# eric612/Mobilenet-YOLO-Pytorch

Hardware: AMD Instinct MI355X
Metric: images/sec MobileNetV2-YOLO 352x352 fwd+bwd @ bs256 (higher is better)
Workload: dtype f32; 1 GPU; MobileNetV2-YOLO 352x352 bs=256/GPU fwd+loss+bwd fp32 (BASELINE configs[1]); global_batch=256, parallelism=dp1

## Files before the change

### include/mnyolo.h

```cpp
#ifndef MNYOLO_H
#define MNYOLO_H

#include <stddef.h>
#include <stdint.h>

#ifdef __cplusplus
extern "C" {
#endif
#pragma GCC visibility push(default)

#define MNY_OK 0
#define MNY_EINVAL (-1)
#define MNY_EHIP (-2)
#define MNY_EUNSUPPORTED (-3)

#define MNY_ACT_NONE 0
#define MNY_ACT_RELU6 1
#define MNY_ACT_LEAKY 2
#define MNY_ACT_RELU 3
#define MNY_ACT_HSWISH 4
#define MNY_ACT_HSIGMOID 5

int mny_version(void);
const char* mny_last_error(void);
// ... 58 lines not shown
int mny_bn_bwd_parts(int64_t M, int C);
int mny_bn_bwd_finalize(const float* red, int parts, int64_t count, const float* gamma,
                        const float* mean, const float* invstd,
                        float* dgamma, float* dbeta, float* coef , int C, void* stream);
int mny_bn_bwd_apply(const float* g, const float* y, const float* scale, const float* shift, int act,
                     const float* coef, float* dy, int64_t M, int C, void* stream);

int mny_add_views(const float* a, const float* a_scale, const float* a_shift, int a_act,
                  const float* b, const float* b_scale, const float* b_shift, int b_act,
                  const float* up, float* out, int N, int H, int W, int C, void* stream);
int mny_mul_views(const float* a, const float* a_scale, const float* a_shift, int a_act,
                  const float* b, const float* b_scale, const float* b_shift, int b_act,
                  float* out, int64_t M, int C, void* stream);
int mny_mul_views_bwd(const float* g, const float* o, const float* o_scale, const float* o_shift, int o_act,
                      const float* addend, float* dst, int64_t M, int C, void* stream);
int mny_partadd_up(const float* a, const float* a_scale, const float* a_shift, int a_act, const float* up,
                   float* out, int N, int H, int W, int Ca, int Cb, void* stream);
int mny_slice_channels(const float* src, float* dst, int accumulate, int64_t M, int Ca, int Cb, void* stream);
int mny_upsample_bwd(const float* src, float* dst, int accumulate, int N, int H, int W, int C, void* stream);
int mny_axpy(const float* src, const float* alpha, float* dst, int accumulate, int64_t n, void* stream);

typedef struct {
    int N, g, A, C;
    int n_anchors_all;
    float ignore_thresh, iou_thresh, iou_weighting;
} mny_yolo_head;

int mny_yolo_loss(const float* head, const float* targets, const int32_t* t_off,
                  const float* anchors_all, const int32_t* mask, const mny_yolo_head* hp,
                  float* out7, float* dhead, void* ws, void* stream);
size_t mny_yolo_loss_ws_bytes(const mny_yolo_head* hp, int total_targets);

int mny_yolo_decode(const float* head, const float* anchors_all, const int32_t* mask,
                    const mny_yolo_head* hp, float val_conf, float* rows, int row_stride,
                    const int32_t* base_counts, int32_t* counts, void* stream);

int mny_nms_per_class(const float* rows, const int32_t* seg_begin, const int32_t* seg_count, int S,
                      int capacity, int max_seg_rows, int num_classes, double thr,
                      int32_t* out_idx, int32_t* out_counts, float* out_rows, void* ws, void* stream);
size_t mny_nms_ws_bytes(int S, int capacity, int num_classes);
size_t mny_nms_status_offset(int S, int capacity, int num_classes);
size_t mny_nms_prefix_offset(int S, int capacity, int num_classes);

int mny_dw_bnbwd_supported(int K, int stride);
int mny_dw_bnbwd_parts(int N, int H, int W, int C);
int mny_dw_bnbwd_parts_k(int N, int H, int W, int C, int K, int flags);
int mny_dw_bnbwd(const float* g, const float* y, const float* scale, const float* shift, int act, const float* coef,
                 const float* x, const float* in_scale, const float* in_shift, int in_act, const float* w,
                 const float* addend, float* dx, float* dw, float* ws, int N, int H, int W, int C, int K, int stride,
                 void* stream);
int mny_dw_bnbwd_s2_parts(int N, int H, int W, int C);
int mny_dw_bnbwd_s2(const float* g, const float* y, const float* scale, const float* shift, int act, const float* coef,
                    const float* x, const float* in_scale, const float* in_shift, int in_act, const float* w,
                    const float* addend, float* dx, float* dw, float* ws, int N, int H, int W, int C, void* stream);
int mny_dw_bnbwd_red(const float* g, const float* y, const float* scale, const float* shift, int act, const float* coef,
                     const float* x, const float* in_scale, const float* in_shift, int in_act, const float* in_mean,
                     const float* in_invstd, const float* w, const float* addend, float* dx, float* dw, float* ws, float* in_red,
                     int N, int H, int W, int C, int K, int stride, void* stream);

int mny_lr_supported(int64_t M, int K, int C);
int mny_lr_gram_parts(int64_t M, int K);
int mny_lr_gram(const float* x, const float* in_scale, const float* in_shift, int in_act, float* parts, int64_t M, int K, void* stream);
int mny_lr_gram_bf16(const void* x, const float* in_scale, const float* in_shift, int in_act, float* parts, int64_t M, int K, void* stream);
int mny_lr_prep(const float* coef, const float* w, float* q, float* r, int C, int K, void* stream);
int mny_pw_lr_fix_parts(int64_t M, int K, int r_act);
int mny_pw_lr_fix(const float* x, const float* in_scale, const float* in_shift, const float* q, const float* r, const float* addend, float* dx,
                  const float* ry, const float* r_scale, const float* r_shift, int r_act, const float* r_mean, const float* r_invstd, float* red,
                  int64_t M, int K, void* stream);
int mny_lr_wfix(float* dw, const float* gram_sums, const float* coef, const float* w, int C, int K, void* stream);
int mny_dw_bnbwd_s2_red_dz(const float* g, const float* y, const float* scale, const float* shift, int act, const float* coef,
                           const float* x, const float* in_scale, const float* in_shift, int in_act, const float* in_mean,
                           const float* in_invstd, const float* w, const float* addend, float* dx, float* dw, float* ws, float* in_red,
                           int N, int H, int W, int C, void* stream);
int mny_dw_bnbwd_s2k5_parts(int N, int H, int W, int C);
int mny_dw_bnbwd_s2k5(const float* g, const float* y, const float* scale, const float* shift, int act, const float* coef,
                      const float* x, const float* in_scale, const float* in_shift, int in_act, const float* in_mean,
                      const float* in_invstd, const float* w, const float* addend, float* dx, float* dw, float* ws, float* in_red,
                      int N, int H, int W, int C, void* stream);
int mny_dw_bnbwd_s2k5_bf16(const void* g, const void* y, const float* scale, const float* shift, int act, const float* coef,
                           const void* x, const float* in_scale, const float* in_shift, int in_act, const float* in_mean,
                           const float* in_invstd, const float* w, const void* addend, void* dx, float* dw, float* ws, float* in_red,
                           int N, int H, int W, int C, void* stream);
int mny_dw_bnbwd_red_dz_supported(int K, int C, int bf16);
int mny_dw_bnbwd_red_dz(const float* g, const float* y, const float* scale, const float* shift, int act, const float* coef,
                        const float* x, const float* in_scale, const float* in_shift, int in_act, const float* in_mean,
                        const float* in_invstd, const float* w, const float* addend, float* dx, float* dw, float* ws, float* in_red,
                        int N, int H, int W, int C, int K, int stride, void* stream);

int mny_pad_rows(const float* src, const float* alpha, float* dst, int64_t M, int C, int Cp, void* stream);
int mny_transpose_pad(const float* src , float* dst , int R, int Cc, int Rp, void* stream);

typedef struct mny_reduce_job {
    const float* parts;
    float* out;
    int64_t n;
    int32_t nparts, block0;
} mny_reduce_job;
int mny_reduce_batch(const mny_reduce_job* jobs, const int32_t* block_job, int nblocks, void* stream);
int mny_pw_wgrad_splits(int64_t M, int K, int Nc);

typedef struct mny_transpose_job {
    const float* src;
    void* dst;
    int32_t R, Cc, Rp, block0;
} mny_transpose_job;
int mny_transpose_batch(const mny_transpose_job* jobs, const int32_t* block_job, int nblocks, void* stream);

typedef struct mny_adamw_chunk {
    float* p;
    const float* g;
    float* m;
    float* v;
    int n;
    int vec4;
} mny_adamw_chunk;
int mny_adamw_step(const mny_adamw_chunk* table_dev, int nchunks, double lr, double beta1, double beta2, double eps,
                   double weight_decay, int64_t step, void* stream);

int mny_pw_dgrad_bnred_supported(int64_t M, int K, int Nc, int act);
int mny_pw_dgrad_bnred_parts(int64_t M, int K, int Nc);
int mny_pw_dgrad_bnred(const float* dy, const float* wT, float* dx, const float* y, const float* scale,
                       const float* shift, int act, const float* mean, const float* invstd, float* red,
                       int64_t M, int K, int Nc, void* stream);
int mny_pw_dgrad_bnred_add_supported(int64_t M, int K, int Nc, int act);
int mny_pw_dgrad_bnred_add(const float* dy, const float* wT, const float* addend, float* dx, const float* y, const float* scale,
                           const float* shift, int act, const float* mean, const float* invstd, float* red, int64_t M, int K, int Nc,
                           void* stream);

typedef struct mny_cut3_job {
    const float* src;
    void* dst;
    int32_t R, C, block0, pad;
} mny_cut3_job;
int mny_pw_w6_supported(int64_t M, int K, int Nc);
size_t mny_pw_w6_bytes(int K, int Nc);
int mny_cut3_batch(const mny_cut3_job* jobs, const int32_t* block_job, int nblocks, void* stream);
int mny_pw_fwd_w6(const float* x, const float* in_scale, const float* in_shift, int in_act, const void* w6, const float* bias,
                  const float* addend, float* y, float* stats, int64_t M, int K, int Nc, void* stream);
int mny_pw_dgrad_bnred_w6(const float* dy, const void* wT6, const float* addend, float* dx, const float* y, const float* scale,
                          const float* shift, int act, const float* mean, const float* invstd, float* red, int64_t M, int K, int Nc,
                          void* stream);

enum {
    MNY_ROUTE_TILE_V1 = 0,
    MNY_ROUTE_DMA_F32 = 1,
    MNY_ROUTE_DMA_X6 = 2,
    MNY_ROUTE_THIN = 3,
    MNY_ROUTE_WIDE = 4,
    MNY_ROUTE_WGRAD_STREAM = 5,
    MNY_ROUTE_WAVE16 = 6
};
int mny_pw_route(int op, int bf16, int64_t M, int K, int Nc);
int mny_pw_last_route(void);

size_t mny_map_ws_bytes(int64_t D, int64_t T);
int mny_map_eval(const float* det_boxes , const float* det_labels, const float* det_scores,
                 const int32_t* det_off , const float* true_boxes ,
                 const float* true_labels, const float* true_diff, const int32_t* true_off, int n_images,
                 int64_t D, int64_t T, int n_classes, float* ap, float* tp_sum, float* fp_sum, float* prec11,
                 float* mean_ap, void* ws, void* stream);
int mny_eval_pack(const float* rows, int64_t D, const float* targets, int64_t T, float* det_boxes,
                  float* det_labels, float* det_scores, float* true_boxes, float* true_labels,
                  float* true_diff, void* stream);

size_t mny_seg_loss_ws_bytes(int64_t n);
int mny_seg_loss(const float* head, const float* seg_maps, int64_t n, float* out3, float* dhead, void* ws,
                 void* stream);
int mny_seg_sigmoid(const float* head , int h, int w, int C, float* out,
                    void* stream);

typedef struct mny_image_desc {
    int64_t offset;
    int32_t h, w;
} mny_image_desc;
size_t mny_prep_ws_bytes(int N, int max_in_h, int max_in_w, int out_h, int out_w);
int mny_prep_batch(const uint8_t* src, const mny_image_desc* desc, int N, int max_in_h, int max_in_w, int out_h,
                   int out_w, const float* mean3, const float* std3, float* out, void* ws, void* stream);

#define MNY_AUG_BRIGHTNESS 0
#define MNY_AUG_CONTRAST 1
#define MNY_AUG_SATURATION 2
#define MNY_AUG_HUE 3
#define MNY_AUG_GAMMA 4
typedef struct mny_aug_item {
    mny_image_desc src;
    int32_t n_ops;
    int32_t op[5];
    float factor[5];
    int32_t hue_shift;
    uint8_t gamma_map[256];
    int32_t exp_h, exp_w, exp_top, exp_left;
    int32_t crop_top, crop_left, crop_h, crop_w;
    int32_t flip;
    int32_t sample;
    int32_t tile_x, tile_y, tile_w, tile_h;
    int32_t mask_x0, mask_y0, mask_x1, mask_y1;
} mny_aug_item;
typedef struct mny_aug_sample {
    int32_t first_item, n_items, canvas_slot, reserved;
} mny_aug_sample;
size_t mny_aug_ws_bytes(int n_items, int n_out, int n_mosaic, int max_in_h, int max_in_w, int canvas, int out_h,
                        int out_w);
int mny_aug_photometric(const uint8_t* src, const mny_aug_item* items, int n, int max_in_h, int max_in_w,
                        uint8_t* dst, void* ws, void* stream);
int mny_aug_batch(const uint8_t* src, const mny_aug_item* items, int n_items, const mny_aug_sample* samples,
                  int n_out, int max_in_h, int max_in_w, int canvas, int n_mosaic, int out_h, int out_w,
                  const float* mean3, const float* std3, float* out, void* ws, void* stream);

#define MNY_AUG_SEG_MAX_CLASSES 8
size_t mny_aug_seg_ws_bytes(int n_items, int n_out, int n_classes, int max_in_h, int max_in_w, int out_h, int out_w);
int mny_aug_seg_batch(const uint8_t* seg_src, const int64_t* seg_offsets, const mny_aug_item* items, int n_items,
                      const mny_aug_sample* samples, int n_out, int n_classes, int max_in_h, int max_in_w, int out_h,
                      int out_w, float* out, void* ws, void* stream);

int mny_stem_fwd_bf16(const float* x_nchw, const float* w, void* y, float* stats, int N, int H, int W, int Cout, void* stream);
int mny_stem_wgrad_bf16(const float* x_nchw, const void* dy, float* dw, float* ws, int N, int H, int W, int Cout, void* stream);
int mny_dw_fwd_bf16(const void* x, const float* in_scale, const float* in_shift, int in_act, const float* w, void* y,
                    float* stats, int N, int H, int W, int C, int K, int stride, void* stream);
int mny_dw_bwd_data_bf16(const void* dy, const float* w, const void* addend, void* dx, int N, int H, int W, int C, int K,
                         int stride, void* stream);
int mny_dw_bwd_weight_bf16(const void* x, const float* in_scale, const float* in_shift, int in_act, const void* dy,
                           float* dw, float* ws, int N, int H, int W, int C, int K, int stride, void* stream);
int mny_pw_fwd_bf16(const void* x, const float* in_scale, const float* in_shift, int in_act, const void* w_bf16,
                    const float* bias, const void* addend, void* y, float* stats, int64_t M, int K, int Nc, void* stream);
int mny_transpose_bf16(const float* src , void* dst , int R, int Cc, void* stream);
int mny_pw_stat_parts_bf16(int64_t M, int K, int Nc);
int mny_pw_wgrad_bf16(const void* x, const float* in_scale, const float* in_shift, int in_act, const void* dy, float* dw,
                      float* dbias, float* ws, int64_t M, int K, int Nc, void* stream);
int mny_bn_bwd_reduce_bf16(const void* g, const void* y, const float* scale, const float* shift, int act, const float* mean,
                           const float* invstd, float* red, int64_t M, int C, void* stream);
int mny_bn_bwd_apply_bf16(const void* g, const void* y, const float* scale, const float* shift, int act, const float* coef,
                          void* dy, int64_t M, int C, void* stream);
int mny_add_views_bf16(const void* a, const float* a_scale, const float* a_shift, int a_act, const void* b,
                       const float* b_scale, const float* b_shift, int b_act, const void* up, void* out, int N, int H, int W,
                       int C, void* stream);
int mny_mul_views_bf16(const void* a, const float* a_scale, const float* a_shift, int a_act, const void* b,
                       const float* b_scale, const float* b_shift, int b_act, void* out, int64_t M, int C, void* stream);
int mny_mul_views_bwd_bf16(const void* g, const void* o, const float* o_scale, const float* o_shift, int o_act,
                           const void* addend, void* dst, int64_t M, int C, void* stream);
int mny_partadd_up_bf16(const void* a, const float* a_scale, const float* a_shift, int a_act, const void* up, void* out,
                        int N, int H, int W, int Ca, int Cb, void* stream);
int mny_slice_channels_bf16(const void* src, void* dst, int accumulate, int64_t M, int Ca, int Cb, void* stream);
int mny_upsample_bwd_bf16(const void* src, void* dst, int accumulate, int N, int H, int W, int C, void* stream);
int mny_dw_bnbwd_bf16(const void* g, const void* y, const float* scale, const float* shift, int act, const float* coef,
                      const void* x, const float* in_scale, const float* in_shift, int in_act, const float* w,
                      const void* addend, void* dx, float* dw, float* ws, int N, int H, int W, int C, int K, int stride,
                      void* stream);
int mny_dw_bnbwd_s2_bf16(const void* g, const void* y, const float* scale, const float* shift, int act, const float* coef,
                         const void* x, const float* in_scale, const float* in_shift, int in_act, const float* w,
                         const void* addend, void* dx, float* dw, float* ws, int N, int H, int W, int C, void* stream);
int mny_dw_bnbwd_red_bf16(const void* g, const void* y, const float* scale, const float* shift, int act, const float* coef,
                          const void* x, const float* in_scale, const float* in_shift, int in_act, const float* in_mean,
                          const float* in_invstd, const float* w, const void* addend, void* dx, float* dw, float* ws, float* in_red,
                          int N, int H, int W, int C, int K, int stride, void* stream);
int mny_pad_rows_bf16(const float* src, const float* alpha, void* dst, int64_t M, int C, int Cp, void* stream);
int mny_transpose_pad_bf16(const float* src, void* dst, int R, int Cc, int Rp, void* stream);
int mny_stem_bnwgrad_bf16(const float* x_nchw, const void* g, const void* y, const float* scale, const float* shift, int act,
                          const float* coef, float* dw, float* ws, int N, int H, int W, int Cout, void* stream);
int mny_pw_bnbwd_supported_bf16(int64_t M, int K, int Nc);
int mny_pw_bnbwd_bf16(const void* g, const void* y, const float* scale, const float* shift, int act, const float* mean, const float* invstd,
                      const float* gamma, const void* x, const float* in_scale, const float* in_shift, int in_act, const float* w,
                      const void* addend, void* dx, float* dw, float* dgamma, float* dbeta, float* ws, int64_t M, int K, int Nc, void* stream);
int mny_pw_dgrad_bnred_supported_bf16(int64_t M, int K, int Nc, int act);
int mny_pw_dgrad_bnred_parts_bf16(int64_t M, int K, int Nc);
int mny_pw_dgrad_bnred_bf16(const void* dy, const void* wT, void* dx, const void* y, const float* scale, const float* shift, int act,
                            const float* mean, const float* invstd, float* red, int64_t M, int K, int Nc, void* stream);
int mny_pw_dgrad_bnred_add_supported_bf16(int64_t M, int K, int Nc, int act);
int mny_pw_dgrad_bnred_add_bf16(const void* dy, const void* wT, const void* addend, void* dx, const void* y, const float* scale,
                                const float* shift, int act, const float* mean, const float* invstd, float* red, int64_t M, int K,
                                int Nc, void* stream);
int mny_transpose_batch_bf16(const mny_transpose_job* jobs, const int32_t* block_job, int nblocks, void* stream);
int mny_pw_wgrad_splits_bf16(int64_t M, int K, int Nc);
int mny_axpy_bf16(const void* src, const float* alpha, void* dst, int accumulate, int64_t n, void* stream);
typedef struct mny_cvt_job {
    const float* src;
    void* dst;
    int64_t n;
    int32_t block0, pad_;
} mny_cvt_job;
int mny_cvt_batch_f32_bf16(const mny_cvt_job* jobs, const int32_t* block_job, int nblocks, void* stream);
int mny_cvt_f32_bf16(const float* src, void* dst, int64_t n, void* stream);
int mny_cvt_bf16_f32(const void* src, float* dst, int64_t n, void* stream);

int mny_bn_eval_stats(const float* running_mean, const float* running_var, float eps, float* mean_out, float* invstd_out, int C,
                      void* stream);
int mny_bn_bwd_finalize_frozen(const float* red, int parts, int64_t count, const float* gamma, const float* mean, const float* invstd,
                               float* dgamma, float* dbeta, float* coef, int C, void* stream);
int mny_exdw_supported(int N, int H, int W, int K, int C, int stride);
int mny_exdw_stat_parts(int64_t M, int K, int C);
int mny_exdw_stats(const float* x, const float* in_scale, const float* in_shift, int in_act, const float* w_exp, float* stats,
                   int64_t M, int K, int C, void* stream);
int mny_exdw_fwd_parts(int N, int H, int W, int K, int C, int stride);
int mny_exdw_fwd(const float* x, const float* in_scale, const float* in_shift, int in_act, const float* w_exp,
                 const float* e_scale, const float* e_shift, const float* w_dw, float* z, float* z_stats,
                 int N, int H, int W, int K, int C, int stride, void* stream);
int mny_exdw_bwd_parts(int N, int H, int W, int K, int C, int stride);
size_t mny_exdw_bwd_ws_floats(int N, int H, int W, int K, int C, int stride);
int mny_exdw_bwd(const float* gz, const float* z, const float* z_scale, const float* z_shift, int z_act, const float* z_coef,
                 const float* x, const float* in_scale, const float* in_shift, int in_act, const float* w_exp,
                 const float* e_scale, const float* e_shift, const float* e_mean, const float* e_invstd, const float* e_gamma,
                 const float* w_dw, const float* addend, float* dx, float* dw_exp, float* dgamma_e, float* dbeta_e,
                 float* dw_dw, float* dw_ws, float* ws, int N, int H, int W, int K, int C, int stride, void* stream);
int mny_exdw_bwd_red_parts(int N, int H, int W, int K, int C, int stride);
int mny_exdw_bwd_red(const float* gz, const float* z, const float* z_scale, const float* z_shift, int z_act, const float* z_coef,
                     const float* x, const float* in_scale, const float* in_shift, int in_act, const float* in_mean, const float* in_invstd,
                     const float* w_exp, const float* e_scale, const float* e_shift, const float* e_mean, const float* e_invstd,
// ... 59 lines not shown
```

### mobilenet-yolo-pytorch_amd/_lib.py

```python
import ctypes
import os
from ctypes import c_char_p, c_double, c_float, c_int, c_int32, c_int64, c_size_t, c_void_p

from . import switches

HERE = os.path.dirname(os.path.abspath(__file__))
LIB_PATH = switches.get("MNY_LIB") or os.path.join(HERE, "libmnyolo.so")

ACT_NONE, ACT_RELU6, ACT_LEAKY, ACT_RELU, ACT_HSWISH, ACT_HSIGMOID = 0, 1, 2, 3, 4, 5
ROUTE_TILE_V1, ROUTE_DMA_F32, ROUTE_DMA_X6, ROUTE_THIN, ROUTE_WIDE, ROUTE_WGRAD_STREAM, ROUTE_WAVE16 = 0, 1, 2, 3, 4, 5, 6


class MnyError(RuntimeError):
    pass


class YoloHead(ctypes.Structure):
    _fields_ = [("N", c_int), ("g", c_int), ("A", c_int), ("C", c_int), ("n_anchors_all", c_int),
                ("ignore_thresh", c_float), ("iou_thresh", c_float), ("iou_weighting", c_float)]


P = c_void_p
_SIGS = {
    "mny_version": (c_int, []),
    "mny_last_error": (c_char_p, []),
    "mny_max_parts": (c_int, []),
    "mny_stem_fwd": (c_int, [P, P, P, P, c_int, c_int, c_int, c_int, P]),
    "mny_stem_stat_parts": (c_int, [c_int, c_int, c_int, c_int]),
    "mny_stem_wgrad": (c_int, [P, P, P, P, c_int, c_int, c_int, c_int, P]),
    "mny_stem_bnwgrad_supported": (c_int, [c_int]),
    "mny_stem_bnwgrad": (c_int, [P, P, P, P, P, c_int, P, P, P, c_int, c_int, c_int, c_int, P]),
    "mny_stem_wgrad_parts": (c_int, [c_int, c_int, c_int, c_int]),
    "mny_dw_fwd": (c_int, [P, P, P, c_int, P, P, P, c_int, c_int, c_int, c_int, c_int, c_int, P]),
    "mny_dw_stat_parts": (c_int, [c_int] * 6),
    "mny_dw_stat_parts_x": (c_int, [c_int] * 7),
    "mny_dw_bwd_data": (c_int, [P, P, P, P, c_int, c_int, c_int, c_int, c_int, c_int, P]),
    "mny_dw_bwd_weight": (c_int, [P, P, P, c_int, P, P, P, c_int, c_int, c_int, c_int, c_int, c_int, P]),
    "mny_dw_wgrad_parts": (c_int, [c_int] * 6),
    "mny_dw_bnbwd_supported": (c_int, [c_int, c_int]),
    "mny_dw_bnbwd_parts": (c_int, [c_int] * 4),
    "mny_dw_bnbwd_parts_k": (c_int, [c_int] * 6),
    "mny_dw_bnbwd": (c_int, [P, P, P, P, c_int, P, P, P, P, c_int, P, P, P, P, P, c_int, c_int, c_int, c_int, c_int, c_int, P]),
    "mny_dw_bnbwd_s2_parts": (c_int, [c_int] * 4),
    "mny_dw_bnbwd_s2": (c_int, [P, P, P, P, c_int, P, P, P, P, c_int, P, P, P, P, P, c_int, c_int, c_int, c_int, P]),
    "mny_dw_bnbwd_red": (c_int, [P, P, P, P, c_int, P, P, P, P, c_int, P, P, P, P, P, P, P, P, c_int, c_int, c_int, c_int, c_int, c_int, P]),
    "mny_exdw_supported": (c_int, [c_int] * 6),
    "mny_exdw_stat_parts": (c_int, [c_int64, c_int, c_int]),
    "mny_exdw_stats": (c_int, [P, P, P, c_int, P, P, c_int64, c_int, c_int, P]),
    "mny_exdw_fwd_parts": (c_int, [c_int] * 6),
    "mny_exdw_fwd": (c_int, [P, P, P, c_int, P, P, P, P, P, P, c_int, c_int, c_int, c_int, c_int, c_int, P]),
    "mny_exdw_bwd_parts": (c_int, [c_int] * 6),
    "mny_exdw_bwd_ws_floats": (c_size_t, [c_int] * 6),
    "mny_exdw_bwd": (c_int, [P, P, P, P, c_int, P, P, P, P, c_int, P, P, P, P, P, P, P, P, P, P, P, P, P, P, P,
                             c_int, c_int, c_int, c_int, c_int, c_int, P]),
    "mny_exdw_bwd_red_parts": (c_int, [c_int] * 6),
    "mny_exdw_bwd_red": (c_int, [P, P, P, P, c_int, P, P, P, P, c_int, P, P, P, P, P, P, P, P, P, P, P, P, P, P, P, P, P, P,
                                 c_int, c_int, c_int, c_int, c_int, c_int, P]),
    "mny_pj_bwd_supported": (c_int, [c_int64, c_int, c_int, c_int]),
    "mny_pj_bwd_parts": (c_int, [c_int64, c_int, c_int]),
    "mny_pj_bwd": (c_int, [P, P, P, P, P, P, P, P, c_int, P, P, P, P, P, c_int64, c_int, c_int, P]),
    "mny_stemdw_supported": (c_int, [c_int] * 6),
    "mny_stemdw_bwd_parts": (c_int, [c_int] * 4),
    "mny_stemdw_bwd_ws_floats": (c_size_t, [c_int] * 4),
    "mny_stemdw_bwd": (c_int, [P, P, P, P, c_int, P, P, P, P, P, P, P, c_int, P, P, P, P, P, P, P, P, P, c_int, c_int, c_int, c_int, P]),
    "mny_adamw_step": (c_int, [P, c_int, c_double, c_double, c_double, c_double, c_double, c_int64, P]),
    "mny_pw_fwd": (c_int, [P, P, P, c_int, P, P, P, P, P, c_int64, c_int, c_int, P]),
    "mny_pw_stat_parts": (c_int, [c_int64, c_int, c_int]),
    "mny_pw_wgrad": (c_int, [P, P, P, c_int, P, P, P, P, c_int64, c_int, c_int, P]),
    "mny_pw_wgrad_ws_floats": (c_size_t, [c_int64, c_int, c_int]),
    "mny_pw_bnbwd_supported": (c_int, [c_int64, c_int, c_int]),
    "mny_pw_bnbwd_ws_floats": (c_size_t, [c_int64, c_int, c_int]),
    "mny_pw_bnbwd": (c_int, [P, P, P, P, c_int, P, P, P, P, P, P, c_int, P, P, P, P, P, P, P, c_int64, c_int, c_int, P]),
    "mny_pw_dgrad_bnred_supported": (c_int, [c_int64, c_int, c_int, c_int]),
    "mny_pw_dgrad_bnred_parts": (c_int, [c_int64, c_int, c_int]),
    "mny_pw_dgrad_bnred": (c_int, [P, P, P, P, P, P, c_int, P, P, P, c_int64, c_int, c_int, P]),
    "mny_pw_dgrad_bnred_add_supported": (c_int, [c_int64, c_int, c_int, c_int]),
    "mny_pw_dgrad_bnred_add": (c_int, [P, P, P, P, P, P, P, c_int, P, P, P, c_int64, c_int, c_int, P]),
    "mny_pw_route": (c_int, [c_int, c_int, c_int64, c_int, c_int]),
    "mny_pw_last_route": (c_int, []),
    "mny_pw_w6_supported": (c_int, [c_int64, c_int, c_int]),
    "mny_pw_w6_bytes": (c_size_t, [c_int, c_int]),
    "mny_cut3_batch": (c_int, [P, P, c_int, P]),
    "mny_pw_fwd_w6": (c_int, [P, P, P, c_int, P, P, P, P, P, c_int64, c_int, c_int, P]),
    "mny_pw_dgrad_bnred_w6": (c_int, [P, P, P, P, P, P, P, c_int, P, P, P, c_int64, c_int, c_int, P]),
    "mny_transpose_batch": (c_int, [P, P, c_int, P]),
    "mny_reduce_batch": (c_int, [P, P, c_int, P]),
    "mny_pw_wgrad_splits": (c_int, [c_int64, c_int, c_int]),
    "mny_transpose": (c_int, [P, P, c_int, c_int, P]),
    "mny_transpose_pad": (c_int, [P, P, c_int, c_int, c_int, P]),
    "mny_pad_rows": (c_int, [P, P, P, c_int64, c_int, c_int, P]),
    "mny_bn_finalize": (c_int, [P, c_int, c_int64, P, P, c_float, c_float, P, P, P, P, P, P, c_int, P]),
    "mny_bn_eval_coeffs": (c_int, [P, P, P, P, c_float, P, P, c_int, P]),
    "mny_bn_bwd_reduce": (c_int, [P, P, P, P, c_int, P, P, P, c_int64, c_int, P]),
    "mny_bn_bwd_parts": (c_int, [c_int64, c_int]),
    "mny_bn_bwd_finalize": (c_int, [P, c_int, c_int64, P, P, P, P, P, P, c_int, P]),
    "mny_bn_eval_stats": (c_int, [P, P, c_float, P, P, c_int, P]),
    "mny_bn_bwd_finalize_frozen": (c_int, [P, c_int, c_int64, P, P, P, P, P, P, c_int, P]),
    "mny_bn_bwd_apply": (c_int, [P, P, P, P, c_int, P, P, c_int64, c_int, P]),
    "mny_add_views": (c_int, [P, P, P, c_int, P, P, P, c_int, P, P, c_int, c_int, c_int, c_int, P]),
    "mny_mul_views": (c_int, [P, P, P, c_int, P, P, P, c_int, P, c_int64, c_int, P]),
    "mny_mul_views_bwd": (c_int, [P, P, P, P, c_int, P, P, c_int64, c_int, P]),
    "mny_partadd_up": (c_int, [P, P, P, c_int, P, P, c_int, c_int, c_int, c_int, c_int, P]),
    "mny_slice_channels": (c_int, [P, P, c_int, c_int64, c_int, c_int, P]),
    "mny_upsample_bwd": (c_int, [P, P, c_int, c_int, c_int, c_int, c_int, P]),
    "mny_axpy": (c_int, [P, P, P, c_int, c_int64, P]),
    "mny_yolo_loss": (c_int, [P, P, P, P, P, ctypes.POINTER(YoloHead), P, P, P, P]),
    "mny_yolo_loss_ws_bytes": (c_size_t, [ctypes.POINTER(YoloHead), c_int]),
    "mny_yolo_decode": (c_int, [P, P, P, ctypes.POINTER(YoloHead), c_float, P, c_int, P, P, P]),
    "mny_nms_per_class": (c_int, [P, P, P, c_int, c_int, c_int, c_int, c_double, P, P, P, P, P]),
    "mny_nms_ws_bytes": (c_size_t, [c_int, c_int, c_int]),
    "mny_nms_status_offset": (c_size_t, [c_int, c_int, c_int]),
    "mny_nms_prefix_offset": (c_size_t, [c_int, c_int, c_int]),
    "mny_map_ws_bytes": (c_size_t, [c_int64, c_int64]),
    "mny_map_eval": (c_int, [P, P, P, P, P, P, P, P, c_int, c_int64, c_int64, c_int, P, P, P, P, P, P, P]),
    "mny_seg_loss_ws_bytes": (c_size_t, [c_int64]),
    "mny_seg_loss": (c_int, [P, P, c_int64, P, P, P, P]),
    "mny_seg_sigmoid": (c_int, [P, c_int, c_int, c_int, P, P]),
    "mny_prep_ws_bytes": (c_size_t, [c_int] * 5),
    "mny_prep_batch": (c_int, [P, P, c_int, c_int, c_int, c_int, c_int, P, P, P, P, P]),
    "mny_aug_ws_bytes": (c_size_t, [c_int] * 8),
    "mny_aug_photometric": (c_int, [P, P, c_int, c_int, c_int, P, P, P]),
    "mny_aug_batch": (c_int, [P, P, c_int, P, c_int, c_int, c_int, c_int, c_int, c_int, c_int, P, P, P, P, P]),
    "mny_aug_seg_ws_bytes": (c_size_t, [c_int] * 7),
    "mny_aug_seg_batch": (c_int, [P, P, P, c_int, P, c_int, c_int, c_int, c_int, c_int, c_int, P, P, P]),
    "mny_eval_pack": (c_int, [P, c_int64, P, c_int64, P, P, P, P, P, P, P]),
}
BF16_TWINS = ("mny_pj_bwd_supported", "mny_pj_bwd_parts", "mny_pj_bwd", "mny_pw_bnbwd_supported", "mny_pw_bnbwd", "mny_pw_wgrad_splits", "mny_transpose_batch", "mny_pw_dgrad_bnred_supported", "mny_pw_dgrad_bnred_parts", "mny_pw_dgrad_bnred", "mny_pw_dgrad_bnred_add", "mny_pw_dgrad_bnred_add_supported", "mny_stem_bnwgrad", "mny_pad_rows", "mny_transpose_pad", "mny_dw_bnbwd", "mny_dw_bnbwd_s2", "mny_dw_bnbwd_red", "mny_stem_fwd", "mny_stem_wgrad", "mny_dw_fwd", "mny_dw_bwd_data", "mny_dw_bwd_weight", "mny_pw_fwd",
              "mny_pw_stat_parts", "mny_pw_wgrad", "mny_bn_bwd_reduce", "mny_bn_bwd_apply", "mny_add_views", "mny_mul_views",
              "mny_mul_views_bwd", "mny_partadd_up", "mny_slice_channels", "mny_upsample_bwd", "mny_axpy")
for _n in BF16_TWINS:
    _SIGS[_n + "_bf16"] = _SIGS[_n]
_SIGS["mny_gate_supported"] = (c_int, [c_int64, c_int, c_int])
_SIGS["mny_gate_parts"] = (c_int, [c_int64])
_SIGS["mny_gate_bwd_parts"] = (c_int, [c_int64])
_SIGS["mny_gate_bwd_red3_supported"] = (c_int, [c_int, c_int])
_SIGS["mny_gate_wq_bytes"] = (c_size_t, [c_int, c_int])
_SIGS["mny_gate_cut_batch_bf16"] = (c_int, [P, c_int, P])
_SIGS["mny_gate_stats1_bf16"] = (c_int, [P, P, P, P, P, c_int64, c_int, c_int, P])
_SIGS["mny_gate_stats2_bf16"] = (c_int, [P, P, P, P, P, P, P, c_int64, c_int, c_int, P])
_SIGS["mny_gate_fwd_bf16"] = (c_int, [P, P, P, P, P, P, P, P, P, P, P, c_int, P, c_int64, c_int, c_int, P])
_SIGS["mny_gate_bwd1_bf16"] = (c_int, [P] * 12 + [c_int64, c_int, c_int, P])
_SIGS["mny_gate_bwd2_bf16"] = (c_int, [P] * 14 + [c_int64, c_int, c_int, P])
_SIGS["mny_gate_bwd3_bf16"] = (c_int, [P] * 16 + [c_int64, c_int, c_int, P])
_SIGS["mny_lr_supported"] = (c_int, [c_int64, c_int, c_int])
_SIGS["mny_lr_gram_parts"] = (c_int, [c_int64, c_int])
_SIGS["mny_lr_gram"] = (c_int, [P, P, P, c_int, P, c_int64, c_int, P])
_SIGS["mny_lr_gram_bf16"] = _SIGS["mny_lr_gram"]
_SIGS["mny_lr_prep"] = (c_int, [P, P, P, P, c_int, c_int, P])
_SIGS["mny_pw_lr_fix_parts"] = (c_int, [c_int64, c_int, c_int])
_SIGS["mny_pw_lr_fix"] = (c_int, [P, P, P, P, P, P, P, P, P, P, c_int, P, P, P, c_int64, c_int, P])
_SIGS["mny_lr_wfix"] = (c_int, [P, P, P, P, c_int, c_int, P])
_SIGS["mny_pw_bnbwd_red_supported"] = (c_int, [c_int64, c_int, c_int])
_SIGS["mny_pw_bnbwd_red_parts"] = (c_int, [c_int64, c_int, c_int])
_SIGS["mny_pw_bnbwd_red"] = (c_int, [P, P, P, P, c_int, P, P, P, P, P, P, c_int, P, P, P, P, P, P, P, P, P, P, c_int, P, P, P, c_int64, c_int, c_int, P])
_SIGS["mny_dw_bnbwd_red_dz_supported"] = (c_int, [c_int, c_int, c_int])
_SIGS["mny_dw_bnbwd_red_dz"] = _SIGS["mny_dw_bnbwd_red"]
_SIGS["mny_dw_bnbwd_s2_red_dz"] = (c_int, [P, P, P, P, c_int, P, P, P, P, c_int, P, P, P, P, P, P, P, P, c_int, c_int, c_int, c_int, P])
_SIGS["mny_dw_bnbwd_s2k5_parts"] = (c_int, [c_int] * 4)
_SIGS["mny_dw_bnbwd_s2k5"] = _SIGS["mny_dw_bnbwd_s2_red_dz"]
_SIGS["mny_dw_bnbwd_s2k5_bf16"] = _SIGS["mny_dw_bnbwd_s2_red_dz"]
_SIGS["mny_transpose_bf16"] = _SIGS["mny_transpose"]
_SIGS["mny_cvt_f32_bf16"] = (c_int, [P, P, c_int64, P])
_SIGS["mny_cvt_batch_f32_bf16"] = (c_int, [P, P, c_int, P])
_SIGS["mny_cvt_bf16_f32"] = (c_int, [P, P, c_int64, P])
EXPORTS = tuple(_SIGS)

_lib = None


def load():
    global _lib
    if _lib is None:
        if not os.path.exists(LIB_PATH):
            raise MnyError("libmnyolo.so not found at %s — run __graft_entry__.build() (hipcc, gfx950). "
                           "There is no CPU fallback." % LIB_PATH)
        switches.warn_unknown()
        lib = ctypes.CDLL(LIB_PATH)
        for name, (res, args) in _SIGS.items():
            fn = getattr(lib, name)
            fn.restype = res
            fn.argtypes = args
        _lib = lib
    return _lib


def call(name, *args):
    lib = load()
    rc = getattr(lib, name)(*args)
    if rc != 0:
        raise MnyError("%s failed (%d): %s" % (name, rc, lib.mny_last_error().decode()))


def query(name, *args):
    v = getattr(load(), name)(*args)
    if isinstance(v, int) and v < 0:
        raise MnyError("%s(%s) -> %d: %s" % (name, args, v, load().mny_last_error().decode()))
    return v
```

### mobilenet-yolo-pytorch_amd/build.py

```python
import os
import subprocess
from concurrent.futures import ThreadPoolExecutor

HERE = os.path.dirname(os.path.abspath(__file__))
CSRC = os.path.join(HERE, "csrc")
OBJ = os.path.join(CSRC, "_obj")
LIB = os.path.join(HERE, "libmnyolo.so")
HIPCC = os.environ.get("HIPCC", "/opt/rocm/bin/hipcc")
ARCH = "gfx950"
BASE_FLAGS = ["--offload-arch=" + ARCH, "-O3", "-std=c++17", "-fPIC", "-Wall", "-Wno-unused-function",
              "-fvisibility=hidden", "-fvisibility-inlines-hidden"]
EXTRA = {"detect.hip": ["-ffp-contract=off"], "evalmap.hip": ["-ffp-contract=off"], "prep.hip": ["-ffp-contract=off"],
         "augment.hip": ["-ffp-contract=off"]}


def sources():
    return sorted(f for f in os.listdir(CSRC) if f.endswith(".hip"))


def _stale(target, deps):
    if not os.path.exists(target):
        return True
    t = os.path.getmtime(target)
    return any(os.path.getmtime(d) > t for d in deps)


def build(force=False, verbose=False):
    os.makedirs(OBJ, exist_ok=True)
    headers = [os.path.join(CSRC, "common.h"), os.path.join(CSRC, "x6.h"), os.path.join(HERE, "..", "include", "mnyolo.h")]
    jobs, objs = [], []
    for src in sources():
        s = os.path.join(CSRC, src)
        o = os.path.join(OBJ, src[:-4] + ".o")
        objs.append(o)
        if force or _stale(o, [s] + headers):
            jobs.append([HIPCC] + BASE_FLAGS + EXTRA.get(src, []) + ["-c", s, "-o", o])

    def run(cmd):
        if verbose:
            print(" ".join(cmd))
        subprocess.check_call(cmd)

    if jobs:
        with ThreadPoolExecutor(max_workers=min(4, len(jobs))) as ex:
            list(ex.map(run, jobs))
    if jobs or force or _stale(LIB, objs):
        run([HIPCC, "--offload-arch=" + ARCH, "-shared", "-fPIC", "-fvisibility=hidden", "-Wl,--exclude-libs,ALL", "-o", LIB] + objs)
    return LIB


if __name__ == "__main__":
    print(build(verbose=True))
```

### mobilenet-yolo-pytorch_amd/csrc/bn_eltwise.hip

```cpp
#include "common.h"

namespace mny {

__device__ __forceinline__ void sum_partial_rows(const float* __restrict__ rows, int parts, int C, int c, int slice, double& s, double& q) {
    double s1 = 0.0, q1 = 0.0, s2 = 0.0, q2 = 0.0, s3 = 0.0, q3 = 0.0;
    s = 0.0; q = 0.0;
    int p = slice;
    const int64_t step = (int64_t)64 * C;
    const float* a = rows + (int64_t)p * 2 * C + c;
    for (; p + 480 < parts; p += 512, a += 16 * step) {
        float v[16], u[16];
#pragma unroll
        for (int i = 0; i < 16; ++i) { v[i] = a[i * step]; u[i] = a[i * step + C]; }
#pragma unroll
        for (int i = 0; i < 16; i += 4) {
            s += (double)v[i];      q += (double)u[i];
            s1 += (double)v[i + 1]; q1 += (double)u[i + 1];
            s2 += (double)v[i + 2]; q2 += (double)u[i + 2];
            s3 += (double)v[i + 3]; q3 += (double)u[i + 3];
        }
    }
    for (; p + 96 < parts; p += 128, a += 4 * step) {
        const float v0 = a[0], u0 = a[C], v1 = a[step], u1 = a[step + C], v2 = a[2 * step], u2 = a[2 * step + C], v3 = a[3 * step], u3 = a[3 * step + C];
        s += (double)v0;  q += (double)u0;
        s1 += (double)v1; q1 += (double)u1;
        s2 += (double)v2; q2 += (double)u2;
        s3 += (double)v3; q3 += (double)u3;
    }
    for (; p < parts; p += 32, a += step) {
        s += (double)a[0];
        q += (double)a[C];
    }
    s = (s + s1) + (s2 + s3);
    q = (q + q1) + (q2 + q3);
}

__global__ __launch_bounds__(1024) void bn_finalize_kernel(const float* __restrict__ stats, int parts, double count,
                                                          const float* __restrict__ gamma, const float* __restrict__ beta,
                                                          float eps, float momentum, float* running_mean, float* running_var,
                                                          float* scale, float* shift, float* mean_out, float* invstd_out, int C) {
    __shared__ double red[2][32][32];
    const int cl = threadIdx.x & 31, slice = threadIdx.x >> 5;
    const int c = blockIdx.x * 32 + cl;
    double s = 0.0, q = 0.0;
    if (c < C) {
        sum_partial_rows(stats, parts, C, c, slice, s, q);
    }
    red[0][slice][cl] = s;
    red[1][slice][cl] = q;
    __syncthreads();
    if (slice == 0 && c < C) {
        s = 0.0; q = 0.0;
        for (int i = 0; i < 32; ++i) { s += red[0][i][cl]; q += red[1][i][cl]; }
        const double mean = s / count;
        double var = q / count - mean * mean;
        if (var < 0.0) var = 0.0;
        const float invstd = (float)(1.0 / sqrt(var + (double)eps));
        const float sc = gamma[c] * invstd;
        scale[c] = sc;
        shift[c] = beta[c] - (float)mean * sc;
        if (mean_out) mean_out[c] = (float)mean;
        if (invstd_out) invstd_out[c] = invstd;
        if (running_mean) {
            const double unbiased = count > 1.0 ? var * count / (count - 1.0) : var;
            running_mean[c] = (1.f - momentum) * running_mean[c] + momentum * (float)mean;
            running_var[c] = (1.f - momentum) * running_var[c] + momentum * (float)unbiased;
        }
    }
}

__global__ void bn_eval_coeffs_kernel(const float* gamma, const float* beta, const float* rm, const float* rv, float eps,
                                      float* scale, float* shift, int C) {
    const int c = blockIdx.x * blockDim.x + threadIdx.x;
    if (c >= C) return;
    const float sc = gamma[c] / sqrtf(rv[c] + eps);
    scale[c] = sc;
    shift[c] = beta[c] - rm[c] * sc;
}

template <typename T>
__global__ __launch_bounds__(256) void bn_bwd_reduce_kernel(const T* __restrict__ g, const T* __restrict__ y,
                                                            const float* __restrict__ scale, const float* __restrict__ shift, int act,
                                                            const float* __restrict__ mean, const float* __restrict__ invstd,
                                                            float* __restrict__ red_out, int64_t M, int C, int cgb, int cg_total) {
    __shared__ float4 red[256 * 2];
    const int tid = threadIdx.x;
    const int cgl = tid % cgb, pix = tid / cgb, ppb = blockDim.x / cgb;
    const int cg = blockIdx.y * cgb + cgl;
    const bool cvalid = cg < cg_total;
    const int c = cg * 4;
    float4 s1 = f4zero(), s2 = f4zero();
    if (cvalid) {
        const float4 sc = ld4(scale + c), sh = ld4(shift + c), mu = ld4(mean + c), is = ld4(invstd + c);
        auto accum = [&](float4 gv, float4 yv) {
            float4 dz;
            dz.x = gv.x * act_bwd(fmaf(yv.x, sc.x, sh.x), act);
            dz.y = gv.y * act_bwd(fmaf(yv.y, sc.y, sh.y), act);
            dz.z = gv.z * act_bwd(fmaf(yv.z, sc.z, sh.z), act);
            dz.w = gv.w * act_bwd(fmaf(yv.w, sc.w, sh.w), act);
            add4(s1, dz);
            s2.x = fmaf(dz.x, (yv.x - mu.x) * is.x, s2.x);
            s2.y = fmaf(dz.y, (yv.y - mu.y) * is.y, s2.y);
            s2.z = fmaf(dz.z, (yv.z - mu.z) * is.z, s2.z);
            s2.w = fmaf(dz.w, (yv.w - mu.w) * is.w, s2.w);
        };
        const int64_t stride = (int64_t)gridDim.x * ppb;
        int64_t m = (int64_t)blockIdx.x * ppb + pix;
        constexpr int U = sizeof(T) == 2 ? 4 : 1;
        if (U > 1) {
            for (; m + (U - 1) * stride < M; m += U * stride) {
                float4 gv[U], yv[U];
#pragma unroll
                for (int u = 0; u < U; ++u) { gv[u] = ld4(g + (m + u * stride) * C + c); yv[u] = ld4(y + (m + u * stride) * C + c); }
#pragma unroll
                for (int u = 0; u < U; ++u) accum(gv[u], yv[u]);
            }
        }
        for (; m < M; m += stride) accum(ld4(g + m * C + c), ld4(y + m * C + c));
    }
    red[tid * 2] = s1;
    red[tid * 2 + 1] = s2;
    __syncthreads();
    if (pix == 0 && cvalid) {
        float4 a = f4zero(), b = f4zero();
        for (int p = 0; p < ppb; ++p) { add4(a, red[(p * cgb + cgl) * 2]); add4(b, red[(p * cgb + cgl) * 2 + 1]); }
        st4(red_out + (int64_t)blockIdx.x * 2 * C + c, a);
        st4(red_out + (int64_t)blockIdx.x * 2 * C + C + c, b);
    }
}

__global__ __launch_bounds__(1024) void bn_bwd_finalize_kernel(const float* __restrict__ red_in, int parts, double count,
                                                              const float* __restrict__ gamma, const float* __restrict__ mean,
                                                              const float* __restrict__ invstd, float* dgamma, float* dbeta,
                                                              float* coef, int C) {
    __shared__ double red[2][32][32];
    const int cl = threadIdx.x & 31, slice = threadIdx.x >> 5;
    const int c = blockIdx.x * 32 + cl;
    double s = 0.0, q = 0.0;
    if (c < C) {
        sum_partial_rows(red_in, parts, C, c, slice, s, q);
    }
    red[0][slice][cl] = s;
    red[1][slice][cl] = q;
    __syncthreads();
    if (slice == 0 && c < C) {
        s = 0.0; q = 0.0;
        for (int i = 0; i < 32; ++i) { s += red[0][i][cl]; q += red[1][i][cl]; }
        dbeta[c] = (float)s;
        dgamma[c] = (float)q;
        const double a = (double)gamma[c] * (double)invstd[c];
        const double b = -a * (double)invstd[c] * q / count;
        coef[c] = (float)a;
        coef[C + c] = (float)b;
        coef[2 * C + c] = (float)(-a * s / count - b * (double)mean[c]);
    }
}

template <typename T>
__global__ __launch_bounds__(256) void bn_bwd_apply_kernel(const T* __restrict__ g, const T* __restrict__ y,
                                                           const float* __restrict__ scale, const float* __restrict__ shift, int act,
                                                           const float* __restrict__ coef, T* __restrict__ dy,
                                                           int64_t M, int C, int cgb, int cg_total) {
    const int cgl = threadIdx.x % cgb, pix = threadIdx.x / cgb, ppb = blockDim.x / cgb;
    const int cg = blockIdx.y * cgb + cgl;
    if (cg >= cg_total) return;
    const int c = cg * 4;
    const float4 sc = scale ? ld4(scale + c) : f4one(), sh = scale ? ld4(shift + c) : f4zero();
    const float4 ca = coef ? ld4(coef + c) : f4one();
    const float4 cb = coef ? ld4(coef + C + c) : f4zero();
    const float4 cc = coef ? ld4(coef + 2 * C + c) : f4zero();
    for (int64_t m = (int64_t)blockIdx.x * ppb + pix; m < M; m += (int64_t)gridDim.x * ppb) {
        const float4 gv = ld4(g + m * C + c), yv = ld4(y + m * C + c);
        float4 o;
        o.x = fmaf(ca.x, gv.x * act_bwd(fmaf(yv.x, sc.x, sh.x), act), fmaf(cb.x, yv.x, cc.x));
        o.y = fmaf(ca.y, gv.y * act_bwd(fmaf(yv.y, sc.y, sh.y), act), fmaf(cb.y, yv.y, cc.y));
        o.z = fmaf(ca.z, gv.z * act_bwd(fmaf(yv.z, sc.z, sh.z), act), fmaf(cb.z, yv.z, cc.z));
        o.w = fmaf(ca.w, gv.w * act_bwd(fmaf(yv.w, sc.w, sh.w), act), fmaf(cb.w, yv.w, cc.w));
        st4_stream(dy + m * C + c, o);
    }
}

template <typename T>
__global__ __launch_bounds__(256) void add_views_kernel(const T* __restrict__ a, const float* __restrict__ a_scale,
                                                        const float* __restrict__ a_shift, int a_act,
                                                        const T* __restrict__ b, const float* __restrict__ b_scale,
                                                        const float* __restrict__ b_shift, int b_act,
                                                        const T* __restrict__ up, T* __restrict__ out,
                                                        int N, int H, int W, int C, int cgb, int cg_total) {
    const int cgl = threadIdx.x % cgb, pix = threadIdx.x / cgb, ppb = blockDim.x / cgb;
    const int cg = blockIdx.y * cgb + cgl;
    if (cg >= cg_total) return;
    const int c = cg * 4;
    const float4 asc = a_scale ? ld4(a_scale + c) : f4one(), ash = a_scale ? ld4(a_shift + c) : f4zero();
    const float4 bsc = b_scale ? ld4(b_scale + c) : f4one(), bsh = b_scale ? ld4(b_shift + c) : f4zero();
    const int64_t M = (int64_t)N * H * W;
    for (int64_t m = (int64_t)blockIdx.x * ppb + pix; m < M; m += (int64_t)gridDim.x * ppb) {
        float4 o = xform4(ld4(a + m * C + c), asc, ash, a_act);
        if (b) add4(o, xform4(ld4(b + m * C + c), bsc, bsh, b_act));
        if (up) {
            const int wi = (int)(m % W), hi = (int)((m / W) % H);
            const int64_t n = m / ((int64_t)W * H);
            add4(o, ld4(up + ((n * (H / 2) + hi / 2) * (W / 2) + wi / 2) * C + c));
        }
        st4_stream(out + m * C + c, o);
    }
}

template <typename T>
__global__ __launch_bounds__(256) void upsample_bwd_kernel(const T* __restrict__ src, T* __restrict__ dst, int accumulate,
                                                           int N, int H, int W, int C, int cgb, int cg_total) {
    const int cgl = threadIdx.x % cgb, pix = threadIdx.x / cgb, ppb = blockDim.x / cgb;
    const int cg = blockIdx.y * cgb + cgl;
    if (cg >= cg_total) return;
    const int c = cg * 4;
    const int Hh = H / 2, Wh = W / 2;
    const int64_t M = (int64_t)N * Hh * Wh;
    for (int64_t m = (int64_t)blockIdx.x * ppb + pix; m < M; m += (int64_t)gridDim.x * ppb) {
        const int wi = (int)(m % Wh), hi = (int)((m / Wh) % Hh);
        const int64_t n = m / ((int64_t)Wh * Hh);
        const T* s = src + ((n * H + 2 * hi) * W + 2 * wi) * C + c;
        float4 o = accumulate ? ld4(dst + m * C + c) : f4zero();
        add4(o, ld4(s)); add4(o, ld4(s + C));
        add4(o, ld4(s + (int64_t)W * C)); add4(o, ld4(s + (int64_t)W * C + C));
        st4(dst + m * C + c, o);
    }
}

template <typename T>
__global__ __launch_bounds__(256) void axpy_kernel(const T* __restrict__ src, const float* __restrict__ alpha,
                                                   T* __restrict__ dst, int accumulate, int64_t n4, int64_t n) {
    const float a = alpha ? alpha[0] : 1.f;
    for (int64_t i = (int64_t)blockIdx.x * blockDim.x + threadIdx.x; i < n4; i += (int64_t)gridDim.x * blockDim.x) {
        float4 v = ld4(src + i * 4);
        float4 d = accumulate ? ld4(dst + i * 4) : f4zero();
        d.x = fmaf(a, v.x, d.x); d.y = fmaf(a, v.y, d.y); d.z = fmaf(a, v.z, d.z); d.w = fmaf(a, v.w, d.w);
        st4(dst + i * 4, d);
    }
    if (blockIdx.x == 0 && threadIdx.x < (n & 3)) {
        const int64_t i = n4 * 4 + threadIdx.x;
        st1(dst + i, (accumulate ? ld1(dst + i) : 0.f) + a * ld1(src + i));
    }
}


template <typename T>
__global__ __launch_bounds__(256) void bn_bwd_reduce_c1_kernel(const T* __restrict__ g, const T* __restrict__ y,
                                                               const float* __restrict__ scale, const float* __restrict__ shift, int act,
                                                               const float* __restrict__ mean, const float* __restrict__ invstd,
                                                               float* __restrict__ red_out, int64_t M, int C, int cb) {
    __shared__ float red[256 * 2];
    const int tid = threadIdx.x;
    const int cl = tid % cb, pix = tid / cb, ppb = blockDim.x / cb;
    const int c = blockIdx.y * cb + cl;
    float s1 = 0.f, s2 = 0.f;
    if (c < C) {
        const float sc = scale[c], sh = shift[c], mu = mean[c], is = invstd[c];
        for (int64_t m = (int64_t)blockIdx.x * ppb + pix; m < M; m += (int64_t)gridDim.x * ppb) {
            const float yv = ld1(y + m * C + c);
            const float dz = ld1(g + m * C + c) * act_bwd(fmaf(yv, sc, sh), act);
            s1 += dz;
            s2 = fmaf(dz, (yv - mu) * is, s2);
        }
    }
    red[tid * 2] = s1; red[tid * 2 + 1] = s2;
    __syncthreads();
    if (pix == 0 && c < C) {
        float a = 0.f, b = 0.f;
        for (int p = 0; p < ppb; ++p) { a += red[(p * cb + cl) * 2]; b += red[(p * cb + cl) * 2 + 1]; }
        red_out[(int64_t)blockIdx.x * 2 * C + c] = a;
        red_out[(int64_t)blockIdx.x * 2 * C + C + c] = b;
    }
}

template <typename T>
__global__ __launch_bounds__(256) void bn_bwd_apply_c1_kernel(const T* __restrict__ g, const T* __restrict__ y,
                                                              const float* __restrict__ scale, const float* __restrict__ shift, int act,
                                                              const float* __restrict__ coef, T* __restrict__ dy, int64_t total, int C) {
    for (int64_t e = (int64_t)blockIdx.x * blockDim.x + threadIdx.x; e < total; e += (int64_t)gridDim.x * blockDim.x) {
        const int c = (int)(e % C);
        const float sc = scale ? scale[c] : 1.f, sh = scale ? shift[c] : 0.f;
        const float ca = coef ? coef[c] : 1.f, cb = coef ? coef[C + c] : 0.f, cc = coef ? coef[2 * C + c] : 0.f;
        const float yv = ld1(y + e);
        st1(dy + e, fmaf(ca, ld1(g + e) * act_bwd(fmaf(yv, sc, sh), act), fmaf(cb, yv, cc)));
    }
}

template <typename T>
__global__ __launch_bounds__(256) void mul_views_kernel(const T* __restrict__ a, const float* __restrict__ a_scale,
                                                        const float* __restrict__ a_shift, int a_act,
                                                        const T* __restrict__ b, const float* __restrict__ b_scale,
                                                        const float* __restrict__ b_shift, int b_act,
                                                        const T* __restrict__ addend, T* __restrict__ out,
                                                        int64_t M, int C, int cgb, int cg_total, int bwd) {
    const int cgl = threadIdx.x % cgb, pix = threadIdx.x / cgb, ppb = blockDim.x / cgb;
    const int cg = blockIdx.y * cgb + cgl;
    if (cg >= cg_total) return;
    const int c = cg * 4;
    const float4 asc = a_scale ? ld4(a_scale + c) : f4one(), ash = a_scale ? ld4(a_shift + c) : f4zero();
    const float4 bsc = b_scale ? ld4(b_scale + c) : f4one(), bsh = b_scale ? ld4(b_shift + c) : f4zero();
    for (int64_t m = (int64_t)blockIdx.x * ppb + pix; m < M; m += (int64_t)gridDim.x * ppb) {
        const float4 x = bwd ? ld4(a + m * C + c) : xform4(ld4(a + m * C + c), asc, ash, a_act);
        const float4 w = xform4(ld4(b + m * C + c), bsc, bsh, b_act);
        float4 o = addend ? ld4(addend + m * C + c) : f4zero();
        fma4(o, x, w);
        st4(out + m * C + c, o);
    }
}

// ... 349 lines not shown
```

### mobilenet-yolo-pytorch_amd/csrc/common.h

```cpp
#pragma once
#include <hip/hip_runtime.h>
#include <stdint.h>
#include <stdio.h>
#include <stdlib.h>
#include <type_traits>

#include "../../include/mnyolo.h"

namespace mny {

void set_error(const char* fmt, ...);
int check_launch(const char* what);
bool allow_lds(const void* kernel, size_t bytes);

#define MNY_REQUIRE(cond, ...)                 \
    do {                                       \
        if (!(cond)) {                         \
            mny::set_error(__VA_ARGS__);       \
            return MNY_EINVAL;                 \
        }                                      \
    } while (0)

constexpr int kWave = 64;
constexpr int kMaxParts = 1024;

__host__ __device__ inline int64_t cdiv(int64_t a, int64_t b) { return (a + b - 1) / b; }

__device__ __forceinline__ float act_slope(int act) { return act == MNY_ACT_NONE ? 1.f : (act == MNY_ACT_LEAKY ? 0.1f : 0.f); }
__device__ __forceinline__ float act_hi(int act) { return act == MNY_ACT_RELU6 ? 6.f : INFINITY; }
__device__ __forceinline__ float act_fwd(float z, int act) {
    if (act >= MNY_ACT_HSWISH) {
        const float h = fminf(fmaxf(z + 3.f, 0.f), 6.f) * (1.f / 6.f);
        return act == MNY_ACT_HSWISH ? z * h : h;
    }
    return fminf(fmaxf(z, act_slope(act) * z), act_hi(act));
}
__device__ __forceinline__ float act_bwd(float z, int act) {
    if (act == MNY_ACT_HSWISH) return z <= -3.f ? 0.f : (z >= 3.f ? 1.f : (2.f * z + 3.f) * (1.f / 6.f));
    if (act == MNY_ACT_HSIGMOID) return (z > -3.f && z < 3.f) ? (1.f / 6.f) : 0.f;
    return (z > 0.f ? 1.f : act_slope(act)) * (z < act_hi(act) ? 1.f : 0.f);
}

__device__ __forceinline__ float4 xform4(float4 v, float4 sc, float4 sh, int act) {
    float4 r;
    r.x = act_fwd(fmaf(v.x, sc.x, sh.x), act);
    r.y = act_fwd(fmaf(v.y, sc.y, sh.y), act);
    r.z = act_fwd(fmaf(v.z, sc.z, sh.z), act);
    r.w = act_fwd(fmaf(v.w, sc.w, sh.w), act);
    return r;
}

__device__ __forceinline__ float4 ld4(const float* p) { return *reinterpret_cast<const float4*>(p); }
__device__ __forceinline__ void st4(float* p, float4 v) { *reinterpret_cast<float4*>(p) = v; }

struct bf16_t { uint16_t v; };
__device__ __forceinline__ uint32_t pack_bf16x2(float lo, float hi) {
    typedef __attribute__((ext_vector_type(2))) __bf16 bf2_t;
    typedef __attribute__((ext_vector_type(2))) float f2_t;
    const f2_t f = {lo, hi};
    return __builtin_bit_cast(uint32_t, __builtin_convertvector(f, bf2_t));
}
__device__ __forceinline__ float4 ld4(const bf16_t* p) {
    const uint2 u = *reinterpret_cast<const uint2*>(p);
    return make_float4(__uint_as_float(u.x << 16), __uint_as_float(u.x & 0xffff0000u), __uint_as_float(u.y << 16),
                       __uint_as_float(u.y & 0xffff0000u));
}
__device__ __forceinline__ void st4(bf16_t* p, float4 v) {
    *reinterpret_cast<uint2*>(p) = make_uint2(pack_bf16x2(v.x, v.y), pack_bf16x2(v.z, v.w));
}
typedef float mny_f4v __attribute__((ext_vector_type(4)));
typedef unsigned mny_u2v __attribute__((ext_vector_type(2)));
__device__ __forceinline__ void st4_stream(float* p, float4 v) {
    const mny_f4v t = {v.x, v.y, v.z, v.w};
    __builtin_nontemporal_store(t, reinterpret_cast<mny_f4v*>(p));
}
__device__ __forceinline__ void st4_stream(bf16_t* p, float4 v) {
    const mny_u2v t = {pack_bf16x2(v.x, v.y), pack_bf16x2(v.z, v.w)};
    __builtin_nontemporal_store(t, reinterpret_cast<mny_u2v*>(p));
}
template <typename T> __device__ __forceinline__ T* at_bytes(T* base, unsigned byte_off) {
    return (T*)((char*)base + byte_off);
}
template <typename T> __device__ __forceinline__ const T* at_bytes(const T* base, unsigned byte_off) {
    return (const T*)((const char*)base + byte_off);
}

__device__ __forceinline__ float ld1(const float* p) { return *p; }
__device__ __forceinline__ void st1(float* p, float v) { *p = v; }
__device__ __forceinline__ float ld1(const bf16_t* p) { return __uint_as_float((uint32_t)p->v << 16); }
__device__ __forceinline__ void st1(bf16_t* p, float v) { p->v = (uint16_t)(pack_bf16x2(v, 0.f) & 0xffffu); }
template <typename T> __device__ __forceinline__ float stored(float v);
template <> __device__ __forceinline__ float stored<float>(float v) { return v; }
template <> __device__ __forceinline__ float stored<bf16_t>(float v) { return __uint_as_float(pack_bf16x2(v, 0.f) << 16); }
template <typename T> __device__ __forceinline__ float4 stored4(float4 v) {
    return make_float4(stored<T>(v.x), stored<T>(v.y), stored<T>(v.z), stored<T>(v.w));
}
__device__ __forceinline__ float4 f4zero() { return make_float4(0.f, 0.f, 0.f, 0.f); }
__device__ __forceinline__ float4 f4one() { return make_float4(1.f, 1.f, 1.f, 1.f); }
__device__ __forceinline__ void fma4(float4& acc, float4 a, float4 b) {
    acc.x = fmaf(a.x, b.x, acc.x); acc.y = fmaf(a.y, b.y, acc.y);
    acc.z = fmaf(a.z, b.z, acc.z); acc.w = fmaf(a.w, b.w, acc.w);
}
__device__ __forceinline__ void add4(float4& acc, float4 a) { acc.x += a.x; acc.y += a.y; acc.z += a.z; acc.w += a.w; }

typedef float v2f __attribute__((ext_vector_type(2)));
struct F4P { v2f lo, hi; };
__device__ __forceinline__ F4P f4p(float4 v) { F4P r; r.lo = v2f{v.x, v.y}; r.hi = v2f{v.z, v.w}; return r; }
__device__ __forceinline__ F4P f4p0() { F4P r; r.lo = v2f{0.f, 0.f}; r.hi = v2f{0.f, 0.f}; return r; }
__device__ __forceinline__ float4 f4u(F4P v) { return make_float4(v.lo.x, v.lo.y, v.hi.x, v.hi.y); }
__device__ __forceinline__ void pfma(F4P& acc, F4P a, F4P b) {
    acc.lo = __builtin_elementwise_fma(a.lo, b.lo, acc.lo);
    acc.hi = __builtin_elementwise_fma(a.hi, b.hi, acc.hi);
}

typedef float v4f_t __attribute__((ext_vector_type(4)));
typedef unsigned v4u_t __attribute__((ext_vector_type(4)));
__device__ __forceinline__ unsigned lds_off(const void* p) {
    return (unsigned)(uintptr_t)(const __attribute__((address_space(3))) char*)p;
}
__device__ __forceinline__ v4f_t lds_read_f4(const float* p) {
    v4f_t v;
    asm volatile("ds_read_b128 %0, %1" : "=v"(v) : "v"(lds_off(p)) : "memory");
    return v;
}
__device__ __forceinline__ v4u_t lds_read_u4(const float* p) {
    v4u_t v;
    asm volatile("ds_read_b128 %0, %1" : "=v"(v) : "v"(lds_off(p)) : "memory");
    return v;
}
template <int OFF>
__device__ __forceinline__ v4f_t lds_read_f4_at(unsigned base) {
    static_assert(OFF >= 0 && OFF < 65536, "ds offset field");
    v4f_t v;
    asm volatile("ds_read_b128 %0, %1 offset:%2" : "=v"(v) : "v"(base), "n"(OFF) : "memory");
    return v;
}
template <int B, int E, typename F>
__device__ __forceinline__ void static_for(F&& f) {
    if constexpr (B < E) {
        f(std::integral_constant<int, B>{});
        static_for<B + 1, E>(f);
    }
}
#define MNY_LGKM_WAIT(first) asm volatile("s_waitcnt lgkmcnt(0)" : "+v"(first))
#define MNY_LGKM_DEP(x) asm volatile("" : "+v"(x))

template <int N>
__device__ __forceinline__ void wait_vmcnt() { asm volatile("s_waitcnt vmcnt(%0)" ::"n"(N) : "memory"); }

#define MNY_SWITCHES(X)                                                                                                              \
    X(GEMM_V1, "MNY_GEMM_V1", kFlag, 0, 1, "pointwise forward / data gradients on the first-generation tile kernels")                \
    X(WGRAD_V1, "MNY_WGRAD_V1", kFlag, 0, 1, "pointwise weight gradients on the first-generation tile kernel")                       \
    X(WGRAD_NO_XCD, "MNY_WGRAD_NO_XCD", kFlag, 0, 1, "weight-gradient workgroups in plain order, not grouped per XCD")               \
    X(X6, "MNY_X6", kInt, -1, 1, "six-product bf16 GEMM: 0 = never (fp32 MFMA), 1 = wherever supported, -1 = per-shape rule")        \
    X(NO_W6, "MNY_NO_W6", kFlag, 0, 1, "no pre-cut weight operand for the six-product GEMM")                                         \
    X(NO_WIDE, "MNY_NO_WIDE", kFlag, 0, 1, "no barrier-free short-reduction kernel (pwwide.hip)")                                    \
    X(NO_WGS, "MNY_NO_WGS", kFlag, 0, 1, "no stream weight-gradient kernel (pwwgs.hip)")                                             \
    X(NO_THIN, "MNY_NO_THIN", kFlag, 0, 1, "no vector-ALU kernel for K = 8..32 (pwthin.hip)")                                        \
    X(NO_PWT, "MNY_NO_PWT", kFlag, 0, 1, "no wave-per-16-pixels thin pointwise kernel (gate.hip)")                                   \
    X(NO_PWE, "MNY_NO_PWE", kFlag, 0, 1, "no wave form of the thin expand unit backward (gate.hip)")                                 \
    X(NO_PJBWD, "MNY_NO_PJBWD", kFlag, 0, 1, "no fused projection backward (pjbwd.hip, gate.hip)")                                   \
    X(NO_LR, "MNY_NO_LR", kFlag, 0, 1, "no low-rank BatchNorm backward of the wide expand units (lrbwd.hip)")                        \
    X(NO_EXDW, "MNY_NO_EXDW", kFlag, 0, 1, "no fused expand + depthwise unit: the materialised path")                                \
    X(EXDW_STATS, "MNY_EXDW_STATS", kWord, 0, 0, "gram (default) | direct: how mny_exdw_stats forms its sums")                       \
    X(NO_STEMDW, "MNY_NO_STEMDW", kFlag, 0, 1, "no fused stem + depthwise backward (stemdw.hip)")                                    \
    X(STEM_WGRAD_VALU, "MNY_STEM_WGRAD_VALU", kFlag, 0, 1, "stem weight gradient on the vector ALU, not the matrix cores")           \
    X(DW_V1, "MNY_DW_V1", kFlag, 0, 1, "3x3 depthwise forward on the first-generation sliding-window kernel")                        \
    X(NO_DWT5, "MNY_NO_DWT5", kFlag, 0, 1, "no tile form of the 5x5 depthwise unit backward")                                        \
    X(DWT3, "MNY_DWT3", kInt, -1, 1, "tile form of the 3x3 depthwise unit backward: 0 / 1, -1 = per-shape rule")                     \
    X(DWTF, "MNY_DWTF", kInt, -1, 1, "tile form of the depthwise forward: 0 / 1, -1 = per-shape rule")                               \
    X(NMS_SMALL, "MNY_NMS_SMALL", kFlag, 0, 0, "NMS buckets of any size through the one-workgroup path")
enum SwitchType { kFlag, kInt, kWord };
enum Switch {
#define X(id, name, type, def, latch, doc) SW_##id,
    MNY_SWITCHES(X)
#undef X
    SW_COUNT
};
int sw(Switch id);

struct CgLayout {
    int cg_total;
    int chunks;
    int cgb;
    int ppb;
    int threads;
};
inline CgLayout make_cg_layout(int C) {
    CgLayout L;
    L.cg_total = C / 4;
    L.chunks = (int)cdiv(L.cg_total, 256);
    L.cgb = (int)cdiv(L.cg_total, L.chunks);
    L.ppb = 256 / L.cgb; if (L.ppb < 1) L.ppb = 1;
    L.threads = L.cgb * L.ppb;
    return L;
}


inline CgLayout make_stencil_layout(int C, int max_cgb = 64) {
    CgLayout L;
    L.cg_total = C / 4;
    L.chunks = (int)cdiv(L.cg_total, max_cgb);
    L.cgb = (int)cdiv(L.cg_total, L.chunks);
    L.ppb = 256 / L.cgb; if (L.ppb < 1) L.ppb = 1;
    L.threads = L.cgb * L.ppb;
    return L;
}

__global__ void reduce_parts_f64_kernel(const float* __restrict__ parts, int nparts, int n, float* __restrict__ out);
int launch_reduce_parts(const float* parts, int nparts, int n, float* out, hipStream_t st);

bool dwt_use(int K, int bf, int red, int C);
int dwt_parts(int N, int H, int W, int C, int K, int bf);
bool dwt_fwd_use(int K, int stride, int bf, int C);
int dwt_fwd_parts(int N, int H, int W, int C, int K);
int dwt_fwd_launch(int bf, const void* x, const float* in_scale, const float* in_shift, int in_act, const float* w, void* y, float* stats, int N, int H,
                   int W, int C, int K, void* stream);
int dwt_launch(int bf, const void* g, const void* y, const float* scale, const float* shift, int act, const float* coef, const void* x,
               const float* in_scale, const float* in_shift, int in_act, const float* w, const void* addend, void* dx, float* dw, float* ws, int N, int H,
               int W, int C, int K, void* stream, const float* in_mean, const float* in_invstd, float* in_red);

bool pwt_ok(int64_t M, int K, int N, int in_act, bool has_bias);
int pwt_parts(int64_t M);
int pwt_launch(const void* x, const float* xs, const float* xb, int xact, const void* w, const void* addend, void* y, float* stats, int64_t M, int K, int N,
               hipStream_t st, const void* rY = nullptr, const float* r_scale = nullptr, const float* r_shift = nullptr, const float* r_mean = nullptr,
               const float* r_invstd = nullptr, int r_act = 0);

bool pwe_ok(int64_t M, int K, int N);
size_t pwe_ws_floats(int64_t M, int K, int N);
int pwe_launch(const void* g, const void* y, const float* scale, const float* shift, int act, const float* mean, const float* invstd, const float* gamma,
               const void* x, const float* in_scale, const float* in_shift, int in_act, const float* w, const void* addend, void* dx, float* dw,
               float* dgamma, float* dbeta, float* ws, int64_t M, int K, int Nc, hipStream_t st);

bool pw_thin_ok(int bf, int red, int64_t M, int K, int N);
int pw_thin_parts(int64_t M, int K, int N, int red);
int pw_thin_launch(int bf, const void* A, const float* in_scale, const float* in_shift, int in_act, const void* W, const float* bias,
                   const void* addend, void* C, float* stats, int64_t M, int K, int N, int red, const void* rY, const float* r_scale,
                   const float* r_shift, const float* r_mean, const float* r_invstd, int r_act, hipStream_t st);

bool pw_wide_ok(int64_t M, int K, int N, bool red);
int pw_wide_parts(int64_t M, int K, int N, bool red);
int pw_wide_launch(const float* A, const float* in_scale, const float* in_shift, int in_act, const float* W, float* C, float* stats,
                   int64_t M, int K, int N, const float* rY, const float* r_scale, const float* r_shift, const float* r_mean,
                   const float* r_invstd, int r_act, const float* addend, hipStream_t st);

bool pw_wide_fix_ok(int64_t M, int K);
int pw_wide_fix_parts(int64_t M, int K);
int pw_wide_fix_launch(const float* A, const float* in_scale, const float* in_shift, const float* Q, const float* bias, const float* addend, float* C,
                       float* stats, int64_t M, int K, const float* rY, const float* r_scale, const float* r_shift, const float* r_mean,
                       const float* r_invstd, int r_act, hipStream_t st);

bool pw_wgs_ok(int64_t M, int K, int N);
int pw_wgs_splits(int64_t M, int K, int N);
int pw_wgs_launch(const float* x, const float* in_scale, const float* in_shift, int in_act, const float* dy, float* partial,
                  int64_t M, int K, int N, hipStream_t st);

__host__ __device__ inline int64_t bnw_stride(int N, int K) { return (int64_t)N * K + (int64_t)K * K + 2 * N + K; }
int pw_bnbwd_finalize_launch(const float* partials, int nparts, float* red, const float* w, const float* gamma, const float* mean,
                             const float* invstd, int64_t M, int Nc, int K, float* dw, float* dgamma, float* dbeta, float* B1, float* Q,
                             float* bias, hipStream_t st);

}
```

### mobilenet-yolo-pytorch_amd/csrc/pwgemm.hip

```cpp
#include <stdlib.h>

#include <map>
#include <type_traits>
#include <mutex>

#include "common.h"
#include "x6.h"

namespace mny {

constexpr int BM = 128;

struct GemmArgs {
    const void* A; const float* in_scale; const float* in_shift; int in_act;
    const void* B; const float* bias; const void* addend; void* C; float* stats;
    int64_t M; int K; int N;
    int m_tiles; int tiles_per_block;
};

template <typename T, int TN, int BK>
__global__ __launch_bounds__(256) void pw_gemm_nt_kernel(GemmArgs p) {
    constexpr int BN = 32 * TN;
    const T* pA = (const T*)p.A;
    const T* pAdd = (const T*)p.addend;
// ... 2304 lines not shown
                    rs1 = make_float4(a1[0], a1[1], a1[2], a1[3]); rs2 = make_float4(a2[0], a2[1], a2[2], a2[3]);
                }
            }
        }
        asm volatile("" ::: "memory");
        load_ad(next);
    }
    if constexpr (RED) {
        __syncthreads();
        float4* sr = reinterpret_cast<float4*>(sB);
        sr[tid] = rs1; sr[256 + tid] = rs2;
        __syncthreads();
        if (tid < 16 && tid * 4 < Kc) {
            float4 a = f4zero(), b = f4zero();
            for (int w = 0; w < 4; ++w)
                for (int h = 0; h < 2; ++h)
                    for (int j = 0; j < 4; ++j) {
                        const int l = w * 64 + h * 32 + tid * 4 + j;
                        add4(a, sr[l]); add4(b, sr[256 + l]);
                    }
            float* dst = p.red + (int64_t)blockIdx.x * 2 * Kc;
            st4(dst + tid * 4, a);
            st4(dst + Kc + tid * 4, b);
        }
    }
}

struct BnwPlan { int TI, splits; int64_t rows_per_block; size_t lds1, lds2; int gx2, tiles_per_block, m_tiles; int TIs, nsl; };

static bool bnw_supported(int64_t M, int K, int N) {
    return M >= 4096 && K <= 32 && K % 4 == 0 && N % 4 == 0 && N <= 192 && N > K;
}

static BnwPlan bnw_plan(int64_t M, int K, int N) {
    BnwPlan pl;
    pl.TI = (int)cdiv(N, 32);
    pl.nsl = pl.TI >= 5 ? 2 : 1;
    pl.TIs = (int)cdiv(pl.TI, pl.nsl);
    int64_t splits = (pl.TIs <= 3 ? 768 : 1024) / pl.nsl;
    const int64_t max_splits = cdiv(M, 64);
    if (splits > max_splits) splits = max_splits;
    pl.rows_per_block = cdiv(cdiv(M, splits), 16) * 16;
    pl.splits = (int)cdiv(M, pl.rows_per_block);
    pl.lds1 = (size_t)3 * 16 * (2 * 32 * pl.TIs + 32) * sizeof(float);
    const size_t need = (size_t)4 * (2 * pl.TIs + 1) * 32 * sizeof(float);
    if (pl.lds1 < need) pl.lds1 = need;
    if (pl.lds1 < 3 * 16 * 64 * sizeof(float)) pl.lds1 = 3 * 16 * 64 * sizeof(float);
    pl.lds2 = (size_t)3 * (64 * 32 + 32 * 32) * sizeof(float) + 64 * sizeof(float) + 2 * 16 * 64 * sizeof(float);
    pl.m_tiles = (int)cdiv(M, 64);
    int gx = pl.m_tiles < 768 ? pl.m_tiles : 768;
    pl.tiles_per_block = (int)cdiv(pl.m_tiles, gx);
    pl.gx2 = (int)cdiv(pl.m_tiles, pl.tiles_per_block);
    return pl;
}

int pw_bnbwd_finalize_launch(const float* partials, int nparts, float* red, const float* w, const float* gamma, const float* mean,
                             const float* invstd, int64_t M, int Nc, int K, float* dw, float* dgamma, float* dbeta, float* B1, float* Q,
                             float* bias, hipStream_t st) {
    const int64_t stride = bnw_stride(Nc, K);
    hipLaunchKernelGGL(reduce_parts_kernel, dim3((unsigned)cdiv(stride, 32)), dim3(256), 0, st, partials, nparts, stride, red);
    hipLaunchKernelGGL(pw_bnbwd_finalize_kernel, dim3((unsigned)cdiv((int64_t)Nc * K, 256)), dim3(256), bnw_finalize_lds(Nc, K), st, red, w, gamma,
                       mean, invstd, (double)M, Nc, K, dw, dgamma, dbeta, B1, Q, bias);
    return check_launch("pw_bnbwd_finalize_kernel");
}

}

using namespace mny;
static thread_local int g_pw_route = -1;

extern "C" int mny_pw_stat_parts(int64_t M, int K, int Nc) {
    if (M <= 0 || K <= 0 || Nc <= 0) return MNY_EINVAL;
    if (pw_thin_ok(0, 0, M, K, Nc)) return pw_thin_parts(M, K, Nc, 0);
    if (pw_wide_ok(M, K, Nc, false)) return pw_wide_parts(M, K, Nc, false) + ((M & 31) ? nt2_plan(M & 31, K, Nc, true).gx : 0);
    if ((K & 3) == 0 && !sw(SW_GEMM_V1)) return nt2_plan(M, K, Nc, true).gx;
    return nt_plan(M, K, Nc).gx;
}
extern "C" int mny_pw_stat_parts_bf16(int64_t M, int K, int Nc) {
    if (M <= 0 || K <= 0 || Nc <= 0) return MNY_EINVAL;
    if (pwt_ok(M, K, Nc, MNY_ACT_NONE, false)) return pwt_parts(M);
    if (pw_thin_ok(1, 0, M, K, Nc)) return pw_thin_parts(M, K, Nc, 0);
    if ((K & 7) == 0 && !sw(SW_GEMM_V1)) return nt2_plan(M, K, Nc, true, 1).gx;
    return nt_plan(M, K, Nc).gx;
}

template <typename T>
static int pw_fwd_v1(const T* x, const float* in_scale, const float* in_shift, int in_act, const T* w, const float* bias,
                     const T* addend, T* y, float* stats, int64_t M, int K, int Nc, hipStream_t st) {
    const bool xf = in_scale != nullptr || in_act != MNY_ACT_NONE;
    NtPlan pl = nt_plan(M, K, Nc, xf);
    MNY_REQUIRE(pl.lds <= 160 * 1024, "pw_fwd: K=%d too large for the LDS scale cache", K);
    GemmArgs a{x, in_scale, in_shift, in_act, w, bias, addend, y, stats, M, K, Nc, pl.m_tiles, pl.tiles_per_block};
    dim3 grid(pl.gx, pl.n_tiles), block(256);
    {
        const void* ks[] = {(const void*)pw_gemm_nt_kernel<T, 1, 16>, (const void*)pw_gemm_nt_kernel<T, 2, 16>, (const void*)pw_gemm_nt_kernel<T, 3, 16>,
                            (const void*)pw_gemm_nt_kernel<T, 4, 16>, (const void*)pw_gemm_nt_kernel<T, 1, 32>, (const void*)pw_gemm_nt_kernel<T, 2, 32>,
                            (const void*)pw_gemm_nt_kernel<T, 3, 32>, (const void*)pw_gemm_nt_kernel<T, 4, 32>};
        for (const void* k : ks)
            if (!allow_lds(k, 160 * 1024)) {
                set_error("pw_fwd: hipFuncSetAttribute failed"); return MNY_EHIP;
            }
    }
#define MNY_NT(TN_, B) hipLaunchKernelGGL((pw_gemm_nt_kernel<T, TN_, B>), grid, block, pl.lds, st, a)
    switch (pl.TN * 100 + pl.BK) {
        case 116: MNY_NT(1, 16); break; case 216: MNY_NT(2, 16); break; case 316: MNY_NT(3, 16); break; case 416: MNY_NT(4, 16); break;
        case 132: MNY_NT(1, 32); break; case 232: MNY_NT(2, 32); break; case 332: MNY_NT(3, 32); break; default: MNY_NT(4, 32); break;
    }
#undef MNY_NT
    return check_launch("pw_gemm_nt_kernel");
}

extern "C" int mny_pw_fwd(const float* x, const float* in_scale, const float* in_shift, int in_act, const float* w,
                          const float* bias, const float* addend, float* y, float* stats, int64_t M, int K, int Nc,
                          void* stream) {
    MNY_REQUIRE(x && w && y, "pw_fwd: null pointer");
    MNY_REQUIRE(M > 0 && K > 0 && Nc > 0, "pw_fwd: empty problem");
    MNY_REQUIRE(!(stats && bias), "pw_fwd: stats and bias are mutually exclusive");
    hipStream_t st = (hipStream_t)stream;
    const bool xf = in_scale != nullptr || in_act != MNY_ACT_NONE;
    const bool force_v1 = sw(SW_GEMM_V1);
    if (pw_thin_ok(0, 0, M, K, Nc)) {
        g_pw_route = MNY_ROUTE_THIN;
        return pw_thin_launch(0, x, in_scale, in_shift, in_act, w, bias, addend, y, stats, M, K, Nc, 0, nullptr, nullptr, nullptr, nullptr, nullptr, 0, st);
    }
    bool took_wide = false;
    if (pw_wide_ok(M, K, Nc, false)) {
        if (!bias && !addend && in_act != MNY_ACT_HSIGMOID) {
            const int64_t Mf = M & ~(int64_t)31;
            g_pw_route = MNY_ROUTE_WIDE;
            took_wide = true;
            const int rc = pw_wide_launch(x, in_scale, in_shift, in_act, w, y, stats, Mf, K, Nc, nullptr, nullptr, nullptr, nullptr, nullptr, 0, nullptr, st);
            if (rc != 0 || Mf == M) return rc;
            if (stats) stats += (int64_t)pw_wide_parts(M, K, Nc, false) * 2 * Nc;
            x += Mf * K; y += Mf * Nc; M -= Mf;
        } else {
            MNY_REQUIRE(!stats, "pw_fwd: statistics with a bias / addend / h-sigmoid input on a wide-kernel shape");
        }
    }
    if ((K & 3) == 0 && !force_v1) {
        Nt2Plan p2 = nt2_plan(M, K, Nc, xf);
        MNY_REQUIRE(p2.lds <= 64 * 1024, "pw_fwd: K=%d too large for the LDS scale cache", K);
        Gemm2Args g{x, in_scale, in_shift, in_act, w, bias, addend, y, stats, M, K, Nc, p2.m_tiles, p2.tiles_per_block, p2.gx, p2.n_tiles,
                    nullptr, nullptr, nullptr, nullptr, nullptr, 0};
        dim3 grid2(p2.grid), block2(256);
        const int XF = !xf ? 0 : (in_act == MNY_ACT_HSWISH ? 2 : 1);
        if (!took_wide) g_pw_route = nt_x6(M, K, Nc) ? MNY_ROUTE_DMA_X6 : MNY_ROUTE_DMA_F32;
        hipLaunchKernelGGL(nt2_kernel(p2.TN, XF, 0, nt_x6(M, K, Nc)), grid2, block2, p2.lds, st, g);
        return check_launch("pw_gemm_nt_dma_kernel");
    }
    if (!took_wide) g_pw_route = MNY_ROUTE_TILE_V1;
    return pw_fwd_v1<float>(x, in_scale, in_shift, in_act, w, bias, addend, y, stats, M, K, Nc, st);
}

constexpr int kRedMaxTn = 4;
static bool dgrad_bnred_ok(int64_t M, int K, int Nc, int act) {
    if (K >= 512 && Nc >= 512) return false;
    if ((pw_thin_ok(0, 1, M, K, Nc) || pw_thin_ok(1, 1, M, K, Nc)) && act == MNY_ACT_HSIGMOID) return false;
    if (pw_wide_ok(M, K, Nc, true) && act >= MNY_ACT_HSWISH) return false;
    return M > 0 && K > 0 && Nc > 0 && (K & 3) == 0 && act >= MNY_ACT_NONE && act <= MNY_ACT_HSIGMOID && !sw(SW_GEMM_V1);
}
extern "C" int mny_pw_dgrad_bnred_supported(int64_t M, int K, int Nc, int act) { return dgrad_bnred_ok(M, K, Nc, act) ? 1 : 0; }
extern "C" int mny_pw_dgrad_bnred_parts(int64_t M, int K, int Nc) {
    if (M <= 0 || K <= 0 || Nc <= 0 || (K & 3)) return MNY_EINVAL;
    if (pw_thin_ok(0, 1, M, K, Nc)) return pw_thin_parts(M, K, Nc, 1);
    if (pw_wide_ok(M, K, Nc, true)) return pw_wide_parts(M, K, Nc, true) + ((M & 31) ? nt2_plan(M & 31, K, Nc, false, 0, kRedMaxTn).gx : 0);
    return nt2_plan(M, K, Nc, false, 0, kRedMaxTn).gx;
}
template <int BF>
static int pw_dgrad_bnred_impl(const void* dy, const void* wT, void* dx, const void* y, const float* scale, const float* shift, int act,
                               const float* mean, const float* invstd, float* red, int64_t M, int K, int Nc, void* stream, const void* addend = nullptr) {
    MNY_REQUIRE(dy && wT && dx && y && scale && shift && mean && invstd && red, "pw_dgrad_bnred: null pointer");
    MNY_REQUIRE(dgrad_bnred_ok(M, K, Nc, act) && (!BF || (K & 7) == 0), "pw_dgrad_bnred: unsupported problem M=%lld K=%d N=%d act=%d (see mny_pw_dgrad_bnred_supported)",
                (long long)M, K, Nc, act);
    if (BF && pwt_ok(M, K, Nc, MNY_ACT_NONE, false)) {
        g_pw_route = MNY_ROUTE_WAVE16;
        return pwt_launch(dy, nullptr, nullptr, MNY_ACT_NONE, wT, addend, dx, red, M, K, Nc, (hipStream_t)stream, y, scale, shift, mean, invstd, act);
    }
    if (pw_thin_ok(BF, 1, M, K, Nc)) g_pw_route = MNY_ROUTE_THIN;
    if (pw_thin_ok(BF, 1, M, K, Nc))
        return pw_thin_launch(BF, dy, nullptr, nullptr, MNY_ACT_NONE, wT, nullptr, addend, dx, red, M, K, Nc, addend ? 2 : 1, y, scale, shift, mean, invstd, act,
                              (hipStream_t)stream);
    bool took_wide = false;
    if (!BF && pw_wide_ok(M, K, Nc, true)) {
        g_pw_route = MNY_ROUTE_WIDE;
        took_wide = true;
        const int64_t Mf = M & ~(int64_t)31;
        const int rc = pw_wide_launch((const float*)dy, nullptr, nullptr, MNY_ACT_NONE, (const float*)wT, (float*)dx, red, Mf, K, Nc, (const float*)y, scale, shift,
                                      mean, invstd, act, (const float*)addend, (hipStream_t)stream);
        if (rc != 0 || Mf == M) return rc;
        red += (int64_t)pw_wide_parts(M, K, Nc, true) * 2 * Nc;
        dy = (const float*)dy + Mf * K; dx = (float*)dx + Mf * Nc; y = (const float*)y + Mf * Nc;
        if (addend) addend = (const float*)addend + Mf * Nc;
        M -= Mf;
    }
    Nt2Plan p2 = nt2_plan(M, K, Nc, false, BF, kRedMaxTn);
    MNY_REQUIRE(p2.lds <= 64 * 1024, "pw_dgrad_bnred: K=%d too large", K);
    Gemm2Args g{dy, nullptr, nullptr, MNY_ACT_NONE, wT, nullptr, addend, dx, red, M, K, Nc, p2.m_tiles, p2.tiles_per_block, p2.gx, p2.n_tiles,
                y, scale, shift, mean, invstd, act};
    Nt2Kernel k;
    constexpr int X = BF ? 0 : 1;
    const bool x6 = !BF && nt_x6(M, K, Nc);
    if (!took_wide) g_pw_route = x6 ? MNY_ROUTE_DMA_X6 : MNY_ROUTE_DMA_F32;
    if (addend) switch (p2.TN) {
        case 1: k = x6 ? (Nt2Kernel)pw_gemm_nt_dma_kernel<1, 0, BF, 2, X> : (Nt2Kernel)pw_gemm_nt_dma_kernel<1, 0, BF, 2>; break;
        case 2: k = x6 ? (Nt2Kernel)pw_gemm_nt_dma_kernel<2, 0, BF, 2, X> : (Nt2Kernel)pw_gemm_nt_dma_kernel<2, 0, BF, 2>; break;
        case 3: k = x6 ? (Nt2Kernel)pw_gemm_nt_dma_kernel<3, 0, BF, 2, X> : (Nt2Kernel)pw_gemm_nt_dma_kernel<3, 0, BF, 2>; break;
        default: k = x6 ? (Nt2Kernel)pw_gemm_nt_dma_kernel<4, 0, BF, 2, X> : (Nt2Kernel)pw_gemm_nt_dma_kernel<4, 0, BF, 2>; break;
    }
    else switch (p2.TN) {
        case 1: k = x6 ? (Nt2Kernel)pw_gemm_nt_dma_kernel<1, 0, BF, 1, X> : (Nt2Kernel)pw_gemm_nt_dma_kernel<1, 0, BF, 1>; break;
        case 2: k = x6 ? (Nt2Kernel)pw_gemm_nt_dma_kernel<2, 0, BF, 1, X> : (Nt2Kernel)pw_gemm_nt_dma_kernel<2, 0, BF, 1>; break;
        case 3: k = x6 ? (Nt2Kernel)pw_gemm_nt_dma_kernel<3, 0, BF, 1, X> : (Nt2Kernel)pw_gemm_nt_dma_kernel<3, 0, BF, 1>; break;
        default: k = x6 ? (Nt2Kernel)pw_gemm_nt_dma_kernel<4, 0, BF, 1, X> : (Nt2Kernel)pw_gemm_nt_dma_kernel<4, 0, BF, 1>; break;
    }
    hipLaunchKernelGGL(k, dim3(p2.grid), dim3(256), p2.lds, (hipStream_t)stream, g);
    return check_launch("pw_gemm_nt_dma_kernel<RED>");
}
extern "C" int mny_pw_dgrad_bnred(const float* dy, const float* wT, float* dx, const float* y, const float* scale, const float* shift, int act,
                                  const float* mean, const float* invstd, float* red, int64_t M, int K, int Nc, void* stream) {
    return pw_dgrad_bnred_impl<0>(dy, wT, dx, y, scale, shift, act, mean, invstd, red, M, K, Nc, stream);
}
extern "C" int mny_pw_dgrad_bnred_add_supported(int64_t M, int K, int Nc, int act) {
    return dgrad_bnred_ok(M, K, Nc, act) && (pw_thin_ok(0, 1, M, K, Nc) || pw_wide_ok(M, K, Nc, true) || nt2_plan(M, K, Nc, false, 0, kRedMaxTn).TN <= 3) ? 1 : 0;
}
extern "C" int mny_pw_dgrad_bnred_add_supported_bf16(int64_t M, int K, int Nc, int act) {
    return dgrad_bnred_ok(M, K, Nc, act) && (K & 7) == 0 && (pwt_ok(M, K, Nc, MNY_ACT_NONE, false) || pw_thin_ok(1, 1, M, K, Nc) || nt2_plan(M, K, Nc, false, 1, kRedMaxTn).TN <= 3) ? 1 : 0;
}
extern "C" int mny_pw_dgrad_bnred_add(const float* dy, const float* wT, const float* addend, float* dx, const float* y, const float* scale, const float* shift,
                                      int act, const float* mean, const float* invstd, float* red, int64_t M, int K, int Nc, void* stream) {
    MNY_REQUIRE(addend && mny_pw_dgrad_bnred_add_supported(M, K, Nc, act), "pw_dgrad_bnred_add: null addend or unsupported shape (mny_pw_dgrad_bnred_add_supported)");
    return pw_dgrad_bnred_impl<0>(dy, wT, dx, y, scale, shift, act, mean, invstd, red, M, K, Nc, stream, addend);
}
extern "C" int mny_pw_dgrad_bnred_add_bf16(const void* dy, const void* wT, const void* addend, void* dx, const void* y, const float* scale, const float* shift,
                                           int act, const float* mean, const float* invstd, float* red, int64_t M, int K, int Nc, void* stream) {
    MNY_REQUIRE(addend && mny_pw_dgrad_bnred_add_supported_bf16(M, K, Nc, act), "pw_dgrad_bnred_add: null addend or unsupported shape");
    return pw_dgrad_bnred_impl<1>(dy, wT, dx, y, scale, shift, act, mean, invstd, red, M, K, Nc, stream, addend);
}
extern "C" int mny_pw_dgrad_bnred_supported_bf16(int64_t M, int K, int Nc, int act) { return dgrad_bnred_ok(M, K, Nc, act) && (K & 7) == 0 ? 1 : 0; }
extern "C" int mny_pw_dgrad_bnred_parts_bf16(int64_t M, int K, int Nc) {
    if (M <= 0 || K <= 0 || Nc <= 0 || (K & 7)) return MNY_EINVAL;
    if (pwt_ok(M, K, Nc, MNY_ACT_NONE, false)) return pwt_parts(M);
    if (pw_thin_ok(1, 1, M, K, Nc)) return pw_thin_parts(M, K, Nc, 1);
    return nt2_plan(M, K, Nc, false, 1, kRedMaxTn).gx;
}
extern "C" int mny_pw_dgrad_bnred_bf16(const void* dy, const void* wT, void* dx, const void* y, const float* scale, const float* shift, int act,
                                       const float* mean, const float* invstd, float* red, int64_t M, int K, int Nc, void* stream) {
    return pw_dgrad_bnred_impl<1>(dy, wT, dx, y, scale, shift, act, mean, invstd, red, M, K, Nc, stream);
}

static bool lr_fix_wide(int64_t M, int K, int r_act) {
    return pw_wide_fix_ok(M, K) && r_act < MNY_ACT_HSWISH;
}
static int pw_lr_fix_impl(const float* x, const float* in_scale, const float* in_shift, const float* q, const float* r, const float* addend, float* dx,
                          const float* ry, const float* r_scale, const float* r_shift, int r_act, const float* r_mean, const float* r_invstd, float* red,
                          int64_t M, int K, void* stream) {
    MNY_REQUIRE(x && q && r && addend && dx && M > 0 && K > 0 && (K & 3) == 0 && (!in_scale) == (!in_shift), "pw_lr_fix: bad arguments (K=%d)", K);
    MNY_REQUIRE(!red || (ry && r_scale && r_shift && r_mean && r_invstd && r_act >= MNY_ACT_NONE && r_act <= MNY_ACT_HSIGMOID), "pw_lr_fix: incomplete reduction target");
    const bool xf = in_scale != nullptr;
    if (red && lr_fix_wide(M, K, r_act)) {
        g_pw_route = MNY_ROUTE_WIDE;
        return pw_wide_fix_launch(x, in_scale, in_shift, q, r, addend, dx, red, M, K, ry, r_scale, r_shift, r_mean, r_invstd, r_act, (hipStream_t)stream);
    }
    Nt2Plan p2 = nt2_plan(M, K, K, xf, 0, 3);
    MNY_REQUIRE(p2.lds <= 64 * 1024, "pw_lr_fix: K=%d too large", K);
    Gemm2Args g{x, in_scale, in_shift, MNY_ACT_NONE, q, r, addend, dx, red, M, K, K, p2.m_tiles, p2.tiles_per_block, p2.gx, p2.n_tiles,
                ry, r_scale, r_shift, r_mean, r_invstd, r_act};
    const bool x6 = nt_x6(M, K, K);
    Nt2Kernel k;
#define MNY_FX(T) (xf ? (x6 ? (Nt2Kernel)pw_gemm_nt_dma_kernel<T, 1, 0, 2, 1, 1> : (Nt2Kernel)pw_gemm_nt_dma_kernel<T, 1, 0, 2, 0, 1>) \
                      : (x6 ? (Nt2Kernel)pw_gemm_nt_dma_kernel<T, 0, 0, 2, 1, 1> : (Nt2Kernel)pw_gemm_nt_dma_kernel<T, 0, 0, 2, 0, 1>))
    if (red) switch (p2.TN) { case 1: k = MNY_FX(1); break; case 2: k = MNY_FX(2); break; default: k = MNY_FX(3); break; }
    else k = nt2_kernel(p2.TN, xf ? 1 : 0, 0, x6 ? 1 : 0);
#undef MNY_FX
    g_pw_route = x6 ? MNY_ROUTE_DMA_X6 : MNY_ROUTE_DMA_F32;
    hipLaunchKernelGGL(k, dim3(p2.grid), dim3(256), p2.lds, (hipStream_t)stream, g);
    return check_launch("pw_gemm_nt_dma_kernel<lr_fix>");
}
extern "C" int mny_pw_lr_fix_parts(int64_t M, int K, int r_act) {
    if (M <= 0 || K <= 0 || (K & 3)) return MNY_EINVAL;
    return lr_fix_wide(M, K, r_act) ? pw_wide_fix_parts(M, K) : nt2_plan(M, K, K, true, 0, 3).gx;
}
extern "C" int mny_pw_lr_fix(const float* x, const float* in_scale, const float* in_shift, const float* q, const float* r, const float* addend, float* dx,
                             const float* ry, const float* r_scale, const float* r_shift, int r_act, const float* r_mean, const float* r_invstd, float* red,
                             int64_t M, int K, void* stream) {
    return pw_lr_fix_impl(x, in_scale, in_shift, q, r, addend, dx, ry, r_scale, r_shift, r_act, r_mean, r_invstd, red, M, K, stream);
}

static bool w6_ok(int64_t M, int K, int Nc) {
    const bool off = sw(SW_NO_W6);
    constexpr double min_ai = 30.0;
    const double ai = 2.0 * K * Nc / (4.0 * (K + Nc));
    return !off && M > 0 && K > 0 && Nc > 0 && (K & 3) == 0 && !pw_thin_ok(0, 0, M, K, Nc) && !pw_wide_ok(M, K, Nc, false) && !pw_wide_ok(M, K, Nc, true) && nt_x6(M, K, Nc) != 0 && ai >= min_ai &&
           !sw(SW_GEMM_V1);
}
extern "C" int mny_pw_w6_supported(int64_t M, int K, int Nc) { return w6_ok(M, K, Nc) ? 1 : 0; }
extern "C" size_t mny_pw_w6_bytes(int K, int Nc) { return (K <= 0 || Nc <= 0) ? 0 : (size_t)3 * Nc * ((K + 15) / 16) * 32; }
extern "C" int mny_cut3_batch(const mny_cut3_job* jobs, const int32_t* block_job, int nblocks, void* stream) {
    MNY_REQUIRE(jobs && block_job && nblocks > 0, "cut3_batch: bad arguments");
    static_assert(sizeof(mny_cut3_job) == sizeof(Cut3Job), "job layout");
    hipLaunchKernelGGL(cut3_batch_kernel, dim3(nblocks), dim3(256), 0, (hipStream_t)stream, reinterpret_cast<const Cut3Job*>(jobs), block_job);
    return check_launch("cut3_batch_kernel");
}
extern "C" int mny_pw_fwd_w6(const float* x, const float* in_scale, const float* in_shift, int in_act, const void* w6, const float* bias,
                             const float* addend, float* y, float* stats, int64_t M, int K, int Nc, void* stream) {
    MNY_REQUIRE(x && w6 && y, "pw_fwd_w6: null pointer");
    MNY_REQUIRE(w6_ok(M, K, Nc), "pw_fwd_w6: unsupported problem M=%lld K=%d N=%d (mny_pw_w6_supported)", (long long)M, K, Nc);
// ... 395 lines not shown
```

### mobilenet-yolo-pytorch_amd/csrc/pwwide.hip

```cpp
#include <mutex>
#include <vector>

#include "common.h"
#include "x6.h"

namespace mny {

struct WideArgs {
    const float* A; const float* in_scale; const float* in_shift; int in_act;
    const float* W;
    float* C; float* stats;
    int64_t M; int K, N;
    int gx, n_blocks; int64_t ntiles;
    const float* rY; const float* r_scale; const float* r_shift; const float* r_mean; const float* r_invstd; int r_act;
    const float* addend;
    const float* bias;
};

template <int KS, int TNB, int XF, int MODE>
__global__ __launch_bounds__(256) __attribute__((amdgpu_waves_per_eu(2, 2))) void pw_wide_kernel(WideArgs p) {
    constexpr int BN = 32 * TNB;
    constexpr bool TWO_ACC = false;
    extern __shared__ __attribute__((aligned(16))) float smem[];
    float* sB = smem;
    float* sScale = sB + TNB * KS * 3 * 256;
    float* sShift = sScale + KS * 16;
    const int tid = threadIdx.x, lane = tid & 63;
    const int wave = __builtin_amdgcn_readfirstlane(tid >> 6);
    const int lrow = lane & 31, khalf = lane >> 5;
    const int bid = blockIdx.x, xcd = bid & 7, local = bid >> 3;
    const int y = local % p.n_blocks, x = (local / p.n_blocks) * 8 + xcd;
    if (x >= p.gx) return;
    const int n0 = y * BN;
    const int K = p.K, N = p.N;

    for (int c = tid; c < TNB * KS * 64; c += 256) {
        const int sidx = c >> 6, l = c & 63, j = l & 31, h = l >> 5;
        const int u = sidx / KS, s = sidx - u * KS;
        const int n = n0 + u * 32 + j;
        const int k0 = s * 16 + 4 * h, k1 = k0 + 8;
        const float* src = p.W + (int64_t)(n < N ? n : 0) * K;
        const float4 v0 = (n < N && k0 < K) ? ld4(src + k0) : f4zero();
        const float4 v1 = (n < N && k1 < K) ? ld4(src + k1) : f4zero();
        bf16x8_t hh, mm, ll;
        x6_split(v4f_t{v0.x, v0.y, v0.z, v0.w}, v4f_t{v1.x, v1.y, v1.z, v1.w}, hh, mm, ll);
        float* dst = sB + (sidx * 3) * 256 + l * 4;
        *reinterpret_cast<v4f_t*>(dst) = __builtin_bit_cast(v4f_t, hh);
        *reinterpret_cast<v4f_t*>(dst + 256) = __builtin_bit_cast(v4f_t, mm);
        *reinterpret_cast<v4f_t*>(dst + 512) = __builtin_bit_cast(v4f_t, ll);
    }
    if ((XF != 0 && MODE < 2) || MODE == 4) {
        const bool has = p.in_scale != nullptr;
        for (int k = tid; k < KS * 16; k += 256) {
            sScale[k] = k < K ? (has ? p.in_scale[k] : 1.f) : 0.f;
            sShift[k] = (k < K && has) ? p.in_shift[k] : 0.f;
        }
    }
    __syncthreads();

    const float slope = act_slope(p.in_act), hi = act_hi(p.in_act);
    const int quad = lrow >> 2, jq = lane & 3;
    const float rslope = act_slope(p.r_act), rhi = act_hi(p.r_act);
    const bool rhsig = p.r_act == MNY_ACT_HSIGMOID;
    float s1[TNB], s2[TNB];
#pragma unroll
    for (int u = 0; u < TNB; ++u) { s1[u] = 0.f; s2[u] = 0.f; }

    const float* bl = sB + lane * 4;
    const float* scl = sScale + 4 * khalf;
    const float* shl = sShift + 4 * khalf;
    const int64_t nslots = (int64_t)p.gx * 4;
    const unsigned rowb = (unsigned)N * 4u;
    float4 g[2 * KS];
    float ry[MODE >= 2 ? 16 : 1], ra[MODE >= 3 ? 16 : 1];
    auto load_g = [&](int64_t tile, int s) {
        const int64_t r = tile * 32 + lrow;
        const float* row = p.A + (r < p.M ? r : p.M - 1) * K;
        int k0 = 16 * s + 4 * khalf, k1 = k0 + 8;
        if (s == KS - 1) { k0 = k0 < K ? k0 : 0; k1 = k1 < K ? k1 : 0; }
        g[2 * s] = ld4(row + k0); g[2 * s + 1] = ld4(row + k1);
    };
    auto load_r = [&](int64_t tile, int u) {
        const int col = n0 + u * 32 + lrow, cc = col < N ? col : 0;
        unsigned voff = (unsigned)(4 * khalf) * rowb + (unsigned)cc * 4u;
        asm volatile("" : "+v"(voff));
        const float* ub = p.rY + tile * 32 * N;
#pragma unroll
        for (int r = 0; r < 16; ++r) ry[r] = ld1(at_bytes(ub + (int64_t)(8 * (r >> 2) + (r & 3)) * N, voff));
        if constexpr (MODE >= 3) {
            const float* ua = p.addend + tile * 32 * N;
#pragma unroll
            for (int r = 0; r < 16; ++r) ra[r] = ld1(at_bytes(ua + (int64_t)(8 * (r >> 2) + (r & 3)) * N, voff));
        }
    };

    auto do_tile = [&](const int64_t tile, const int64_t next) {
        const int64_t wrow = tile * 32;
        bf16x8_t ah[KS], am[KS], al[KS];
#pragma unroll
        for (int s = 0; s < KS; ++s) {
            const float4 a0 = g[2 * s], a1 = g[2 * s + 1];
            float z[8] = {a0.x, a0.y, a0.z, a0.w, a1.x, a1.y, a1.z, a1.w};
            if ((XF != 0 && MODE < 2) || MODE == 4) {
                v4f_t c0 = *reinterpret_cast<const v4f_t*>(scl + 16 * s), c1 = *reinterpret_cast<const v4f_t*>(scl + 16 * s + 8);
                v4f_t h0 = *reinterpret_cast<const v4f_t*>(shl + 16 * s), h1 = *reinterpret_cast<const v4f_t*>(shl + 16 * s + 8);
                asm volatile("s_waitcnt lgkmcnt(0)" : "+v"(c0), "+v"(c1), "+v"(h0), "+v"(h1));
                const float sv[8] = {c0.x, c0.y, c0.z, c0.w, c1.x, c1.y, c1.z, c1.w}, hv[8] = {h0.x, h0.y, h0.z, h0.w, h1.x, h1.y, h1.z, h1.w};
#pragma unroll
                for (int e = 0; e < 8; ++e) {
                    const float t = fmaf(z[e], sv[e], hv[e]);
                    z[e] = MODE == 4 ? t : (XF == 1 ? fminf(fmaxf(t, slope * t), hi) : t * fminf(fmaxf(t + 3.f, 0.f), 6.f) * (1.f / 6.f));
                }
            }
            x6_split(v4f_t{z[0], z[1], z[2], z[3]}, v4f_t{z[4], z[5], z[6], z[7]}, ah[s], am[s], al[s]);
            asm volatile("" : "+v"(ah[s]), "+v"(am[s]), "+v"(al[s]) :: "memory");
            load_g(next, s);
            __builtin_amdgcn_sched_barrier(0);
        }
        float* cbase = p.C + wrow * N;
#pragma unroll
        for (int u = 0; u < TNB; ++u) {
            float4 rc = f4zero();
            float cbias = 0.f;
            if (MODE >= 2) {
                const int colx = n0 + u * 32 + lrow;
                rc = make_float4(p.r_scale[colx], p.r_shift[colx], p.r_mean[colx], p.r_invstd[colx]);
                if (MODE == 4) cbias = p.bias[colx];
            }
            f32x16 acc, acc1;
#pragma unroll
            for (int r = 0; r < 16; ++r) { acc[r] = 0.f; acc1[r] = 0.f; }
#pragma unroll
            for (int s = 0; s < KS; ++s) {
                const float* bsrc = bl + ((u * KS + s) * 3) * 256;
                const bf16x8_t bh = __builtin_bit_cast(bf16x8_t, *reinterpret_cast<const v4f_t*>(bsrc));
                const bf16x8_t bm = __builtin_bit_cast(bf16x8_t, *reinterpret_cast<const v4f_t*>(bsrc + 256));
                const bf16x8_t bl_ = __builtin_bit_cast(bf16x8_t, *reinterpret_cast<const v4f_t*>(bsrc + 512));
                f32x16& a = (TWO_ACC && (s & 1)) ? acc1 : acc;
                a = __builtin_amdgcn_mfma_f32_32x32x16_bf16(al[s], bh, a, 0, 0, 0);
                a = __builtin_amdgcn_mfma_f32_32x32x16_bf16(ah[s], bl_, a, 0, 0, 0);
                a = __builtin_amdgcn_mfma_f32_32x32x16_bf16(am[s], bm, a, 0, 0, 0);
                a = __builtin_amdgcn_mfma_f32_32x32x16_bf16(am[s], bh, a, 0, 0, 0);
                a = __builtin_amdgcn_mfma_f32_32x32x16_bf16(ah[s], bm, a, 0, 0, 0);
                a = __builtin_amdgcn_mfma_f32_32x32x16_bf16(ah[s], bh, a, 0, 0, 0);
            }
            if (TWO_ACC) {
#pragma unroll
                for (int r = 0; r < 16; ++r) acc[r] += acc1[r];
            }
            if (MODE >= 2) {
#pragma unroll
                for (int r = 0; r < 16; ++r) {
                    const float zz = fmaf(ry[r], rc.x, rc.y);
                    float dact;
                    if (XF == 0) dact = (zz > 0.f ? 1.f : rslope) * (zz < rhi ? 1.f : 0.f);
                    else {
                        const float dsw = zz <= -3.f ? 0.f : (zz >= 3.f ? 1.f : (2.f * zz + 3.f) * (1.f / 6.f));
                        const float dsg = (zz > -3.f && zz < 3.f) ? (1.f / 6.f) : 0.f;
                        dact = rhsig ? dsg : dsw;
                    }
                    if (MODE >= 3) acc[r] += ra[r];
                    if (MODE == 4) acc[r] += cbias;
                    const float dz = acc[r] * dact;
                    s1[u] += dz; s2[u] = fmaf(dz, (ry[r] - rc.z) * rc.w, s2[u]);
                }
                asm volatile("" : "+v"(acc) :: "memory");
                if (u + 1 < TNB) load_r(tile, u + 1); else load_r(next, 0);
                __builtin_amdgcn_sched_barrier(0);
            } else if (MODE == 1) {
                v2f a1 = v2f{0.f, 0.f}, a2 = v2f{0.f, 0.f};
#pragma unroll
                for (int r = 0; r < 16; r += 2) {
                    const v2f q = v2f{acc[r], acc[r + 1]};
                    a1 += q;
                    a2 = __builtin_elementwise_fma(q, q, a2);
                }
                s1[u] += a1.x + a1.y; s2[u] += a2.x + a2.y;
            }
            unsigned off0 = (unsigned)(4 * khalf + jq) * rowb + (unsigned)(n0 + u * 32 + quad * 4) * 4u;
            asm volatile("" : "+v"(off0));
#pragma unroll
            for (int gq = 0; gq < 4; ++gq) {
                float r0 = acc[gq * 4 + 0], r1 = acc[gq * 4 + 1], r2 = acc[gq * 4 + 2], r3 = acc[gq * 4 + 3];
                {
                    const bool odd = lane & 1;
                    const float xa = odd ? r0 : r1, xb = odd ? r2 : r3;
                    const float ya = __builtin_bit_cast(float, __builtin_amdgcn_mov_dpp(__builtin_bit_cast(int, xa), 0xB1, 0xF, 0xF, true));
                    const float yb = __builtin_bit_cast(float, __builtin_amdgcn_mov_dpp(__builtin_bit_cast(int, xb), 0xB1, 0xF, 0xF, true));
                    if (odd) { r0 = ya; r2 = yb; } else { r1 = ya; r3 = yb; }
                }
                {
                    const bool hi2 = lane & 2;
                    const float xa = hi2 ? r0 : r2, xb = hi2 ? r1 : r3;
                    const float ya = __builtin_bit_cast(float, __builtin_amdgcn_mov_dpp(__builtin_bit_cast(int, xa), 0x4E, 0xF, 0xF, true));
                    const float yb = __builtin_bit_cast(float, __builtin_amdgcn_mov_dpp(__builtin_bit_cast(int, xb), 0x4E, 0xF, 0xF, true));
                    if (hi2) { r0 = ya; r1 = yb; } else { r2 = ya; r3 = yb; }
                }
                st4(at_bytes(cbase + (int64_t)(8 * gq) * N, off0), make_float4(r0, r1, r2, r3));
            }
            __builtin_amdgcn_sched_barrier(0);
        }
    };

    int64_t tile = (int64_t)x * 4 + wave;
    if (tile < p.ntiles) {
#pragma unroll
        for (int s = 0; s < KS; ++s) load_g(tile, s);
        if (MODE >= 2) load_r(tile, 0);
    }
    if (tile < p.ntiles) {
        do_tile(tile, tile + nslots < p.ntiles ? tile + nslots : tile);
        tile += nslots;
        for (; tile < p.ntiles; tile += nslots) do_tile(tile, tile + nslots < p.ntiles ? tile + nslots : tile);
    }

    if (MODE != 0) {
        __syncthreads();
        float* red = smem;
#pragma unroll
        for (int u = 0; u < TNB; ++u) {
            const float a = s1[u] + __shfl_xor(s1[u], 32);
            const float b = s2[u] + __shfl_xor(s2[u], 32);
            if (khalf == 0) {
                red[(wave * BN + u * 32 + lrow) * 2 + 0] = a;
                red[(wave * BN + u * 32 + lrow) * 2 + 1] = b;
            }
        }
        __syncthreads();
        if (tid < BN) {
            float a = 0.f, b = 0.f;
#pragma unroll
            for (int w = 0; w < 4; ++w) { a += red[(w * BN + tid) * 2]; b += red[(w * BN + tid) * 2 + 1]; }
            p.stats[(int64_t)x * 2 * N + n0 + tid] = a;
            p.stats[(int64_t)x * 2 * N + N + n0 + tid] = b;
        }
    }
}

struct WidePlan { int KS, TNB, n_blocks, gx, grid; int64_t ntiles; size_t lds; };

static bool wide_on() {
    return !sw(SW_NO_WIDE) && !sw(SW_GEMM_V1);
}

static int wide_tnb(int , int N, bool red) {
    const int cap = red ? 3 : 4;
    if (N % 96 == 0 && cap >= 3) return 3;
    if (N % 128 == 0 && cap >= 4) return 4;
    return N % 64 == 0 ? 2 : 0;
}

bool pw_wide_ok(int64_t M, int K, int N, bool red) {
    return wide_on() && M >= 8192 && K >= 52 && K <= 96 && (K & 3) == 0 && N >= 64 && wide_tnb(K, N, red) != 0 && N >= K;
}

static WidePlan wide_plan(int64_t M, int K, int N, bool red) {
    WidePlan pl;
    pl.KS = (K + 15) / 16;
    pl.TNB = wide_tnb(K, N, red);
    pl.n_blocks = N / (32 * pl.TNB);
    pl.ntiles = M / 32;
    constexpr int res = 512;
    int64_t gx = res / pl.n_blocks;
    if (gx >= 8) gx = gx / 8 * 8;
    if (gx < 1) gx = 1;
    const int64_t max_gx = cdiv(pl.ntiles, 4);
    if (gx > max_gx) gx = max_gx;
    pl.gx = (int)gx;
    pl.grid = (int)(cdiv(gx, 8) * 8) * pl.n_blocks;
    pl.lds = (size_t)(pl.TNB * pl.KS * 3 * 256 + 2 * pl.KS * 16) * sizeof(float);
    const size_t need = (size_t)4 * 32 * pl.TNB * 2 * sizeof(float);
    if (pl.lds < need) pl.lds = need;
    return pl;
}

int pw_wide_parts(int64_t M, int K, int N, bool red) { return wide_plan(M, K, N, red).gx; }

typedef void (*WideKernel)(WideArgs);
template <int KS, int TNB>
static WideKernel wide_pick_fwd(int xf, int mode) {
    switch (mode * 3 + xf) {
        case 0: return pw_wide_kernel<KS, TNB, 0, 0>; case 1: return pw_wide_kernel<KS, TNB, 1, 0>; case 2: return pw_wide_kernel<KS, TNB, 2, 0>;
        case 3: return pw_wide_kernel<KS, TNB, 0, 1>; case 4: return pw_wide_kernel<KS, TNB, 1, 1>; default: return pw_wide_kernel<KS, TNB, 2, 1>;
    }
}
template <int KS, int TNB>
static WideKernel wide_pick_red(int xf, int mode) {
    if (mode == 4) {
        if constexpr (KS == TNB * 2) return pw_wide_kernel<KS, TNB, 0, 4>;
        else return nullptr;
    }
    return mode == 2 ? pw_wide_kernel<KS, TNB, 0, 2> : pw_wide_kernel<KS, TNB, 0, 3>;
}
static WideKernel wide_pick(int KS, int TNB, int xf, int mode) {
    if (mode >= 2) switch (KS * 10 + TNB) {
        case 42: return wide_pick_red<4, 2>(xf, mode); case 43: return wide_pick_red<4, 3>(xf, mode);
        case 52: return wide_pick_red<5, 2>(xf, mode); case 53: return wide_pick_red<5, 3>(xf, mode);
        case 62: return wide_pick_red<6, 2>(xf, mode); default: return wide_pick_red<6, 3>(xf, mode);
    }
    switch (KS * 10 + TNB) {
        case 42: return wide_pick_fwd<4, 2>(xf, mode); case 43: return wide_pick_fwd<4, 3>(xf, mode); case 44: return wide_pick_fwd<4, 4>(xf, mode);
        case 52: return wide_pick_fwd<5, 2>(xf, mode); case 53: return wide_pick_fwd<5, 3>(xf, mode); case 54: return wide_pick_fwd<5, 4>(xf, mode);
        case 62: return wide_pick_fwd<6, 2>(xf, mode); case 63: return wide_pick_fwd<6, 3>(xf, mode); default: return wide_pick_fwd<6, 4>(xf, mode);
    }
}

bool pw_wide_fix_ok(int64_t M, int K) { return pw_wide_ok(M, K, K, true) && (M & 31) == 0 && (K == 64 || K == 96); }
int pw_wide_fix_parts(int64_t M, int K) { return wide_plan(M, K, K, true).gx; }
int pw_wide_fix_launch(const float* A, const float* in_scale, const float* in_shift, const float* Q, const float* bias, const float* addend, float* C,
                       float* stats, int64_t M, int K, const float* rY, const float* r_scale, const float* r_shift, const float* r_mean,
                       const float* r_invstd, int r_act, hipStream_t st) {
    MNY_REQUIRE(pw_wide_fix_ok(M, K) && rY && addend && bias && stats && r_act < MNY_ACT_HSWISH, "pw_wide_fix: unsupported problem M=%lld K=%d", (long long)M, K);
    const WidePlan pl = wide_plan(M, K, K, true);
    WideArgs a{A, in_scale, in_shift, MNY_ACT_NONE, Q, C, stats, M, K, K, pl.gx, pl.n_blocks, pl.ntiles, rY, r_scale, r_shift, r_mean, r_invstd, r_act, addend, bias};
    const WideKernel k = wide_pick(pl.KS, pl.TNB, 0, 4);
    MNY_REQUIRE(k != nullptr, "pw_wide_fix: no kernel for K=%d", K);
    if (!allow_lds((const void*)k, 80 * 1024)) {
        set_error("pw_wide: hipFuncSetAttribute failed"); return MNY_EHIP;
    }
    hipLaunchKernelGGL(k, dim3(pl.grid), dim3(256), pl.lds, st, a);
    return check_launch("pw_wide_kernel<fix>");
}

int pw_wide_launch(const float* A, const float* in_scale, const float* in_shift, int in_act, const float* W, float* C, float* stats,
                   int64_t M, int K, int N, const float* rY, const float* r_scale, const float* r_shift, const float* r_mean,
                   const float* r_invstd, int r_act, const float* addend, hipStream_t st) {
    MNY_REQUIRE(pw_wide_ok(M, K, N, rY != nullptr) && (M & 31) == 0, "pw_wide: unsupported problem M=%lld K=%d N=%d (whole 32-row tiles: callers send the last M %% 32 rows elsewhere)", (long long)M, K, N);
    const WidePlan pl = wide_plan(M, K, N, rY != nullptr);
    MNY_REQUIRE(pl.KS >= 4 && pl.KS <= 6 && pl.TNB >= 2 && pl.TNB <= 4, "pw_wide: no kernel for K=%d, column block %d", K, 32 * pl.TNB);
    const bool xf = in_scale != nullptr || in_act != MNY_ACT_NONE;
    const int mode = rY ? (addend ? 3 : 2) : (stats ? 1 : 0);
    const int XF = rY ? (r_act >= MNY_ACT_HSWISH ? 2 : 0) : (!xf ? 0 : (in_act == MNY_ACT_HSWISH ? 2 : 1));
    MNY_REQUIRE(!(rY && xf), "pw_wide: the reduction form takes its A operand as is");
    MNY_REQUIRE(!rY || r_act < MNY_ACT_HSWISH, "pw_wide: the reduction form knows the clamp family only (mny_pw_dgrad_bnred_supported)");
    MNY_REQUIRE(rY || !addend, "pw_wide: a plain addend is not supported (callers route it to the LDS-DMA kernel)");
    MNY_REQUIRE(in_act != MNY_ACT_HSIGMOID, "pw_wide: h-sigmoid input transform is not supported");
    WideArgs a{A, in_scale, in_shift, in_act, W, C, stats, M, K, N, pl.gx, pl.n_blocks, pl.ntiles, rY, r_scale, r_shift, r_mean, r_invstd, r_act, addend, nullptr};
    const WideKernel k = wide_pick(pl.KS, pl.TNB, XF, mode);
    if (!allow_lds((const void*)k, 80 * 1024)) {
        set_error("pw_wide: hipFuncSetAttribute failed"); return MNY_EHIP;
    }
    hipLaunchKernelGGL(k, dim3(pl.grid), dim3(256), pl.lds, st, a);
    return check_launch("pw_wide_kernel");
}

}
```

### mobilenet-yolo-pytorch_amd/engine.py

```python
import ctypes
import itertools
import os
import re
import warnings

import numpy as np
import torch

from . import _lib, switches
from ._lib import ACT_NONE, MnyError, YoloHead

_FWD_TICK = itertools.count()

BN_EPS = 1e-5
BN_MOMENTUM = 0.1
_vp = ctypes.c_void_p


def _ptr(t):
    return _vp(t.data_ptr()) if t is not None else None


class CallList:

# ... 79 lines not shown
            path = "libamdhip64.so"
            try:
                tlib = os.path.join(os.path.dirname(os.path.abspath(torch.__file__)), "lib")
                cands = []
                with open("/proc/self/maps") as f:
                    for line in f:
                        if "libamdhip64.so" in line:
                            cands.append(line.split()[-1])
                mine = [c for c in cands if os.path.dirname(os.path.abspath(c)) == tlib]
                uniq = sorted(set(cands))
                if mine:
                    path = mine[0]
                elif len(uniq) == 1:
                    path = uniq[0]
                elif uniq:
                    raise OSError("several HIP runtimes mapped (%s), none of them torch's" % ", ".join(uniq))
            except OSError as e:
                warnings.warn("raw HIP events unavailable (%s); timing brackets use torch.cuda.Event" % (e,))
                cls._hip = False
                raise MnyError("no unambiguous HIP runtime")
            cls._hip = ctypes.CDLL(path)
            cls._hip.hipEventCreate.argtypes = [ctypes.POINTER(ctypes.c_void_p)]
            cls._hip.hipEventRecord.argtypes = [ctypes.c_void_p, ctypes.c_void_p]
            cls._hip.hipEventElapsedTime.argtypes = [ctypes.POINTER(ctypes.c_float), ctypes.c_void_p, ctypes.c_void_p]
        return cls._hip

    def __init__(self):
        h = ctypes.c_void_p()
        if self._rt().hipEventCreate(ctypes.byref(h)) != 0:
            raise MnyError("hipEventCreate failed")
        self.h = h

    @classmethod
    def _new(cls):
        if cls._hip is not False:
            try:
                ev = cls()
                if not cls._checked:
                    ev2 = cls()
                    st = _vp(torch.cuda.current_stream().cuda_stream)
                    ev.record(st); ev2.record(st)
                    torch.cuda.current_stream().synchronize()
                    ev.elapsed_time(ev2)
                    cls._checked = True
                return ev
            except (OSError, AttributeError, MnyError, RuntimeError) as e:
                warnings.warn("raw HIP events unavailable (%s); timing brackets fall back to torch.cuda.Event" % (e,))
                cls._hip = False
        return _TorchEvent()

    @classmethod
    def reserve(cls, n):
        cls._next = 0
        while len(cls._pool) < n:
            cls._pool.append(cls._new())

    @classmethod
    def take(cls):
        if cls._next == len(cls._pool):
            cls._pool.append(cls._new())
        cls._next += 1
        return cls._pool[cls._next - 1]

    def record(self, stream):
        if self._hip.hipEventRecord(self.h, stream) != 0:
            raise MnyError("hipEventRecord failed")

    def elapsed_time(self, other):
        ms = ctypes.c_float()
        if self._hip.hipEventElapsedTime(ctypes.byref(ms), self.h, other.h) != 0:
            raise MnyError("hipEventElapsedTime failed (events not complete?)")
        return float(ms.value)


class _Unit:
    __slots__ = ("Y", "coef4", "scale", "shift", "mean", "invstd", "act", "C", "M", "shape")


class _Grad:
    __slots__ = ("buf", "shared")

    def __init__(self):
        self.buf, self.shared = None, False


_NO_VIEW = (None, None, None, ACT_NONE)
_HARD = (_lib.ACT_HSWISH, _lib.ACT_HSIGMOID)


class NetPlan:
    def __init__(self, net, N, H, W, training, act_dtype=torch.float32, bn_batch=None, frozen_bwd=False):
        self.net, self.N, self.H, self.W, self.training = net, N, H, W, training
        bn_batch = training if bn_batch is None else bool(bn_batch)
        self.bn_batch = bn_batch
        self.frozen = bool(training and not bn_batch and frozen_bwd)
        self.fwd_gen = 0
        self.inflight_gen = None
        self.last_fwd_tick = -1
        self.resident_bytes = 0
        dev = net.device
        self.dev = dev
        assert act_dtype in (torch.float32, torch.bfloat16), act_dtype
        sw_hipgraph, sw_side, sw_exdw_k, sw_no_gate = (switches.get(n) for n in ("MNY_HIPGRAPH", "MNY_SIDE_STREAM", "MNY_EXDW_K", "MNY_NO_GATE"))
        self.sw_no_lr, self.sw_no_lr_s2, self.sw_no_dwfuse5s2 = (switches.get(n) for n in ("MNY_NO_LR", "MNY_NO_LR_S2", "MNY_NO_DWFUSE5S2"))
        self.adt = act_dtype
        self.bf16 = act_dtype == torch.bfloat16
        self.eb = 2 if self.bf16 else 4
        assert H % 32 == 0 and W % 32 == 0, "input height/width must be multiples of 32 (got %dx%d)" % (H, W)
        g = net.graph
        self.stream = _vp(0)
        self.x_ptr = _vp(0)
        self.timing = None
        self.routes = {"fwd": {}, "bwd": {}}
        self._recorded = set()
        self.reducer = None
        self.use_graphs = training and sw_hipgraph
        auto_side = N * H * W <= 48 * 1000 * 1000
        self.side_on = training and not self.use_graphs and (sw_side == 1 or (sw_side is None and auto_side))
        self.stream_side = _vp(0)
        self._side_stream = torch.cuda.Stream(dev) if self.side_on else None
        self._ev_fork = torch.cuda.Event() if self.side_on else None
        self._ev_join = torch.cuda.Event() if self.side_on else None
        self.stream_side2 = _vp(0)
        self._side2_stream = torch.cuda.Stream(dev) if self.side_on else None
        self._ev_fork2 = torch.cuda.Event() if self.side_on else None
        self._ev_join2 = torch.cuda.Event() if self.side_on else None
        self._side_used = False
        self.graphs = {}
        self.eager_steps = 0
        self.x_static = None
        self.fwd = CallList()
        self.bwd = None
        self._cvt_jobs = []
        self._cut_jobs = []
        self.wT, self.wT6 = {}, {}
        self._loss_side = False
        self._head0_call = None
        self.head32 = {}
        self.units = {}
        self.reals = {}
        self._f32 = dict(device=dev, dtype=torch.float32)
        self._act = dict(device=dev, dtype=self.adt)
        self._P = net.param_tensors
        self.max_parts = _lib.query("mny_max_parts")
        self.maxC = max(v.C for v in g.values)
        self.stats_ws = torch.empty(self.max_parts * 2 * self.maxC, **self._f32)
        self.param_ptrs = [(t, t.data_ptr()) for t in net.all_state_tensors()]
        self._analyse_graph(g)
        self._match_exdw(g, sw_exdw_k)
        self._match_gates(g, sw_no_gate)
        self.dead_side = bool(self.side_on and bn_batch
                              and any(nd.out.id not in self.live and nd.op in ("dw", "pw", "add") for nd in g.nodes))
        self.stats_ws_side = torch.empty(self.max_parts * 2 * self.maxC, **self._f32) if self.dead_side else self.stats_ws
        dead_forked = self._build_forward(g)
        self._flush_cvt_jobs()
        self._flush_cut_jobs(self.fwd, at_head=True)
        self._flush_gate_jobs()
        self.heads = [self.head32.get(o.id, self.reals[o.id]) for o in g.outputs]
        self.seg_head = self.head32.get(g.seg_out.id, self.reals[g.seg_out.id]) if g.seg_out is not None else None
        self._build_detection()
        if dead_forked or self._loss_side:
            self.fwd.add_py(self._join_side, "join")
        if training and (bn_batch or self.frozen):
            self._build_backward(g)

    def _shape(self, v):
        return (self.N, self.H // v.down, self.W // v.down, v.C)

    def _rows(self, v):
        shp = self._shape(v)
        return shp[0] * shp[1] * shp[2]

    def _view(self, v):
        if v.kind == "unit":
            u = self.units[v.id]
            assert u.Y is not None, "%s is the un-materialised expand output of an exdw unit" % v.name
            return (u.Y, u.scale, u.shift, v.act)
        return (self.reals[v.id], None, None, ACT_NONE)

    def _analyse_graph(self, g):
        self.loss_outputs = list(g.outputs) + ([g.seg_out] if g.seg_out is not None else [])
        self.out_ids = {v.id for v in self.loss_outputs}
        self.consumers = {}
        for nd in g.nodes:
            for v in nd.ins:
                self.consumers.setdefault(v.id, []).append(nd)
        self.n_consumers = {v.id: len(self.consumers.get(v.id, ())) for v in g.values}
        for v in self.loss_outputs:
            self.n_consumers[v.id] += 1
        self.live = set()
        stack = list(self.loss_outputs)
        while stack:
            v = stack.pop()
            if v.node is None or v.id in self.live:
                continue
            self.live.add(v.id)
            stack.extend(v.node.ins)
        self.bwd_order = [nd for nd in reversed(g.nodes) if nd.out.id in self.live]
        self.last_consumer = {}
        for nd in self.bwd_order:
            for v in nd.ins:
                self.last_consumer[v.id] = nd

    def _match_exdw(self, g, sw_exdw_k):
        self.exdw_pw, self.exdw_dw = {}, {}
        if self.bf16 or self.frozen:
            return
        ks = set(int(v) for v in sw_exdw_k.split(",") if v)
        for nd in g.nodes:
            if nd.op != "pw" or nd.out.id in self.out_ids or len(self.consumers.get(nd.out.id, ())) != 1:
                continue
            d = self.consumers[nd.out.id][0]
            i = nd.ins[0]
            ish = self._shape(i)
            if (d.op == "dw" and d.k == 3 and d.stride == 2 and nd.out.act == _lib.ACT_RELU6 and d.out.act == _lib.ACT_RELU6 and not nd.bias
                    and i.act in (ACT_NONE, _lib.ACT_RELU6, _lib.ACT_LEAKY, _lib.ACT_RELU) and i.C in ks
                    and _lib.query("mny_exdw_supported", self.N, ish[1], ish[2], i.C, nd.out.C, 2) == 1):
                self.exdw_pw[nd.out.id] = d
                self.exdw_dw[d.out.id] = nd

    def _match_gates(self, g, sw_no_gate):
        self.gates, self.gate_units, self.gate_absorbed = {}, {}, set()
        if not self.bf16 or self.frozen or sw_no_gate:
            return
        cons, out_ids = self.consumers, self.out_ids
        for nd in g.nodes:
            if nd.op != "mul":
                continue
            tv_, sv = nd.ins
            se3 = sv.node
            se0 = se3.ins[0].node if (se3 is not None and se3.op == "pw") else None
            if (se0 is None or se0.op != "pw" or se0.ins[0] is not tv_ or tv_.kind != "unit" or tv_.act != ACT_NONE or sv.act != _lib.ACT_HSIGMOID
                    or se0.out.act != _lib.ACT_RELU or se0.bias or se3.bias or len(cons.get(se0.out.id, ())) != 1 or len(cons.get(sv.id, ())) != 1
                    or len(cons.get(tv_.id, ())) != 2 or tv_.id in out_ids or se0.out.id in out_ids or sv.id in out_ids or nd.out.id in out_ids):
                continue
            tsh = self._shape(tv_)
            if _lib.query("mny_gate_supported", tsh[0] * tsh[1] * tsh[2], tv_.C, se0.out.C) != 1:
                continue
            gate = dict(t=tv_, se0=se0, se3=se3, mul=nd, add=None,
                        wq=torch.empty(int(_lib.query("mny_gate_wq_bytes", tv_.C, se0.out.C)), device=self.dev, dtype=torch.uint8))
            emit_at = nd
            mc = cons.get(nd.out.id, [])
            if len(mc) == 1 and mc[0].op == "add" and mc[0].k == 1 and mc[0].ins[0] is nd.out:
                gate["add"] = mc[0]
                emit_at = mc[0]
                self.gate_absorbed.add(nd.out.id)
            self.gates[emit_at.out.id] = gate
            self.gate_units[se0.out.id] = gate
            self.gate_units[se3.out.id] = gate

    def _build_forward(self, g):
        dead_forked = False
        for nd in g.nodes:
            o = nd.out
            dead = (self.dead_side and o.id not in self.live and nd.op in ("dw", "pw", "add")
                    and o.id not in self.exdw_pw and o.id not in self.exdw_dw)
            st = self.stream_side if dead else self.stream
            sws = self.stats_ws_side if dead else self.stats_ws
            if dead and not dead_forked:
                self.fwd.add_py(self._fork_side, "fork")
                dead_forked = True
            if nd.op == "pw" and o.id in self.gate_units:
                self._new_unit(o, materialise=False)
            elif o.id in self.gate_absorbed:
                pass
            elif o.id in self.gates:
                self._emit_gate_forward(self.gates[o.id], nd)
            elif nd.op in self._FWD:
                self._FWD[nd.op](self, nd, st, sws)
            else:
                raise AssertionError(nd.op)
        return dead_forked

    def _new_unit(self, o, materialise=True):
        shp = self._shape(o)
        u = _Unit()
        u.Y = torch.empty(shp, **self._act) if materialise else None
        u.coef4 = torch.empty(4, o.C, **self._f32)
        u.scale, u.shift, u.mean, u.invstd = u.coef4[0], u.coef4[1], u.coef4[2], u.coef4[3]
        u.act, u.C, u.M, u.shape = o.act, o.C, shp[0] * shp[1] * shp[2], shp
        self.units[o.id] = u
        return u

    def _new_real(self, o):
        t = torch.empty(self._shape(o), **self._act)
        self.reals[o.id] = t
        return t

    def _emit_bn_tail(self, bn, u, parts, M, sws, st):
        P = self._P
        gam, bet, rm, rv = P[bn + ".weight"], P[bn + ".bias"], P[bn + ".running_mean"], P[bn + ".running_var"]
        if self.bn_batch:
            self.fwd.add("mny_bn_finalize", sws, parts, M, gam, bet, BN_EPS, BN_MOMENTUM, rm, rv, u.scale, u.shift, u.mean, u.invstd, u.C, st)
        else:
            self.fwd.add("mny_bn_eval_coeffs", gam, bet, rm, rv, BN_EPS, u.scale, u.shift, u.C, self.stream)
            if self.frozen:
                self.fwd.add("mny_bn_eval_stats", rm, rv, BN_EPS, u.mean, u.invstd, u.C, self.stream)

    def _emit_pw_gemm(self, calls, x, wop, w6, bias, addend, out, stats, M, K, Nc, st, tag=""):
        calls.add("mny_pw_fwd_w6" if w6 else self.K("mny_pw_fwd"), x[0], x[1], x[2], x[3], wop, bias, addend, out, stats, M, K, Nc, st,
                  label=self.K("mny_pw_fwd"),
                  meta=dict(flops=2 * M * K * Nc, bytes=self.eb * (M * K + M * Nc) + 4 * K * Nc, shape="%sM%d K%d N%d" % (tag, M, K, Nc)))

    def _fwd_weight(self, w, M, K, Nc):
        w6 = self._w6_planes(w, M, K, Nc)
        return (w6, True) if w6 is not None else (self._gemm_weight(w), False)

    def _fwd_unit(self, nd, st, sws):
        o = nd.out
        u = self._new_unit(o, materialise=o.id not in self.exdw_pw)
        stats = sws if self.bn_batch else None
        if nd.op == "stem":
            conv = self._fwd_stem
        elif nd.op == "dw":
            conv = self._fwd_exdw_dw if o.id in self.exdw_dw else self._fwd_dw
        else:
            conv = self._fwd_exdw_pw if o.id in self.exdw_pw else self._fwd_pw
        parts = conv(nd, u, self._P[nd.conv + ".weight"], stats, st)
        self._emit_bn_tail(nd.bn, u, parts, u.M, sws, st)

    def _fwd_stem(self, nd, u, w, stats, st):
        N, H, W, C = self.N, self.H, self.W, u.C
        self.fwd.add(self.K("mny_stem_fwd"), self.x_ptr, w, u.Y, stats, N, H, W, C, self.stream,
                     meta=dict(flops=2 * u.M * C * 27, bytes=4 * N * 3 * H * W + self.eb * u.M * C))
        return _lib.query("mny_stem_stat_parts", N, H, W, C)

    def _fwd_exdw_dw(self, nd, u, w, stats, st):
        pn = self.exdw_dw[nd.out.id]
        pi, pu = pn.ins[0], self.units[pn.out.id]
        psh = self._shape(pi)
        xv = self._view(pi)
        N, M, C = self.N, u.M, u.C
        Mx = N * psh[1] * psh[2]
        self.fwd.add("mny_exdw_fwd", xv[0], xv[1], xv[2], xv[3], self._P[pn.conv + ".weight"], pu.scale, pu.shift, w, u.Y, stats,
                     N, psh[1], psh[2], pi.C, C, 2, self.stream,
                     meta=dict(flops=2 * Mx * pi.C * C + 2 * M * C * 9, bytes=self.eb * (Mx * pi.C + M * C), shape="exdw K%d C%d H%d" % (pi.C, C, psh[1])))
        return _lib.query("mny_exdw_fwd_parts", N, psh[1], psh[2], pi.C, C, 2)

    def _fwd_dw(self, nd, u, w, stats, st):
        i = nd.ins[0]
        ish = self._shape(i)
        xv = self._view(i)
        N, M, C = self.N, u.M, u.C
        self.fwd.add(self.K("mny_dw_fwd"), xv[0], xv[1], xv[2], xv[3], w, u.Y, stats, N, ish[1], ish[2], C, nd.k, nd.stride, st,
                     meta=dict(flops=2 * M * C * nd.k * nd.k, bytes=self.eb * (N * ish[1] * ish[2] * C + M * C) + 4 * C * nd.k * nd.k,
                               shape="C%d H%d s%d" % (C, ish[1], nd.stride)))
        return _lib.query("mny_dw_stat_parts_x", N, ish[1], ish[2], C, nd.k, nd.stride, 1 if self.bf16 else 0)

    def _fwd_exdw_pw(self, nd, u, w, stats, st):
        i = nd.ins[0]
        xv = self._view(i)
        M, C = u.M, u.C
        if self.bn_batch:
            self.fwd.add("mny_exdw_stats", xv[0], xv[1], xv[2], xv[3], w, stats, M, i.C, C, self.stream,
                         meta=dict(flops=2 * M * i.C * (i.C + 1), bytes=self.eb * M * i.C,
                                   shape="exdw stats M%d K%d N%d" % (M, i.C, C)))
        return _lib.query("mny_exdw_stat_parts", M, i.C, C)

    def _fwd_pw(self, nd, u, w, stats, st):
        i = nd.ins[0]
        wop, w6 = self._fwd_weight(w, u.M, i.C, u.C)
        self._emit_pw_gemm(self.fwd, self._view(i), wop, w6, None, None, u.Y, stats, u.M, i.C, u.C, st)
        return _lib.query(self.K("mny_pw_stat_parts"), u.M, i.C, u.C)

    def _fwd_head(self, nd, st, sws):
        o, i = nd.out, nd.ins[0]
        t = self._new_real(o)
        M = t.numel() // o.C
        wop, w6 = self._fwd_weight(self._P[nd.conv + ".weight"], M, i.C, o.C)
        self._emit_pw_gemm(self.fwd, self._view(i), wop, w6, self._P[nd.conv + ".bias"], None, t, None, M, i.C, o.C, st)
        if self.bf16:
            t32 = torch.empty(t.shape, **self._f32)
            self.fwd.add("mny_cvt_bf16_f32", t, t32, t.numel(), st)
            self.head32[o.id] = t32
        g = self.net.graph
        if g.outputs and o is g.outputs[0]:
            self._head0_call = self.fwd.calls[-1]

    def _fwd_add(self, nd, st, sws):
        a = self._view(nd.ins[0])
        has_b, has_up = nd.k & 1, nd.k & 2
        b = self._view(nd.ins[1]) if has_b else _NO_VIEW
        up = self.reals[nd.ins[-1].id] if has_up else None
        if has_up:
            assert nd.ins[-1].kind == "real"
        t = self._new_real(nd.out)
        self.fwd.add(self.K("mny_add_views"), a[0], a[1], a[2], a[3], b[0], b[1], b[2], b[3], up, t, *t.shape, st)

    def _fwd_mul(self, nd, st, sws):
        a, b = self._view(nd.ins[0]), self._view(nd.ins[1])
        t = self._new_real(nd.out)
        self.fwd.add(self.K("mny_mul_views"), a[0], a[1], a[2], a[3], b[0], b[1], b[2], b[3], t, t.numel() // nd.out.C, nd.out.C, self.stream)

    def _fwd_partadd(self, nd, st, sws):
        a = self._view(nd.ins[0])
        up = self.reals[nd.ins[1].id]
        t = self._new_real(nd.out)
        self.fwd.add(self.K("mny_partadd_up"), a[0], a[1], a[2], a[3], up, t, t.shape[0], t.shape[1], t.shape[2], nd.ins[0].C, nd.out.C, st)

    _FWD = {"stem": _fwd_unit, "dw": _fwd_unit, "pw": _fwd_unit, "pwb": _fwd_head, "add": _fwd_add, "mul": _fwd_mul, "partadd": _fwd_partadd}

    def _emit_gate_forward(self, gate, nd):
        t, se0, se3 = gate["t"], gate["se0"], gate["se3"]
        u1, u2 = self.units[se0.out.id], self.units[se3.out.id]
        tsh = self._shape(t)
        M, C, R = tsh[0] * tsh[1] * tsh[2], t.C, se0.out.C
        tv = self._view(t)
        wq = gate["wq"]
        out = self._new_real(nd.out)
        parts = _lib.query("mny_gate_parts", M)
        eb = self.eb
        for un, hn in ((u1, se0), (u2, se3)):
            if self.bn_batch and hn is se0:
                self.fwd.add("mny_gate_stats1_bf16", tv[0], tv[1], tv[2], wq, self.stats_ws, M, C, R, self.stream,
                             meta=dict(flops=2 * M * C * R, bytes=eb * M * C, shape="gate stats1 M%d C%d R%d" % (M, C, R)))
            elif self.bn_batch:
                self.fwd.add("mny_gate_stats2_bf16", tv[0], tv[1], tv[2], wq, u1.scale, u1.shift, self.stats_ws, M, C, R, self.stream,
                             meta=dict(flops=4 * M * C * R, bytes=eb * M * C, shape="gate stats2 M%d C%d R%d" % (M, C, R)))
            self._emit_bn_tail(hn.bn, un, parts, M, self.stats_ws, self.stream)
        a = _NO_VIEW
        if gate["add"] is not None:
            a = self._view(gate["add"].ins[1])
        self.fwd.add("mny_gate_fwd_bf16", tv[0], tv[1], tv[2], wq, u1.scale, u1.shift, u2.scale, u2.shift, a[0], a[1], a[2], a[3], out,
                     M, C, R, self.stream,
                     meta=dict(flops=4 * M * C * R, bytes=eb * M * C * (3 if a[0] is not None else 2), shape="gate M%d C%d R%d%s" % (M, C, R, " +add" if a[0] is not None else "")))

    def _flush_gate_jobs(self):
        if not self.gates:
            return
        P, gl = self._P, list(self.gates.values())
        rows = [(P[gt["se0"].conv + ".weight"].data_ptr(), P[gt["se3"].conv + ".weight"].data_ptr(), gt["wq"].data_ptr(), gt["t"].C, gt["se0"].out.C) for gt in gl]
        self.gate_jobs, _ = self._job_table(rows, [("w1", np.uint64), ("w2", np.uint64), ("wq", np.uint64), ("C", np.int32), ("R", np.int32)])
        self.fwd.add("mny_gate_cut_batch_bf16", self.gate_jobs, len(gl), self.stream)
        self.fwd.calls.insert(0, self.fwd.calls.pop())

    def _build_detection(self):
        net, dev, N = self.net, self.dev, self.N
        f32 = dict(device=dev, dtype=torch.float32)
        self.hp, self.anchors, self.masks = [], [], []
        img = [self.H, self.W]
        for hi, hs in enumerate(net.yolo_losses):
            g = self.heads[hi].shape[1]
            assert self.heads[hi].shape[1] == self.heads[hi].shape[2], "square grids only (yolo_loss.py:71)"
            hs.img_size = img
            anchors = torch.tensor([(aw / img[0], ah / img[1]) for aw, ah in hs.anchors], dtype=torch.float32).to(dev)
            self.anchors.append(anchors)
            self.masks.append(torch.tensor(hs.mask, dtype=torch.int32).to(dev))
            self.hp.append(YoloHead(N, g, len(hs.mask), hs.num_classes, len(hs.anchors), hs.ignore_threshold, hs.iou_thresh, hs.iou_weighting))
        if self.training:
            self.out14 = torch.zeros(2, 7, **f32)
            self.dheads = [torch.empty_like(h) for h in self.heads]
            self.t_ptr, self.off_ptr = _vp(0), _vp(0)
            self.loss_ws = []
            for hi in range(2):
                nbytes = _lib.query("mny_yolo_loss_ws_bytes", ctypes.byref(self.hp[hi]), 0)
                ws = torch.empty(nbytes, device=dev, dtype=torch.uint8)
                self.loss_ws.append(ws)
                pos = next((k + 1 for k, c in enumerate(self.fwd.calls) if c is self._head0_call), None)
                early = (hi == 0 and self.side_on and self.bn_batch and pos is not None and pos < len(self.fwd.calls))
                self.fwd.add("mny_yolo_loss", self.heads[hi], self.t_ptr, self.off_ptr, self.anchors[hi], self.masks[hi],
                             ctypes.byref(self.hp[hi]), self.out14[hi], self.dheads[hi], ws, self.stream_side if early else self.stream)
                if early:
                    loss_call = self.fwd.calls.pop()
                    self.fwd.add_py(self._fork_side, "fork")
                    fork_call = self.fwd.calls.pop()
                    self.fwd.calls[pos:pos] = [fork_call, loss_call]
                    self._loss_side = True
            self.t_dev = torch.zeros(max(4 * N, 64), 5, **f32)
            self.off_dev = torch.zeros(N + 1, device=dev, dtype=torch.int32)
            if self.seg_head is not None:
                self.seg_out3 = torch.zeros(3, **f32)
                self.seg_maps = torch.zeros_like(self.seg_head)
                self.dheads.append(torch.empty_like(self.seg_head))
                self.seg_ws = torch.empty(max(_lib.query("mny_seg_loss_ws_bytes", self.seg_head.numel()), 8), device=dev, dtype=torch.uint8)
                self.fwd.add("mny_seg_loss", self.seg_head, self.seg_maps, self.seg_head.numel(), self.seg_out3, self.dheads[2], self.seg_ws, self.stream)
        else:
            C = net.num_classes
            self.cells = [hp.A * hp.g * hp.g for hp in self.hp]
            self.cap = sum(self.cells)
            self.rows = torch.zeros(N, self.cap, 7, **f32)
            self.cnt0 = torch.zeros(N, device=dev, dtype=torch.int32)
            self.cnt1 = torch.zeros(N, device=dev, dtype=torch.int32)
            self.seg_begin = (torch.arange(N, dtype=torch.int32) * self.cap).to(dev)
            self.out_idx = torch.zeros(N * self.cap, device=dev, dtype=torch.int32)
            self.out_counts = torch.zeros(N, device=dev, dtype=torch.int32)
            self.out_rows = torch.zeros(N * self.cap, 7, **f32)
            self.nms_ws = torch.empty(_lib.query("mny_nms_ws_bytes", N, N * self.cap, C), device=dev, dtype=torch.uint8)
            self.val_conf = [ctypes.c_float(0.1), ctypes.c_float(0.1)]
            self.det = CallList()
            self.det.add("mny_yolo_decode", self.heads[0], self.anchors[0], self.masks[0], ctypes.byref(self.hp[0]), self.val_conf[0],
                         self.rows, self.cap, None, self.cnt0, self.stream)
            self.det.add("mny_yolo_decode", self.heads[1], self.anchors[1], self.masks[1], ctypes.byref(self.hp[1]), self.val_conf[1],
                         self.rows, self.cap, self.cnt0, self.cnt1, self.stream)
            self.det.add("mny_nms_per_class", self.rows, self.seg_begin, self.cnt1, N, N * self.cap, self.cap, C, ctypes.c_double(0.45),
                         self.out_idx, self.out_counts, self.out_rows, self.nms_ws, self.stream)
            so = _lib.query("mny_nms_status_offset", N, N * self.cap, C)
            self.nms_status = self.nms_ws[so:so + 4].view(torch.int32)
            if self.seg_head is not None:
                _, sh, sw, sc = self.seg_head.shape
                self.seg_eval = torch.zeros(sc, sh, sw, **f32)
                self.det.add("mny_seg_sigmoid", self.seg_head, sh, sw, sc, self.seg_eval, self.stream)


    def _build_backward(self, g):
        bwd = self.bwd = CallList()
        order = self.bwd_order
        self._plan_grad_arena(order)
        self._written = set()
        self.shared_tmp = []
        self._red_jobs, self._red_keep, self._post_reduce = [], [], []
        self._uses = {}
        for nd in order:
            if nd.conv:
# ... 830 lines not shown
```

### mobilenet-yolo-pytorch_amd/ops.py

```python
import ctypes

import torch

from . import _lib
from ._lib import ACT_NONE, YoloHead, call, query

BN_EPS = 1e-5
BN_MOMENTUM = 0.1


def _p(t):
    if t is None:
        return None
    assert t.is_cuda and t.dtype in (torch.float32, torch.int32, torch.bfloat16) and t.is_contiguous(), \
        "libmnyolo needs contiguous fp32/bf16/int32 device tensors (got %s %s)" % (t.device, t.dtype)
    return ctypes.c_void_p(t.data_ptr())


def _st():
    return ctypes.c_void_p(torch.cuda.current_stream().cuda_stream)


def _new(*shape, like=None, dtype=torch.float32):
    return torch.empty(shape, device=like.device, dtype=dtype)
# ... 16 lines not shown
def stem_wgrad(x_nchw, dy):
    N, _, H, W = x_nchw.shape
    Co = dy.shape[3]
    parts = query("mny_stem_wgrad_parts", N, H, W, Co)
    ws = _new(parts, Co * 27, like=dy)
    dw = _new(Co, 3, 3, 3, like=dy)
    call(_k("mny_stem_wgrad", dy), _p(x_nchw), _p(dy), _p(dw), _p(ws), N, H, W, Co, _st())
    return dw


def stem_bnwgrad(x_nchw, g, y, scale, shift, act, gamma, mean, invstd):
    N, _, H, W = x_nchw.shape
    Co = y.shape[3]
    M = y.numel() // Co
    parts = query("mny_bn_bwd_parts", M, Co)
    red = _new(parts, 2, Co, like=gamma)
    call(_k("mny_bn_bwd_reduce", y), _p(g), _p(y), _p(scale), _p(shift), act, _p(mean), _p(invstd), _p(red), M, Co, _st())
    dgamma, dbeta, coef = _new(Co, like=gamma), _new(Co, like=gamma), _new(3, Co, like=gamma)
    call("mny_bn_bwd_finalize", _p(red), parts, M, _p(gamma), _p(mean), _p(invstd), _p(dgamma), _p(dbeta), _p(coef), Co, _st())
    ws = _new(query("mny_stem_wgrad_parts", N, H, W, Co), Co * 27, like=gamma)
    dw = _new(Co, 3, 3, 3, like=gamma)
    call(_k("mny_stem_bnwgrad", y), _p(x_nchw), _p(g), _p(y), _p(scale), _p(shift), act, _p(coef), _p(dw), _p(ws), N, H, W, Co, _st())
    return dw, dgamma, dbeta


def dw_fwd(view, w, stride, want_stats=True):
    x, sc, sh, act = view
    N, H, W, C = x.shape
    K = w.shape[-1]
    Ho, Wo = (H + 2 * (K // 2) - K) // stride + 1, (W + 2 * (K // 2) - K) // stride + 1
    y = _new(N, Ho, Wo, C, like=x, dtype=x.dtype)
    stats = _new(query("mny_dw_stat_parts_x", N, H, W, C, K, stride, 1 if x.dtype == torch.bfloat16 else 0), 2, C, like=x) if want_stats else None
    call(_k("mny_dw_fwd", x), _p(x), _p(sc), _p(sh), act, _p(w), _p(y), _p(stats), N, H, W, C, K, stride, _st())
    return y, stats


def dw_bwd_data(dy, w, in_hw, stride, addend=None, out=None):
    N, _, _, C = dy.shape
    H, W = in_hw
    K = w.shape[-1]
    dx = out if out is not None else _new(N, H, W, C, like=dy, dtype=dy.dtype)
    call(_k("mny_dw_bwd_data", dy), _p(dy), _p(w), _p(addend), _p(dx), N, H, W, C, K, stride, _st())
    return dx


def dw_bwd_weight(view, dy, K, stride):
    x, sc, sh, act = view
    N, H, W, C = x.shape
    ws = _new(query("mny_dw_wgrad_parts", N, H, W, C, K, stride), C * K * K, like=x)
    dw = _new(C, 1, K, K, like=x)
    call(_k("mny_dw_bwd_weight", x), _p(x), _p(sc), _p(sh), act, _p(dy), _p(dw), _p(ws), N, H, W, C, K, stride, _st())
    return dw


def dw_bnbwd(g, y, scale, shift, act, coef, xview, w, addend=None, in_stats=None):
    x, xs, xh, xact = xview
    N, H, W, C = x.shape
    k = w.shape[-1]
    parts = query("mny_dw_bnbwd_parts_k", N, H, W, C, k, (1 if x.dtype == torch.bfloat16 else 0) | (2 if in_stats is not None else 0))
    ws = _new(parts, C * k * k, like=x)
    dx = torch.empty_like(x)
    dw = _new(C, 1, k, k, like=x)
    if in_stats is None:
        call(_k("mny_dw_bnbwd", x), _p(g), _p(y), _p(scale), _p(shift), act, _p(coef), _p(x), _p(xs), _p(xh), xact, _p(w), _p(addend), _p(dx),
             _p(dw), _p(ws), N, H, W, C, k, 1, _st())
        return dx, dw
    red = _new(parts, 2, C, like=x)
    call(_k("mny_dw_bnbwd_red", x), _p(g), _p(y), _p(scale), _p(shift), act, _p(coef), _p(x), _p(xs), _p(xh), xact, _p(in_stats[0]), _p(in_stats[1]),
         _p(w), _p(addend), _p(dx), _p(dw), _p(ws), _p(red), N, H, W, C, k, 1, _st())
    return dx, dw, red


def dw_bnbwd_s2(g, y, scale, shift, act, coef, xview, w, addend=None):
    x, xs, xh, xact = xview
    N, H, W, C = x.shape
    ws = _new(query("mny_dw_bnbwd_s2_parts", N, H, W, C), C * 9, like=x)
    dx = torch.empty_like(x)
    dw = _new(C, 1, 3, 3, like=x)
    call(_k("mny_dw_bnbwd_s2", x), _p(g), _p(y), _p(scale), _p(shift), act, _p(coef), _p(x), _p(xs), _p(xh), xact, _p(w), _p(addend), _p(dx),
         _p(dw), _p(ws), N, H, W, C, _st())
    return dx, dw


def dw_bnbwd_s2k5(g, y, scale, shift, act, coef, xview, w, addend=None, in_stats=None):
    x, xs, xh, xact = xview
    N, H, W, C = x.shape
    parts = query("mny_dw_bnbwd_s2k5_parts", N, H, W, C)
    ws = _new(parts, C * 25, like=w)
    dx = torch.empty_like(x)
    dw = _new(C, 1, 5, 5, like=w)
    red = _new(parts, 2, C, like=w) if in_stats is not None else None
    mu, istd = in_stats if in_stats is not None else (None, None)
    call(_k("mny_dw_bnbwd_s2k5", x), _p(g), _p(y), _p(scale), _p(shift), act, _p(coef), _p(x), _p(xs), _p(xh), xact, _p(mu), _p(istd), _p(w), _p(addend),
         _p(dx), _p(dw), _p(ws), _p(red), N, H, W, C, _st())
    return (dx, dw) if red is None else (dx, dw, red)


def pw_fwd(view, w2d, bias=None, addend=None, want_stats=True, out=None):
    x, sc, sh, act = view
    assert w2d.dtype == x.dtype, "pw_fwd: weight dtype %s must match the activation storage type %s" % (w2d.dtype, x.dtype)
    K = x.shape[-1]
    M = x.numel() // K
    Nc = w2d.shape[0]
    y = out if out is not None else _new(*x.shape[:-1], Nc, like=x, dtype=x.dtype)
    stats = _new(query(_k("mny_pw_stat_parts", x), M, K, Nc), 2, Nc, like=x) if want_stats else None
    call(_k("mny_pw_fwd", x), _p(x), _p(sc), _p(sh), act, _p(w2d), _p(bias), _p(addend), _p(y), _p(stats), M, K, Nc, _st())
    return y, stats


def pw_wgrad(view, dy, want_dbias=False):
    x, sc, sh, act = view
    K = x.shape[-1]
    M = x.numel() // K
    Nc = dy.shape[-1]
    ws = _new(query("mny_pw_wgrad_ws_floats", M, K, Nc), like=x)
    dw = _new(Nc, K, like=x)
    db = _new(Nc, like=x) if want_dbias else None
    call(_k("mny_pw_wgrad", x), _p(x), _p(sc), _p(sh), act, _p(dy), _p(dw), _p(db), _p(ws), M, K, Nc, _st())
    return dw, db


def pw_bnbwd(g, y, scale, shift, act, mean, invstd, gamma, xview, w2d, addend=None, want_dx=True):
    x, xs, xh, xact = xview
    K, Nc = x.shape[-1], y.shape[-1]
    M = y.numel() // Nc
    assert query(_k("mny_pw_bnbwd_supported", y), M, K, Nc) == 1
    ws = _new(query("mny_pw_bnbwd_ws_floats", M, K, Nc), like=y, dtype=torch.float32)
    dx = torch.empty_like(x) if want_dx else None
    dw, dgamma, dbeta = _new(Nc, K, like=y, dtype=torch.float32), _new(Nc, like=y, dtype=torch.float32), _new(Nc, like=y, dtype=torch.float32)
    call(_k("mny_pw_bnbwd", y), _p(g), _p(y), _p(scale), _p(shift), act, _p(mean), _p(invstd), _p(gamma), _p(x), _p(xs), _p(xh), xact,
         _p(w2d), _p(addend), _p(dx), _p(dw), _p(dgamma), _p(dbeta), _p(ws), M, K, Nc, _st())
    return dx, dw, dgamma, dbeta


def pw_dgrad_bnred(dy, wT, y_unit, scale, shift, act, mean, invstd, addend=None):
    M, K = dy.numel() // dy.shape[-1], dy.shape[-1]
    Nc = wT.shape[0]
    parts = query("mny_pw_dgrad_bnred_parts", M, K, Nc)
    dx = torch.empty(*dy.shape[:-1], Nc, device=dy.device, dtype=torch.float32)
    red = torch.empty(parts, 2, Nc, device=dy.device, dtype=torch.float32)
    if addend is None:
        call("mny_pw_dgrad_bnred", _p(dy), _p(wT), _p(dx), _p(y_unit), _p(scale), _p(shift), int(act), _p(mean), _p(invstd), _p(red), M, K, Nc, _st())
    else:
        call("mny_pw_dgrad_bnred_add", _p(dy), _p(wT), _p(addend), _p(dx), _p(y_unit), _p(scale), _p(shift), int(act), _p(mean), _p(invstd), _p(red),
             M, K, Nc, _st())
    return dx, red


def transpose(w2d, dtype=torch.float32):
    R, C = w2d.shape
    out = _new(C, R, like=w2d, dtype=dtype)
    call(_k("mny_transpose", out), _p(w2d), _p(out), R, C, _st())
    return out


def bn_finalize(stats, count, gamma, beta, running_mean=None, running_var=None):
    C = gamma.numel()
    scale, shift, mean, invstd = (_new(C, like=gamma) for _ in range(4))
    call("mny_bn_finalize", _p(stats), stats.shape[0], count, _p(gamma), _p(beta), BN_EPS, BN_MOMENTUM,
         _p(running_mean), _p(running_var), _p(scale), _p(shift), _p(mean), _p(invstd), C, _st())
    return scale, shift, mean, invstd


def bn_eval_coeffs(gamma, beta, rm, rv):
    C = gamma.numel()
    scale, shift = _new(C, like=gamma), _new(C, like=gamma)
    call("mny_bn_eval_coeffs", _p(gamma), _p(beta), _p(rm), _p(rv), BN_EPS, _p(scale), _p(shift), C, _st())
    return scale, shift


def bn_backward(g, y, scale, shift, act, gamma, mean, invstd, out=None):
    C = y.shape[-1]
    M = y.numel() // C
    parts = query("mny_bn_bwd_parts", M, C)
    red = _new(parts, 2, C, like=y)
    call(_k("mny_bn_bwd_reduce", y), _p(g), _p(y), _p(scale), _p(shift), act, _p(mean), _p(invstd), _p(red), M, C, _st())
    dgamma, dbeta, coef = _new(C, like=y), _new(C, like=y), _new(3, C, like=y)
    call("mny_bn_bwd_finalize", _p(red), parts, M, _p(gamma), _p(mean), _p(invstd), _p(dgamma), _p(dbeta), _p(coef), C, _st())
    dy = out if out is not None else torch.empty_like(y)
    call(_k("mny_bn_bwd_apply", y), _p(g), _p(y), _p(scale), _p(shift), act, _p(coef), _p(dy), M, C, _st())
    return dy, dgamma, dbeta


def add_views(a, b=None, up=None, out=None):
    x = a[0]
    N, H, W, C = x.shape
    o = out if out is not None else torch.empty_like(x)
    bt, bsc, bsh, bact = b if b is not None else (None, None, None, ACT_NONE)
    call(_k("mny_add_views", x), _p(a[0]), _p(a[1]), _p(a[2]), a[3], _p(bt), _p(bsc), _p(bsh), bact, _p(up), _p(o), N, H, W, C, _st())
    return o


def upsample_bwd(src, dst=None, accumulate=False):
    N, H, W, C = src.shape
    d = dst if dst is not None else _new(N, H // 2, W // 2, C, like=src, dtype=src.dtype)
    call(_k("mny_upsample_bwd", src), _p(src), _p(d), int(accumulate), N, H, W, C, _st())
    return d


def axpy(src, dst, alpha=None, accumulate=False):
    call(_k("mny_axpy", src), _p(src), _p(alpha), _p(dst), int(accumulate), src.numel(), _st())
    return dst


def make_head(N, g, A, C, n_anchors_all, ignore_thresh, iou_thresh, iou_weighting):
    return YoloHead(N, g, A, C, n_anchors_all, ignore_thresh, iou_thresh, iou_weighting)


def yolo_loss(head, targets, t_off, anchors_all, mask, hp, ws=None):
    nbytes = query("mny_yolo_loss_ws_bytes", ctypes.byref(hp), 0)
    if ws is None:
        ws = torch.empty(nbytes, device=head.device, dtype=torch.uint8)
    assert ws.dtype == torch.uint8 and ws.is_contiguous() and ws.numel() >= nbytes, "yolo_loss: workspace too small"
    out7 = _new(7, like=head)
    dhead = torch.empty_like(head)
    call("mny_yolo_loss", _p(head), _p(targets), _p(t_off), _p(anchors_all), _p(mask), ctypes.byref(hp),
         _p(out7), _p(dhead), ctypes.c_void_p(ws.data_ptr()), _st())
    return out7, dhead


def yolo_decode(head, anchors_all, mask, hp, val_conf, rows=None, row_stride=None, base_counts=None):
    cells = hp.A * hp.g * hp.g
    row_stride = row_stride or cells
    if rows is None:
        rows = _new(hp.N, row_stride, 7, like=head)
    counts = _new(hp.N, like=head, dtype=torch.int32)
    call("mny_yolo_decode", _p(head), _p(anchors_all), _p(mask), ctypes.byref(hp), float(val_conf), _p(rows), int(row_stride),
         _p(base_counts), _p(counts), _st())
    return rows, counts


def nms_per_class(rows, seg_begin, seg_count, num_classes, thr=0.45, max_seg_rows=0, gather=True):
    capacity = rows.shape[0]
    S = seg_begin.numel()
    nbytes = query("mny_nms_ws_bytes", S, capacity, num_classes)
    ws = torch.empty(nbytes, device=seg_begin.device, dtype=torch.uint8)
    out_idx = torch.empty(max(capacity, 1), device=seg_begin.device, dtype=torch.int32)
    out_counts = torch.empty(S, device=seg_begin.device, dtype=torch.int32)
    out_rows = torch.empty(max(capacity, 1), 7, device=seg_begin.device) if gather else None
    call("mny_nms_per_class", _p(rows) if capacity else None, _p(seg_begin), _p(seg_count), S, capacity, int(max_seg_rows), num_classes,
         float(thr), _p(out_idx), _p(out_counts), _p(out_rows), ctypes.c_void_p(ws.data_ptr()), _st())
    so = query("mny_nms_status_offset", S, capacity, num_classes)
    po = query("mny_nms_prefix_offset", S, capacity, num_classes)
    status = ws[so:so + 4].view(torch.int32)
    prefix = ws[po:po + 4 * (S + 1)].view(torch.int32)
    return out_idx, out_counts, out_rows, prefix, status
```

### mobilenet-yolo-pytorch_amd/switches.py

```python
import os
import warnings

FLAG, INT, WORD, TEXT = "flag", "int", "word", "text"

TABLE = (
    ("MNY_LIB", TEXT, None, "loader", "path of another libmnyolo.so build to load (A/B on one machine)"),
    ("MNY_HIPGRAPH", FLAG, 0, "plan", "replay training plans through captured hipGraphs"),
    ("MNY_SIDE_STREAM", INT, None, "plan", "weight gradients on a side stream: 0 / 1, unset = up to 48 M input pixels"),
    ("MNY_NO_GATE", FLAG, 0, "plan", "per-pixel gates as separate convs, BatchNorms and a multiply, not fused units"),
    ("MNY_EXDW_K", TEXT, "16,24", "plan", "input widths whose expand + depthwise pairs run as one unit"),
    ("MNY_NO_LR", FLAG, 0, "plan lib", "no low-rank BatchNorm backward of the wide expand units (lrbwd.hip)"),
    ("MNY_NO_LR_S2", FLAG, 0, "plan", "no low-rank BatchNorm backward behind the stride-2 depthwise units"),
    ("MNY_NO_DWFUSE5S2", FLAG, 0, "plan", "5x5 stride-2 depthwise units on the generic backward kernels"),
    ("MNY_GEMM_V1", FLAG, 0, "lib", "pointwise forward / data gradients on the first-generation tile kernels"),
    ("MNY_WGRAD_V1", FLAG, 0, "lib", "pointwise weight gradients on the first-generation tile kernel"),
    ("MNY_WGRAD_NO_XCD", FLAG, 0, "lib", "weight-gradient workgroups in plain order, not grouped per XCD"),
    ("MNY_X6", INT, -1, "lib", "six-product bf16 GEMM: 0 = never (fp32 MFMA), 1 = wherever supported, -1 = per-shape rule"),
    ("MNY_NO_W6", FLAG, 0, "lib", "no pre-cut weight operand for the six-product GEMM"),
    ("MNY_NO_WIDE", FLAG, 0, "lib", "no barrier-free short-reduction kernel (pwwide.hip)"),
    ("MNY_NO_WGS", FLAG, 0, "lib", "no stream weight-gradient kernel (pwwgs.hip)"),
    ("MNY_NO_THIN", FLAG, 0, "lib", "no vector-ALU kernel for K = 8..32 (pwthin.hip)"),
    ("MNY_NO_PWT", FLAG, 0, "lib", "no wave-per-16-pixels thin pointwise kernel (gate.hip)"),
    ("MNY_NO_PWE", FLAG, 0, "lib", "no wave form of the thin expand unit backward (gate.hip)"),
    ("MNY_NO_PJBWD", FLAG, 0, "lib", "no fused projection backward (pjbwd.hip, gate.hip)"),
    ("MNY_NO_EXDW", FLAG, 0, "lib", "no fused expand + depthwise unit: the materialised path"),
    ("MNY_EXDW_STATS", WORD, 0, "lib", "gram (default) | direct: how mny_exdw_stats forms its sums"),
    ("MNY_NO_STEMDW", FLAG, 0, "lib", "no fused stem + depthwise backward (stemdw.hip)"),
    ("MNY_STEM_WGRAD_VALU", FLAG, 0, "lib", "stem weight gradient on the vector ALU, not the matrix cores"),
    ("MNY_DW_V1", FLAG, 0, "lib", "3x3 depthwise forward on the first-generation sliding-window kernel"),
    ("MNY_NO_DWT5", FLAG, 0, "lib", "no tile form of the 5x5 depthwise unit backward"),
    ("MNY_DWT3", INT, -1, "lib", "tile form of the 3x3 depthwise unit backward: 0 / 1, -1 = per-shape rule"),
    ("MNY_DWTF", INT, -1, "lib", "tile form of the depthwise forward: 0 / 1, -1 = per-shape rule"),
    ("MNY_NMS_SMALL", FLAG, 0, "lib", "NMS buckets of any size through the one-workgroup path"),
    ("MNY_FORCE_DP", FLAG, 0, "bench", "bench.py: run the RCCL data-parallel path even with one rank"),
    ("MNY_LAUNCHER_PARENT_CLEAN", FLAG, 0, "bench", "bench.py: set by its launcher for the rank processes it starts"),
    ("MNY_PRINT_MARKS", FLAG, 0, "bench", "bench.py: print the backward call list's marks"),
)
_ROWS = {row[0]: row for row in TABLE}


def get(name):
    _, kind, default, _, _ = _ROWS[name]
    raw = os.environ.get(name)
    if kind == FLAG:
        return raw not in (None, "", "0")
    if raw in (None, ""):
        return default
    return int(raw) if kind == INT else raw


def warn_unknown():
    for name in sorted(os.environ):
        if name.startswith("MNY_") and name not in _ROWS:
            warnings.warn("%s is set but is not a switch of this build (retired or misspelled?): it has no effect — see switches.py" % name,
                          RuntimeWarning, stacklevel=3)
```

Before: 7128 images/s.

## Fuse BatchNorm finalize into pointwise forward GEMM via last-block ticket tail

Adds a finalize tail to the wide pointwise forward kernel. Each workgroup takes an atomic ticket after writing its partial statistics, and the last one to arrive reduces them and writes the BN scale, shift, mean, invstd and running stats. The engine uses this for supported fp32 batch-stat shapes and skips the separate bn_finalize launch, which saves a kernel launch and a dependency gap per layer. The cost is serialized tail work in one workgroup, device-scope fences, and a ticket buffer that must reset correctly. The existing finalize kernels are refactored onto a shared header.

```diff
diff --git a/include/mnyolo.h b/include/mnyolo.h
--- a/include/mnyolo.h
+++ b/include/mnyolo.h
@@ -234,6 +234,24 @@
 };
 int mny_pw_route(int op, int bf16, int64_t M, int K, int Nc);
 int mny_pw_last_route(void);
+
+#define MNY_FIN_MAX_GROUPS 64
+typedef struct mny_bn_fin {
+    const float* gamma;
+    const float* beta;
+    float* running_mean;
+    float* running_var;
+    float* scale;
+    float* shift;
+    float* mean;
+    float* invstd;
+    int32_t* tickets;
+    double count;
+    float eps, momentum;
+} mny_bn_fin;
+int mny_pw_fwd_fin_supported(int64_t M, int K, int Nc);
+int mny_pw_fwd_fin(const float* x, const float* in_scale, const float* in_shift, int in_act, const float* w, float* y, float* stats,
+                   int64_t M, int K, int Nc, const mny_bn_fin* fin, void* stream);
 
 size_t mny_map_ws_bytes(int64_t D, int64_t T);
 int mny_map_eval(const float* det_boxes , const float* det_labels, const float* det_scores,
diff --git a/mobilenet-yolo-pytorch_amd/_lib.py b/mobilenet-yolo-pytorch_amd/_lib.py
--- a/mobilenet-yolo-pytorch_amd/_lib.py
+++ b/mobilenet-yolo-pytorch_amd/_lib.py
@@ -13,6 +13,15 @@
 
 class MnyError(RuntimeError):
     pass
+
+
+FIN_MAX_GROUPS = 64
+
+
+class BnFin(ctypes.Structure):
+    _fields_ = [("gamma", ctypes.c_void_p), ("beta", ctypes.c_void_p), ("running_mean", ctypes.c_void_p), ("running_var", ctypes.c_void_p),
+                ("scale", ctypes.c_void_p), ("shift", ctypes.c_void_p), ("mean", ctypes.c_void_p), ("invstd", ctypes.c_void_p),
+                ("tickets", ctypes.c_void_p), ("count", ctypes.c_double), ("eps", c_float), ("momentum", c_float)]
 
 
 class YoloHead(ctypes.Structure):
@@ -78,6 +87,8 @@
     "mny_pw_dgrad_bnred_add": (c_int, [P, P, P, P, P, P, P, c_int, P, P, P, c_int64, c_int, c_int, P]),
     "mny_pw_route": (c_int, [c_int, c_int, c_int64, c_int, c_int]),
     "mny_pw_last_route": (c_int, []),
+    "mny_pw_fwd_fin_supported": (c_int, [c_int64, c_int, c_int]),
+    "mny_pw_fwd_fin": (c_int, [P, P, P, c_int, P, P, P, c_int64, c_int, c_int, P, P]),
     "mny_pw_w6_supported": (c_int, [c_int64, c_int, c_int]),
     "mny_pw_w6_bytes": (c_size_t, [c_int, c_int]),
     "mny_cut3_batch": (c_int, [P, P, c_int, P]),
diff --git a/mobilenet-yolo-pytorch_amd/build.py b/mobilenet-yolo-pytorch_amd/build.py
--- a/mobilenet-yolo-pytorch_amd/build.py
+++ b/mobilenet-yolo-pytorch_amd/build.py
@@ -27,7 +27,7 @@
 
 def build(force=False, verbose=False):
     os.makedirs(OBJ, exist_ok=True)
-    headers = [os.path.join(CSRC, "common.h"), os.path.join(CSRC, "x6.h"), os.path.join(HERE, "..", "include", "mnyolo.h")]
+    headers = [os.path.join(CSRC, "common.h"), os.path.join(CSRC, "x6.h"), os.path.join(CSRC, "bn_finalize.h"), os.path.join(HERE, "..", "include", "mnyolo.h")]
     jobs, objs = [], []
     for src in sources():
         s = os.path.join(CSRC, src)
diff --git a/mobilenet-yolo-pytorch_amd/csrc/bn_eltwise.hip b/mobilenet-yolo-pytorch_amd/csrc/bn_eltwise.hip
--- a/mobilenet-yolo-pytorch_amd/csrc/bn_eltwise.hip
+++ b/mobilenet-yolo-pytorch_amd/csrc/bn_eltwise.hip
@@ -1,72 +1,16 @@
 #include "common.h"
+#include "bn_finalize.h"
 
 namespace mny {
-
-__device__ __forceinline__ void sum_partial_rows(const float* __restrict__ rows, int parts, int C, int c, int slice, double& s, double& q) {
-    double s1 = 0.0, q1 = 0.0, s2 = 0.0, q2 = 0.0, s3 = 0.0, q3 = 0.0;
-    s = 0.0; q = 0.0;
-    int p = slice;
-    const int64_t step = (int64_t)64 * C;
-    const float* a = rows + (int64_t)p * 2 * C + c;
-    for (; p + 480 < parts; p += 512, a += 16 * step) {
-        float v[16], u[16];
-#pragma unroll
-        for (int i = 0; i < 16; ++i) { v[i] = a[i * step]; u[i] = a[i * step + C]; }
-#pragma unroll
-        for (int i = 0; i < 16; i += 4) {
-            s += (double)v[i];      q += (double)u[i];
-            s1 += (double)v[i + 1]; q1 += (double)u[i + 1];
-            s2 += (double)v[i + 2]; q2 += (double)u[i + 2];
-            s3 += (double)v[i + 3]; q3 += (double)u[i + 3];
-        }
-    }
-    for (; p + 96 < parts; p += 128, a += 4 * step) {
-        const float v0 = a[0], u0 = a[C], v1 = a[step], u1 = a[step + C], v2 = a[2 * step], u2 = a[2 * step + C], v3 = a[3 * step], u3 = a[3 * step + C];
-        s += (double)v0;  q += (double)u0;
-        s1 += (double)v1; q1 += (double)u1;
-        s2 += (double)v2; q2 += (double)u2;
-        s3 += (double)v3; q3 += (double)u3;
-    }
-    for (; p < parts; p += 32, a += step) {
-        s += (double)a[0];
-        q += (double)a[C];
-    }
-    s = (s + s1) + (s2 + s3);
-    q = (q + q1) + (q2 + q3);
-}
 
 __global__ __launch_bounds__(1024) void bn_finalize_kernel(const float* __restrict__ stats, int parts, double count,
                                                           const float* __restrict__ gamma, const float* __restrict__ beta,
                                                           float eps, float momentum, float* running_mean, float* running_var,
                                                           float* scale, float* shift, float* mean_out, float* invstd_out, int C) {
-    __shared__ double red[2][32][32];
-    const int cl = threadIdx.x & 31, slice = threadIdx.x >> 5;
-    const int c = blockIdx.x * 32 + cl;
-    double s = 0.0, q = 0.0;
-    if (c < C) {
-        sum_partial_rows(stats, parts, C, c, slice, s, q);
-    }
-    red[0][slice][cl] = s;
-    red[1][slice][cl] = q;
-    __syncthreads();
-    if (slice == 0 && c < C) {
-        s = 0.0; q = 0.0;
-        for (int i = 0; i < 32; ++i) { s += red[0][i][cl]; q += red[1][i][cl]; }
-        const double mean = s / count;
-        double var = q / count - mean * mean;
-        if (var < 0.0) var = 0.0;
-        const float invstd = (float)(1.0 / sqrt(var + (double)eps));
-        const float sc = gamma[c] * invstd;
-        scale[c] = sc;
-        shift[c] = beta[c] - (float)mean * sc;
-        if (mean_out) mean_out[c] = (float)mean;
-        if (invstd_out) invstd_out[c] = invstd;
-        if (running_mean) {
-            const double unbiased = count > 1.0 ? var * count / (count - 1.0) : var;
-            running_mean[c] = (1.f - momentum) * running_mean[c] + momentum * (float)mean;
-            running_var[c] = (1.f - momentum) * running_var[c] + momentum * (float)unbiased;
-        }
-    }
+    __shared__ double red[2 * 32 * 32];
+    const int c0 = blockIdx.x * 32;
+    const BnFwdOut o{count, gamma, beta, eps, momentum, running_mean, running_var, scale, shift, mean_out, invstd_out};
+    bn_finalize_channels<false, 1024>(stats, parts, C, c0, min(c0 + 32, C), o, 1, red, threadIdx.x);
 }
 
 __global__ void bn_eval_coeffs_kernel(const float* gamma, const float* beta, const float* rm, const float* rv, float eps,
@@ -133,27 +77,10 @@
                                                               const float* __restrict__ gamma, const float* __restrict__ mean,
                                                               const float* __restrict__ invstd, float* dgamma, float* dbeta,
                                                               float* coef, int C) {
-    __shared__ double red[2][32][32];
-    const int cl = threadIdx.x & 31, slice = threadIdx.x >> 5;
-    const int c = blockIdx.x * 32 + cl;
-    double s = 0.0, q = 0.0;
-    if (c < C) {
-        sum_partial_rows(red_in, parts, C, c, slice, s, q);
-    }
-    red[0][slice][cl] = s;
-    red[1][slice][cl] = q;
-    __syncthreads();
-    if (slice == 0 && c < C) {
-        s = 0.0; q = 0.0;
-        for (int i = 0; i < 32; ++i) { s += red[0][i][cl]; q += red[1][i][cl]; }
-        dbeta[c] = (float)s;
-        dgamma[c] = (float)q;
-        const double a = (double)gamma[c] * (double)invstd[c];
-        const double b = -a * (double)invstd[c] * q / count;
-        coef[c] = (float)a;
-        coef[C + c] = (float)b;
-        coef[2 * C + c] = (float)(-a * s / count - b * (double)mean[c]);
-    }
+    __shared__ double red[2 * 32 * 32];
+    const int c0 = blockIdx.x * 32;
+    const BnBwdOut o{count, gamma, mean, invstd, dgamma, dbeta, coef};
+    bn_bwd_finalize_channels<false, 1024>(red_in, parts, C, c0, min(c0 + 32, C), o, 1, red, threadIdx.x);
 }
 
 template <typename T>
diff --git a/mobilenet-yolo-pytorch_amd/csrc/bn_finalize.h b/mobilenet-yolo-pytorch_amd/csrc/bn_finalize.h
--- /dev/null
+++ b/mobilenet-yolo-pytorch_amd/csrc/bn_finalize.h
@@ -0,0 +1,150 @@
+#pragma once
+#include "common.h"
+
+namespace mny {
+
+typedef ::mny_bn_fin BnFin;
+
+template <bool DEV>
+__device__ __forceinline__ float fin_ld(const float* p) {
+    if constexpr (DEV) return __hip_atomic_load(p, __ATOMIC_RELAXED, __HIP_MEMORY_SCOPE_AGENT);
+    else return *p;
+}
+
+template <bool DEV>
+__device__ __forceinline__ void sum_partial_rows(const float* __restrict__ rows, int parts, int C, int c, int slice, double& s, double& q) {
+    double s1 = 0.0, q1 = 0.0, s2 = 0.0, q2 = 0.0, s3 = 0.0, q3 = 0.0;
+    s = 0.0; q = 0.0;
+    int p = slice;
+    const int64_t step = (int64_t)64 * C;
+    const float* a = rows + (int64_t)p * 2 * C + c;
+    for (; p + 480 < parts; p += 512, a += 16 * step) {
+        float v[16], u[16];
+#pragma unroll
+        for (int i = 0; i < 16; ++i) { v[i] = fin_ld<DEV>(a + i * step); u[i] = fin_ld<DEV>(a + i * step + C); }
+#pragma unroll
+        for (int i = 0; i < 16; i += 4) {
+            s += (double)v[i];      q += (double)u[i];
+            s1 += (double)v[i + 1]; q1 += (double)u[i + 1];
+            s2 += (double)v[i + 2]; q2 += (double)u[i + 2];
+            s3 += (double)v[i + 3]; q3 += (double)u[i + 3];
+        }
+    }
+    for (; p + 96 < parts; p += 128, a += 4 * step) {
+        const float v0 = fin_ld<DEV>(a), u0 = fin_ld<DEV>(a + C), v1 = fin_ld<DEV>(a + step), u1 = fin_ld<DEV>(a + step + C);
+        const float v2 = fin_ld<DEV>(a + 2 * step), u2 = fin_ld<DEV>(a + 2 * step + C), v3 = fin_ld<DEV>(a + 3 * step), u3 = fin_ld<DEV>(a + 3 * step + C);
+        s += (double)v0;  q += (double)u0;
+        s1 += (double)v1; q1 += (double)u1;
+        s2 += (double)v2; q2 += (double)u2;
+        s3 += (double)v3; q3 += (double)u3;
+    }
+    for (; p < parts; p += 32, a += step) {
+        s += (double)fin_ld<DEV>(a);
+        q += (double)fin_ld<DEV>(a + C);
+    }
+    s = (s + s1) + (s2 + s3);
+    q = (q + q1) + (q2 + q3);
+}
+
+template <bool DEV, int NT, typename F>
+__device__ __forceinline__ void bn_sum_channels(const float* __restrict__ rows, int parts, int C, int c0, int c1, int nb, double* red, int tid, F&& fin) {
+    for (int cb = c0; cb < c1; cb += 32 * nb) {
+        const int nitems = min(nb, (c1 - cb + 31) >> 5) * 1024;
+#pragma unroll 2
+        for (int item = tid; item < nitems; item += NT) {
+            const int blk = item >> 10, slice = (item >> 5) & 31, cl = item & 31;
+            const int c = cb + blk * 32 + cl;
+            double s = 0.0, q = 0.0;
+            if (c < c1) sum_partial_rows<DEV>(rows, parts, C, c, slice, s, q);
+            red[(blk * 2 + 0) * 1024 + slice * 32 + cl] = s;
+            red[(blk * 2 + 1) * 1024 + slice * 32 + cl] = q;
+        }
+        __syncthreads();
+        for (int l = tid; l < (nitems >> 5); l += NT) {
+            const int blk = l >> 5, cl = l & 31;
+            const int c = cb + blk * 32 + cl;
+            if (c < c1) {
+                double s = 0.0, q = 0.0;
+                for (int i = 0; i < 32; ++i) { s += red[(blk * 2 + 0) * 1024 + i * 32 + cl]; q += red[(blk * 2 + 1) * 1024 + i * 32 + cl]; }
+                fin(c, s, q);
+            }
+        }
+        __syncthreads();
+    }
+}
+
+struct BnFwdOut {
+    double count;
+    const float* gamma; const float* beta;
+    float eps, momentum;
+    float* running_mean; float* running_var; float* scale; float* shift; float* mean_out; float* invstd_out;
+};
+__device__ __forceinline__ void bn_fwd_channel(const BnFwdOut& o, int c, double s, double q) {
+    const double count = o.count;
+    const double mean = s / count;
+    double var = q / count - mean * mean;
+    if (var < 0.0) var = 0.0;
+    const float invstd = (float)(1.0 / sqrt(var + (double)o.eps));
+    const float sc = o.gamma[c] * invstd;
+    o.scale[c] = sc;
+    o.shift[c] = o.beta[c] - (float)mean * sc;
+    if (o.mean_out) o.mean_out[c] = (float)mean;
+    if (o.invstd_out) o.invstd_out[c] = invstd;
+    if (o.running_mean) {
+        const double unbiased = count > 1.0 ? var * count / (count - 1.0) : var;
+        o.running_mean[c] = (1.f - o.momentum) * o.running_mean[c] + o.momentum * (float)mean;
+        o.running_var[c] = (1.f - o.momentum) * o.running_var[c] + o.momentum * (float)unbiased;
+    }
+}
+template <bool DEV, int NT>
+__device__ __forceinline__ void bn_finalize_channels(const float* __restrict__ stats, int parts, int C, int c0, int c1, const BnFwdOut& o, int nb,
+                                                     double* red, int tid) {
+    bn_sum_channels<DEV, NT>(stats, parts, C, c0, c1, nb, red, tid, [&](int c, double s, double q) { bn_fwd_channel(o, c, s, q); });
+}
+
+struct BnBwdOut {
+    double count;
+    const float* gamma; const float* mean; const float* invstd;
+    float* dgamma; float* dbeta; float* coef;
+};
+__device__ __forceinline__ void bn_bwd_channel(const BnBwdOut& o, int C, int c, double s, double q) {
+    o.dbeta[c] = (float)s;
+    o.dgamma[c] = (float)q;
+    const double a = (double)o.gamma[c] * (double)o.invstd[c];
+    const double b = -a * (double)o.invstd[c] * q / o.count;
+    o.coef[c] = (float)a;
+    o.coef[C + c] = (float)b;
+    o.coef[2 * C + c] = (float)(-a * s / o.count - b * (double)o.mean[c]);
+}
+template <bool DEV, int NT>
+__device__ __forceinline__ void bn_bwd_finalize_channels(const float* __restrict__ red_in, int parts, int C, int c0, int c1, const BnBwdOut& o, int nb,
+                                                         double* red, int tid) {
+    bn_sum_channels<DEV, NT>(red_in, parts, C, c0, c1, nb, red, tid, [&](int c, double s, double q) { bn_bwd_channel(o, C, c, s, q); });
+}
+
+__device__ __forceinline__ void fin_st(float* p, float v) { __hip_atomic_store(p, v, __ATOMIC_RELAXED, __HIP_MEMORY_SCOPE_AGENT); }
+
+__device__ __forceinline__ void mny_finalize_tail(const BnFin* __restrict__ f, const float* rows, int parts, int C, int group, int c0, int c1, int nb,
+                                                  double* red, int* flag, int tid) {
+    wait_vmcnt<0>();
+    __syncthreads();
+    if (tid == 0) {
+        int* t = f->tickets + group;
+        __builtin_amdgcn_fence(__ATOMIC_RELEASE, "agent");
+        wait_vmcnt<0>();
+        const int drawn = __hip_atomic_fetch_add(t, 1, __ATOMIC_RELAXED, __HIP_MEMORY_SCOPE_AGENT);
+        const int last = drawn == parts - 1;
+        if (last) {
+            __hip_atomic_store(t, 0, __ATOMIC_RELAXED, __HIP_MEMORY_SCOPE_AGENT);
+            __builtin_amdgcn_fence(__ATOMIC_ACQUIRE, "agent");
+            wait_vmcnt<0>();
+        }
+        *flag = last;
+    }
+    __syncthreads();
+    if (!*flag) return;
+    const BnFwdOut o{f->count, f->gamma, f->beta, f->eps, f->momentum, f->running_mean, f->running_var, f->scale, f->shift, f->mean, f->invstd};
+    bn_finalize_channels<true, 256>(rows, parts, C, c0, c1, o, nb, red, tid);
+}
+
+}
diff --git a/mobilenet-yolo-pytorch_amd/csrc/common.h b/mobilenet-yolo-pytorch_amd/csrc/common.h
--- a/mobilenet-yolo-pytorch_amd/csrc/common.h
+++ b/mobilenet-yolo-pytorch_amd/csrc/common.h
@@ -169,7 +169,8 @@
     X(NO_DWT5, "MNY_NO_DWT5", kFlag, 0, 1, "no tile form of the 5x5 depthwise unit backward")                                        \
     X(DWT3, "MNY_DWT3", kInt, -1, 1, "tile form of the 3x3 depthwise unit backward: 0 / 1, -1 = per-shape rule")                     \
     X(DWTF, "MNY_DWTF", kInt, -1, 1, "tile form of the depthwise forward: 0 / 1, -1 = per-shape rule")                               \
-    X(NMS_SMALL, "MNY_NMS_SMALL", kFlag, 0, 0, "NMS buckets of any size through the one-workgroup path")
+    X(NMS_SMALL, "MNY_NMS_SMALL", kFlag, 0, 0, "NMS buckets of any size through the one-workgroup path")                              \
+    X(NO_FUSED_FINALIZE, "MNY_NO_FUSED_FINALIZE", kFlag, 0, 0, "BatchNorm finalize as a launch of its own behind every producer")
 enum SwitchType { kFlag, kInt, kWord };
 enum Switch {
 #define X(id, name, type, def, latch, doc) SW_##id,
@@ -242,7 +243,8 @@
 int pw_wide_parts(int64_t M, int K, int N, bool red);
 int pw_wide_launch(const float* A, const float* in_scale, const float* in_shift, int in_act, const float* W, float* C, float* stats,
                    int64_t M, int K, int N, const float* rY, const float* r_scale, const float* r_shift, const float* r_mean,
-                   const float* r_invstd, int r_act, const float* addend, hipStream_t st);
+                   const float* r_invstd, int r_act, const float* addend, hipStream_t st, const void* fin = nullptr);
+bool pw_wide_fin_ok(int64_t M, int K, int N);
 
 bool pw_wide_fix_ok(int64_t M, int K);
 int pw_wide_fix_parts(int64_t M, int K);
diff --git a/mobilenet-yolo-pytorch_amd/csrc/pwgemm.hip b/mobilenet-yolo-pytorch_amd/csrc/pwgemm.hip
--- a/mobilenet-yolo-pytorch_amd/csrc/pwgemm.hip
+++ b/mobilenet-yolo-pytorch_amd/csrc/pwgemm.hip
@@ -2480,6 +2480,20 @@
     return pw_fwd_v1<float>(x, in_scale, in_shift, in_act, w, bias, addend, y, stats, M, K, Nc, st);
 }
 
+extern "C" int mny_pw_fwd_fin_supported(int64_t M, int K, int Nc) {
+    if (M <= 0 || K <= 0 || Nc <= 0) return MNY_EINVAL;
+    return !pw_thin_ok(0, 0, M, K, Nc) && pw_wide_fin_ok(M, K, Nc) ? 1 : 0;
+}
+extern "C" int mny_pw_fwd_fin(const float* x, const float* in_scale, const float* in_shift, int in_act, const float* w, float* y, float* stats,
+                              int64_t M, int K, int Nc, const mny_bn_fin* fin, void* stream) {
+    MNY_REQUIRE(x && w && y && stats && fin, "pw_fwd_fin: null pointer");
+    MNY_REQUIRE(M > 0 && K > 0 && Nc > 0, "pw_fwd_fin: empty problem");
+    MNY_REQUIRE(mny_pw_fwd_fin_supported(M, K, Nc) == 1 && in_act != MNY_ACT_HSIGMOID,
+                "pw_fwd_fin: M=%lld K=%d N=%d does not carry its finalize (mny_pw_fwd_fin_supported): call mny_pw_fwd and mny_bn_finalize", (long long)M, K, Nc);
+    g_pw_route = MNY_ROUTE_WIDE;
+    return pw_wide_launch(x, in_scale, in_shift, in_act, w, y, stats, M, K, Nc, nullptr, nullptr, nullptr, nullptr, nullptr, 0, nullptr, (hipStream_t)stream, fin);
+}
+
 constexpr int kRedMaxTn = 4;
 static bool dgrad_bnred_ok(int64_t M, int K, int Nc, int act) {
     if (K >= 512 && Nc >= 512) return false;
diff --git a/mobilenet-yolo-pytorch_amd/csrc/pwwide.hip b/mobilenet-yolo-pytorch_amd/csrc/pwwide.hip
--- a/mobilenet-yolo-pytorch_amd/csrc/pwwide.hip
+++ b/mobilenet-yolo-pytorch_amd/csrc/pwwide.hip
@@ -2,6 +2,7 @@
 #include <vector>
 
 #include "common.h"
+#include "bn_finalize.h"
 #include "x6.h"
 
 namespace mny {
@@ -15,10 +16,12 @@
     const float* rY; const float* r_scale; const float* r_shift; const float* r_mean; const float* r_invstd; int r_act;
     const float* addend;
     const float* bias;
+    const BnFin* fin;
 };
 
-template <int KS, int TNB, int XF, int MODE>
+template <int KS, int TNB, int XF, int MODE, bool FIN = false>
 __global__ __launch_bounds__(256) __attribute__((amdgpu_waves_per_eu(2, 2))) void pw_wide_kernel(WideArgs p) {
+    static_assert(!FIN || MODE == 1, "the finalize tail belongs to the forward statistics form");
     constexpr int BN = 32 * TNB;
     constexpr bool TWO_ACC = false;
     extern __shared__ __attribute__((aligned(16))) float smem[];
@@ -231,9 +234,16 @@
             float a = 0.f, b = 0.f;
 #pragma unroll
             for (int w = 0; w < 4; ++w) { a += red[(w * BN + tid) * 2]; b += red[(w * BN + tid) * 2 + 1]; }
-            p.stats[(int64_t)x * 2 * N + n0 + tid] = a;
-            p.stats[(int64_t)x * 2 * N + N + n0 + tid] = b;
-        }
+            if constexpr (FIN) {
+                fin_st(p.stats + (int64_t)x * 2 * N + n0 + tid, a);
+                fin_st(p.stats + (int64_t)x * 2 * N + N + n0 + tid, b);
+            } else {
+                p.stats[(int64_t)x * 2 * N + n0 + tid] = a;
+                p.stats[(int64_t)x * 2 * N + N + n0 + tid] = b;
+            }
+        }
+        if constexpr (FIN)
+            mny_finalize_tail(p.fin, p.stats, p.gx, N, y, n0, n0 + BN, TNB, reinterpret_cast<double*>(smem), reinterpret_cast<int*>(smem + TNB * 4096), tid);
     }
 }
 
@@ -276,6 +286,14 @@
 
 int pw_wide_parts(int64_t M, int K, int N, bool red) { return wide_plan(M, K, N, red).gx; }
 
+constexpr size_t kFinMaxBytes = 128 * 1024;
+static size_t wide_fin_lds(int TNB) { return (size_t)TNB * 2 * 32 * 32 * sizeof(double) + 16; }
+bool pw_wide_fin_ok(int64_t M, int K, int N) {
+    if (sw(SW_NO_FUSED_FINALIZE) || !pw_wide_ok(M, K, N, false) || (M & 31) != 0) return false;
+    const WidePlan pl = wide_plan(M, K, N, false);
+    return pl.n_blocks <= MNY_FIN_MAX_GROUPS && (size_t)pl.gx * 2 * 32 * pl.TNB * sizeof(float) <= kFinMaxBytes;
+}
+
 typedef void (*WideKernel)(WideArgs);
 template <int KS, int TNB>
 static WideKernel wide_pick_fwd(int xf, int mode) {
@@ -285,6 +303,10 @@
     }
 }
 template <int KS, int TNB>
+static WideKernel wide_pick_fin(int xf) {
+    return xf == 0 ? pw_wide_kernel<KS, TNB, 0, 1, true> : xf == 1 ? pw_wide_kernel<KS, TNB, 1, 1, true> : pw_wide_kernel<KS, TNB, 2, 1, true>;
+}
+template <int KS, int TNB>
 static WideKernel wide_pick_red(int xf, int mode) {
     if (mode == 4) {
         if constexpr (KS == TNB * 2) return pw_wide_kernel<KS, TNB, 0, 4>;
@@ -292,7 +314,12 @@
     }
     return mode == 2 ? pw_wide_kernel<KS, TNB, 0, 2> : pw_wide_kernel<KS, TNB, 0, 3>;
 }
-static WideKernel wide_pick(int KS, int TNB, int xf, int mode) {
+static WideKernel wide_pick(int KS, int TNB, int xf, int mode, bool fin = false) {
+    if (fin) switch (KS * 10 + TNB) {
+        case 42: return wide_pick_fin<4, 2>(xf); case 43: return wide_pick_fin<4, 3>(xf); case 44: return wide_pick_fin<4, 4>(xf);
+        case 52: return wide_pick_fin<5, 2>(xf); case 53: return wide_pick_fin<5, 3>(xf); case 54: return wide_pick_fin<5, 4>(xf);
+        case 62: return wide_pick_fin<6, 2>(xf); case 63: return wide_pick_fin<6, 3>(xf); default: return wide_pick_fin<6, 4>(xf);
+    }
     if (mode >= 2) switch (KS * 10 + TNB) {
         case 42: return wide_pick_red<4, 2>(xf, mode); case 43: return wide_pick_red<4, 3>(xf, mode);
         case 52: return wide_pick_red<5, 2>(xf, mode); case 53: return wide_pick_red<5, 3>(xf, mode);
@@ -312,7 +339,7 @@
                        const float* r_invstd, int r_act, hipStream_t st) {
     MNY_REQUIRE(pw_wide_fix_ok(M, K) && rY && addend && bias && stats && r_act < MNY_ACT_HSWISH, "pw_wide_fix: unsupported problem M=%lld K=%d", (long long)M, K);
     const WidePlan pl = wide_plan(M, K, K, true);
-    WideArgs a{A, in_scale, in_shift, MNY_ACT_NONE, Q, C, stats, M, K, K, pl.gx, pl.n_blocks, pl.ntiles, rY, r_scale, r_shift, r_mean, r_invstd, r_act, addend, bias};
+    WideArgs a{A, in_scale, in_shift, MNY_ACT_NONE, Q, C, stats, M, K, K, pl.gx, pl.n_blocks, pl.ntiles, rY, r_scale, r_shift, r_mean, r_invstd, r_act, addend, bias, nullptr};
     const WideKernel k = wide_pick(pl.KS, pl.TNB, 0, 4);
     MNY_REQUIRE(k != nullptr, "pw_wide_fix: no kernel for K=%d", K);
     if (!allow_lds((const void*)k, 80 * 1024)) {
@@ -324,7 +351,7 @@
 
 int pw_wide_launch(const float* A, const float* in_scale, const float* in_shift, int in_act, const float* W, float* C, float* stats,
                    int64_t M, int K, int N, const float* rY, const float* r_scale, const float* r_shift, const float* r_mean,
-                   const float* r_invstd, int r_act, const float* addend, hipStream_t st) {
+                   const float* r_invstd, int r_act, const float* addend, hipStream_t st, const void* fin) {
     MNY_REQUIRE(pw_wide_ok(M, K, N, rY != nullptr) && (M & 31) == 0, "pw_wide: unsupported problem M=%lld K=%d N=%d (whole 32-row tiles: callers send the last M %% 32 rows elsewhere)", (long long)M, K, N);
     const WidePlan pl = wide_plan(M, K, N, rY != nullptr);
     MNY_REQUIRE(pl.KS >= 4 && pl.KS <= 6 && pl.TNB >= 2 && pl.TNB <= 4, "pw_wide: no kernel for K=%d, column block %d", K, 32 * pl.TNB);
@@ -335,12 +362,16 @@
     MNY_REQUIRE(!rY || r_act < MNY_ACT_HSWISH, "pw_wide: the reduction form knows the clamp family only (mny_pw_dgrad_bnred_supported)");
     MNY_REQUIRE(rY || !addend, "pw_wide: a plain addend is not supported (callers route it to the LDS-DMA kernel)");
     MNY_REQUIRE(in_act != MNY_ACT_HSIGMOID, "pw_wide: h-sigmoid input transform is not supported");
-    WideArgs a{A, in_scale, in_shift, in_act, W, C, stats, M, K, N, pl.gx, pl.n_blocks, pl.ntiles, rY, r_scale, r_shift, r_mean, r_invstd, r_act, addend, nullptr};
-    const WideKernel k = wide_pick(pl.KS, pl.TNB, XF, mode);
+    MNY_REQUIRE(!fin || (mode == 1 && pw_wide_fin_ok(M, K, N)), "pw_wide: no finalize tail for M=%lld K=%d N=%d", (long long)M, K, N);
+    WideArgs a{A, in_scale, in_shift, in_act, W, C, stats, M, K, N, pl.gx, pl.n_blocks, pl.ntiles, rY, r_scale, r_shift, r_mean, r_invstd, r_act, addend, nullptr,
+               (const BnFin*)fin};
+    const WideKernel k = wide_pick(pl.KS, pl.TNB, XF, mode, fin != nullptr);
+    size_t lds = pl.lds;
+    if (fin && lds < wide_fin_lds(pl.TNB)) lds = wide_fin_lds(pl.TNB);
     if (!allow_lds((const void*)k, 80 * 1024)) {
         set_error("pw_wide: hipFuncSetAttribute failed"); return MNY_EHIP;
     }
-    hipLaunchKernelGGL(k, dim3(pl.grid), dim3(256), pl.lds, st, a);
+    hipLaunchKernelGGL(k, dim3(pl.grid), dim3(256), lds, st, a);
     return check_launch("pw_wide_kernel");
 }
 
diff --git a/mobilenet-yolo-pytorch_amd/engine.py b/mobilenet-yolo-pytorch_amd/engine.py
--- a/mobilenet-yolo-pytorch_amd/engine.py
+++ b/mobilenet-yolo-pytorch_amd/engine.py
@@ -255,6 +255,8 @@
         self.dead_side = bool(self.side_on and bn_batch
                               and any(nd.out.id not in self.live and nd.op in ("dw", "pw", "add") for nd in g.nodes))
         self.stats_ws_side = torch.empty(self.max_parts * 2 * self.maxC, **self._f32) if self.dead_side else self.stats_ws
+        self._fin_tickets = {ws.data_ptr(): torch.zeros(_lib.FIN_MAX_GROUPS, device=dev, dtype=torch.int32) for ws in (self.stats_ws, self.stats_ws_side)}
+        self.fused_finalizes = 0
         dead_forked = self._build_forward(g)
         self._flush_cvt_jobs()
         self._flush_cut_jobs(self.fwd, at_head=True)
@@ -420,7 +422,8 @@
         else:
             conv = self._fwd_exdw_pw if o.id in self.exdw_pw else self._fwd_pw
         parts = conv(nd, u, self._P[nd.conv + ".weight"], stats, st)
-        self._emit_bn_tail(nd.bn, u, parts, u.M, sws, st)
+        if parts is not None:
+            self._emit_bn_tail(nd.bn, u, parts, u.M, sws, st)
 
     def _fwd_stem(self, nd, u, w, stats, st):
         N, H, W, C = self.N, self.H, self.W, u.C
@@ -460,8 +463,22 @@
                                    shape="exdw stats M%d K%d N%d" % (M, i.C, C)))
         return _lib.query("mny_exdw_stat_parts", M, i.C, C)
 
+    def _fin_desc(self, bn, u, M, sws):
+        P = self._P
+        d = _lib.BnFin(*[t.data_ptr() for t in (P[bn + ".weight"], P[bn + ".bias"], P[bn + ".running_mean"], P[bn + ".running_var"],
+                                                u.scale, u.shift, u.mean, u.invstd, self._fin_tickets[sws.data_ptr()])], float(M), BN_EPS, BN_MOMENTUM)
+        return torch.frombuffer(bytearray(bytes(d)), dtype=torch.uint8).to(self.dev)
+
     def _fwd_pw(self, nd, u, w, stats, st):
         i = nd.ins[0]
+        if (self.bn_batch and not self.bf16 and stats is not None
+                and _lib.query("mny_pw_fwd_fin_supported", u.M, i.C, u.C) == 1 and i.act != _lib.ACT_HSIGMOID):
+            x = self._view(i)
+            self.fwd.add("mny_pw_fwd_fin", x[0], x[1], x[2], x[3], self._gemm_weight(w), u.Y, stats, u.M, i.C, u.C, self._fin_desc(nd.bn, u, u.M, stats), st,
+                         label="mny_pw_fwd", meta=dict(flops=2 * u.M * i.C * u.C, bytes=self.eb * (u.M * i.C + u.M * u.C) + 4 * i.C * u.C,
+                                                       shape="M%d K%d N%d +fin" % (u.M, i.C, u.C)))
+            self.fused_finalizes += 1
+            return None
         wop, w6 = self._fwd_weight(w, u.M, i.C, u.C)
         self._emit_pw_gemm(self.fwd, self._view(i), wop, w6, None, None, u.Y, stats, u.M, i.C, u.C, st)
         return _lib.query(self.K("mny_pw_stat_parts"), u.M, i.C, u.C)
diff --git a/mobilenet-yolo-pytorch_amd/ops.py b/mobilenet-yolo-pytorch_amd/ops.py
--- a/mobilenet-yolo-pytorch_amd/ops.py
+++ b/mobilenet-yolo-pytorch_amd/ops.py
@@ -192,6 +192,35 @@
     out = _new(C, R, like=w2d, dtype=dtype)
     call(_k("mny_transpose", out), _p(w2d), _p(out), R, C, _st())
     return out
+
+
+def bn_fin_desc(count, gamma, beta, scale, shift, mean, invstd, tickets, running_mean=None, running_var=None):
+    d = _lib.BnFin(*[t.data_ptr() if t is not None else None for t in (gamma, beta, running_mean, running_var, scale, shift, mean, invstd, tickets)],
+                   float(count), BN_EPS, BN_MOMENTUM)
+    return torch.frombuffer(bytearray(bytes(d)), dtype=torch.uint8).to(gamma.device)
+
+
+def pw_fwd_bn(view, w, gamma, beta, running_mean=None, running_var=None, tickets=None, stats=None):
+    x, sc, sh, act = view
+    K, Nc = x.shape[-1], w.shape[0]
+    M = x.numel() // K
+    y = _new(*x.shape[:-1], Nc, like=x)
+    parts = query("mny_pw_stat_parts", M, K, Nc)
+    if stats is None:
+        stats = _new(parts, 2, Nc, like=x)
+    coef = _new(4, Nc, like=x)
+    fused = x.dtype == torch.float32 and act != _lib.ACT_HSIGMOID and query("mny_pw_fwd_fin_supported", M, K, Nc) == 1
+    if fused:
+        if tickets is None:
+            tickets = torch.zeros(_lib.FIN_MAX_GROUPS, device=x.device, dtype=torch.int32)
+        fin = bn_fin_desc(M, gamma, beta, coef[0], coef[1], coef[2], coef[3], tickets, running_mean, running_var)
+        call("mny_pw_fwd_fin", _p(x), _p(sc), _p(sh), act, _p(w), _p(y), _p(stats), M, K, Nc, ctypes.c_void_p(fin.data_ptr()), _st())
+        y._mny_keep = (fin, tickets)
+    else:
+        call("mny_pw_fwd", _p(x), _p(sc), _p(sh), act, _p(w), None, None, _p(y), _p(stats), M, K, Nc, _st())
+        call("mny_bn_finalize", _p(stats), parts, M, _p(gamma), _p(beta), BN_EPS, BN_MOMENTUM, _p(running_mean), _p(running_var),
+             _p(coef[0]), _p(coef[1]), _p(coef[2]), _p(coef[3]), Nc, _st())
+    return y, coef, fused
 
 
 def bn_finalize(stats, count, gamma, beta, running_mean=None, running_var=None):
diff --git a/mobilenet-yolo-pytorch_amd/switches.py b/mobilenet-yolo-pytorch_amd/switches.py
--- a/mobilenet-yolo-pytorch_amd/switches.py
+++ b/mobilenet-yolo-pytorch_amd/switches.py
@@ -32,6 +32,7 @@
     ("MNY_DWT3", INT, -1, "lib", "tile form of the 3x3 depthwise unit backward: 0 / 1, -1 = per-shape rule"),
     ("MNY_DWTF", INT, -1, "lib", "tile form of the depthwise forward: 0 / 1, -1 = per-shape rule"),
     ("MNY_NMS_SMALL", FLAG, 0, "lib", "NMS buckets of any size through the one-workgroup path"),
+    ("MNY_NO_FUSED_FINALIZE", FLAG, 0, "lib", "BatchNorm finalize as a launch of its own behind every producer"),
     ("MNY_FORCE_DP", FLAG, 0, "bench", "bench.py: run the RCCL data-parallel path even with one rank"),
     ("MNY_LAUNCHER_PARENT_CLEAN", FLAG, 0, "bench", "bench.py: set by its launcher for the rank processes it starts"),
     ("MNY_PRINT_MARKS", FLAG, 0, "bench", "bench.py: print the backward call list's marks"),
```

New measurement: 7083 images/s. About the same (-0.6%).
